# tomasjakab/imm

Hardware: AMD Instinct MI355X
Metric: training images/sec at 128x128 K=10 (higher is better)
Workload: dtype bf16; 1 GPU; BASELINE configs[1] (N>1: configs[2]): CelebA-shape 128x128 K=10 IMM training step (fwd + VGG16 perceptual loss + bwd + clip + Adam), batch 32 per GPU; global_batch=32, image_size=128, n_maps=10, parallelism=dp1, hip_graph=True, weights=seeded random init; synthetic VGG16 (vgg16.caffemodel.h5 unavailable offline)

## Files before the change

__graft_entry__.py:

```python
import os
import sys

ROOT = os.path.dirname(os.path.abspath(__file__))
if ROOT not in sys.path:
    sys.path.insert(0, ROOT)


def build():
    from imm_amd import build as _b
    lib = _b.build()
    import imm_amd
    from imm_amd import _lib
    handle = _lib.load()
    for name in _lib.declared_symbols() + _lib.alignment_symbols() + _lib.compose_symbols() + _lib.unalign_symbols() + _lib.track_symbols():
        getattr(handle, name)
    from oracle import imm_oracle, np_ref
    print('built', lib)


def smoke():
    import torch
    from oracle import imm_oracle as O
    from imm_amd.models.imm_model import IMMModel
    from imm_amd.train.cnn_train_multi import TrainStep
    from imm_amd.utils.box import Box
    assert torch.cuda.is_available(), 'smoke() needs cuda:0'
    torch.cuda.set_device(0)
    cfg = O.default_model_config(10)
    inputs = O.synthetic_inputs(2, 128, seed=0)
    model = IMMModel(Box(dict(cfg)), dtype=torch.bfloat16, device='cuda:0')
    ts = TrainStep(model, 2, 128, world_size=1, use_graph=True)
    loss = ts.step(inputs)
    ts.synchronize()
    eng = model.engine
    P, S = O.init_params(cfg, 128)
    out = O.forward(P, S, inputs, cfg, training=True)
    mu_err = float((eng.mu.cpu() - out['gauss_yx']).abs().max())
    loss_rel = abs(float(loss) - float(out['loss'])) / abs(float(out['loss']))
    print('smoke: loss %.4f (oracle %.4f, rel %.2e)  max|mu - oracle| %.2e  step_count %d' % (
        float(loss), float(out['loss']), loss_rel, mu_err, int(eng.step_count)))
    assert mu_err < 1e-3, mu_err
    assert loss_rel < 1e-3, loss_rel
    assert int(eng.step_count) == 1 and bool(torch.isfinite(eng.params).all())


if __name__ == '__main__':
    build()
    if len(sys.argv) > 1 and sys.argv[1] == 'smoke':
        smoke()
```

imm_amd/_lib.py:

```python
import ctypes as C
import os

import torch

_HERE = os.path.dirname(os.path.abspath(__file__))
LIB_PATH = os.environ.get('IMM_HIP_LIB') or os.path.join(_HERE, 'libimm_hip.so')

IMM_BF16, IMM_F16, IMM_F32 = 0, 1, 2
CONV_BIAS, CONV_RELU, CONV_STATS, CONV_MASK, CONV_OUT_F32 = 1, 2, 4, 8, 16
SSE_BLOCKS = 512
OPTIMIZERS = {'adam': 0, 'adadelta': 1, 'adagrad': 2}
GAUSS_MODES = {'rot': 0, 'flat': 1, 'ankush': 2}
ABI_VERSION = 28


class ImmHipError(RuntimeError):
    pass


class ConvDesc(C.Structure):
    _fields_ = [(n, C.c_int32) for n in (
        'batch', 'hi', 'wi', 'ci', 'ldx', 'ho', 'wo', 'co', 'ldy', 'kh', 'kw', 'stride', 'pad_t', 'pad_l',
        'updiv', 'kpad', 'flags', 'ldmask', 'out_scale', 'out_off_y', 'out_off_x')]


class WgradJob(C.Structure):
    _fields_ = [('desc', ConvDesc), ('x', C.c_void_p), ('dy', C.c_void_p), ('slab', C.c_void_p), ('lddy', C.c_int32),
                ('nsplit', C.c_int32), ('x_scale', C.c_void_p), ('x_shift', C.c_void_p), ('x_relu', C.c_int32),
                ('reserved', C.c_int32)]


class OptHParams(C.Structure):
    _fields_ = [('lr_start', C.c_float), ('lr_decay', C.c_float), ('lr_step', C.c_int32), ('lr_multiple', C.c_float),
                ('beta1', C.c_float), ('beta2', C.c_float), ('eps', C.c_float), ('clip', C.c_float),
                ('grad_scale', C.c_float), ('optim', C.c_int32),
                ('scale_growth_interval', C.c_int32), ('scale_max', C.c_float)]


class KeypointDesc(C.Structure):
    _fields_ = [('w', C.c_void_p), ('b', C.c_void_p), ('geom', C.c_void_p), ('keypoints', C.c_void_p), ('m', C.c_int32),
                ('image_size', C.c_int32)]


_P, _I, _L, _F, _D = C.c_void_p, C.c_int, C.c_int64, C.c_float, C.c_double
_SIGS = {
    'imm_abi_version': [],
    'imm_device_info': [_P],
    'imm_set_cu_limit': [_I],
    'imm_get_cu_limit': [],
    'imm_graph_begin': [_P],
    'imm_graph_end': [_P, C.POINTER(C.c_void_p)],
    'imm_graph_launch': [_P, _P],
    'imm_graph_destroy': [_P],
    'imm_pack_weights': [_P, _P, _I, _I, _I, _I, _I, _I, _I, _I, _I, _P],
    'imm_pack_weights_multi': [_P, _P, _I, _I, _I, _P],
    'imm_pack_weights_multi_blocks': [_I, _I, _I],
    'imm_wgrad_reduce_multi': [_P, _P, _I, _I, _P],
    'imm_conv2d': [C.POINTER(ConvDesc), _I, _P, _P, _P, _P, _P, _P, _P],
    'imm_conv_stats_blocks': [C.POINTER(ConvDesc)],
    'imm_conv2d_variant': [C.POINTER(ConvDesc), _I],
    'imm_conv2d_tap_supported': [C.POINTER(ConvDesc)],
    'imm_conv2d_tap': [C.POINTER(ConvDesc), _I, _P, _P, _P, _P, _P, _I, _P, _I, _P, _I, _I, _P],
    'imm_conv2d_wgrad': [C.POINTER(ConvDesc), _I, _P, _P, _I, _P, _I, _P],
    'imm_conv2d_wgrad_splits': [C.POINTER(ConvDesc), _I],
    'imm_conv2d_wgrad_variant': [C.POINTER(ConvDesc), _I, _I, C.POINTER(C.c_int), C.POINTER(C.c_int), C.POINTER(C.c_int)],
    'imm_conv2d_wgrad_multi_plan': [_P, _I, _I, _P],
    'imm_conv2d_wgrad_multi': [_P, _P, _P],
    'imm_conv2d_wgrad_reduce': [_P, _I, _I, _I, _I, _I, _I, _I, _P, _P],
    'imm_colsum': [_P, _I, _L, _I, _I, _I, _P, _P, _P],
    'imm_colsum_blocks': [_L, _I],
    'imm_bn_finalize': [_P, _I, _I, _L, _P, _P, _F, _F, _I, _P, _P, _P, _P, _P, _P, _P],
    'imm_bn_apply_relu': [_P, _I, _L, _I, _I, _P, _P, _I, _P, _I, _P],
    'imm_bn_apply_fused': [_P, _I, _I, _L, _P, _P, _F, _F, _I, _P, _P, _P, _P, _P, _P, _P, _I, _I, _I, _P, _I, _P, _I, _I, _I, _P],
    'imm_bn_bwd_apply_fused': [_P, _I, _I, _L, _P, _P, _I, _P, _I, _I, _P, _P, _P, _P, _I, _P, _P, _P, _I, _P],
    'imm_rows_reduce': [_P, _I, _I, _I, _P, _P],
    'imm_bn_bwd_reduce': [_P, _I, _P, _I, _I, _L, _I, _P, _P, _P, _P, _I, _P, _P],
    'imm_bn_bwd_blocks': [_L, _I],
    'imm_bn_bwd_reduce_up': [_P, _I, _P, _I, _P, _I, _I, _I, _I, _I, _I, _P, _P, _P, _P, _I, _P, _P],
    'imm_bn_bwd_finalize': [_P, _I, _I, _I, _L, _P, _P, _P, _I, _P, _P, _P, _P],
    'imm_bn_bwd_apply': [_P, _I, _P, _I, _I, _L, _I, _P, _P, _P, _P, _I, _P, _P, _I, _P],
    'imm_upsample2x_fwd': [_P, _P, _I, _I, _I, _I, _I, _I, _I, _P],
    'imm_upsample2x_bwd': [_P, _P, _I, _I, _I, _I, _I, _I, _I, _P],
    'imm_resize_ac_fwd': [_P, _P, _I, _I, _I, _I, _I, _I, _I, _I, _I, _P],
    'imm_resize_ac_bwd': [_P, _P, _I, _I, _I, _I, _I, _I, _I, _I, _I, _P],
    'imm_maxpool2_fwd': [_P, _P, _I, _I, _I, _I, _I, _P],
    'imm_maxpool2_bwd': [_P, _P, _P, _I, _I, _I, _I, _I, _I, _P],
    'imm_pack_image': [_P, _P, _I, _L, _P],
    'imm_pack_image_taps': [_P, _P, _I, _I, _I, _I, _I, _I, _I, _P],
    'imm_softargmax_gauss_fwd': [_P, _I, _I, _I, _I, _I, _F, _I, _P, _P, _P, _P, _I, _I, _I, _P],
    'imm_softargmax_gauss_bwd': [_P, _I, _I, _I, _I, _I, _I, _F, _I, _P, _P, _P, _P, _I, _I, _P],
    'imm_gauss_render_f32': [_P, _I, _I, _F, _I, _P, _I, _P],
    'imm_pose_head_fwd': [_P, _I, _I, _P, _I, _P, _I, _I, _I, _I, _I, _F, _I, _P, _I, _P, _P, _P, _P, _I, _I,
                          C.POINTER(KeypointDesc), _P],
    'imm_pose_head_bwd': [_P, _I, _I, _I, _I, _I, _I, _F, _I, _P, _P, _P, _P, _I, _I, _P, _I, _I, _P, _I, _P, _P],
    'imm_vgg_conv1_1_fwd': [_P, _P, _I, _I, _I, _P, _P, _P, _I, _I, _P],
    'imm_vgg_head_supported': [_I, _I, _I],
    'imm_vgg_head_fwd': [_P, _P, _I, _I, _I, _P, _P, _P, _I, _P, _P, _I, _P, _P, _I, _P],
    'imm_vgg_conv1_1_bwd': [_P, _I, _I, _I, _P, _P, _P, _I, _P, _P, _I, _I, _P, _I, _P],
    'imm_image_loss_grad': [_P, _P, _I, _I, _I, _P, _P, _I, _I, _P, _I, _I, _P],
    'imm_copy_f32': [_P, _P, _L, _P],
    'imm_debug_stamp': [_P, _I, _P],
    'imm_tps_warp': [_P, _I, _I, _I, _I, _I, _P, _I, _P, _P, _I, _P, _P, _I, _P],
    'imm_tps_warp_pad': [_P, _I, _I, _I, _I, _I, _I, _I, _I, _I, _I, _I, _I, _I, _P, _I, _P, _P, _I, _P],
    'imm_conv2d_group': [_P, _I, _I, _P, _P, _P, _P, _P, _P],
    'imm_conv_first_supported': [_I, _I, _I, _I],
    'imm_conv_first_stats_blocks': [_I, _I],
    'imm_conv_first': [_P, _P, _I, _P, _P, _I, _P, _I, _I, _I, _I, _I, _P],
    'imm_conv2d_nol_supported': [C.POINTER(ConvDesc)],
    'imm_conv2d_nol_stats_blocks': [C.POINTER(ConvDesc)],
    'imm_conv2d_nol': [C.POINTER(ConvDesc), _I, _P, _P, _P, _I, _P, _P, _P, _P, _P],
    'imm_conv2d_dgrad_s2_supported': [_I, _I, _I, _I, _I, _I],
    'imm_conv2d_dgrad_s2': [_P, _I, _P, _I, _P, _I, _I, _I, _I, _I, _I, _P],
    'imm_conv2d_group_stats_blocks': [_P, _I],
    'imm_upsample2x_bwd_bn': [_P, _P, _I, _I, _I, _I, _I, _I, _I, _P, _I, _P, _P],
    'imm_upsample2x_bwd_bn_blocks': [_I, _I, _I, _I],
    'imm_crc32c': [_P, C.c_uint64, C.POINTER(C.c_uint32)],
    'imm_rccl_unique_id': [_P],
    'imm_rccl_init': [_I, _I, _P, C.POINTER(C.c_void_p)],
    'imm_rccl_allreduce': [_P, _P, _L, _P],
    'imm_rccl_destroy': [_P],
    'imm_resize_crop_u8': [_P, _P, _P, _P, _I, _I, _I, _I, _I, _I, _I, _I, _P, _I, _P],
    'imm_unpool_tap_grad': [_P, _P, _P, _P, _I, _I, _I, _I, _P, _I, _P, _I, _P],
    'imm_masked_sse_pool': [_P, _P, _I, _I, _I, _I, _P, _I, _P, _P, _P, _P],
    'imm_masked_sse_multi': [_I, _P, _P, _P, _P, _P, _I, _I, _P, _I, _I, _P],
    'imm_masked_sse_all': [_I, _P, _P, _P, _P, _P, _I, _I, _P, _I, _I, _P, _I, _P, _I, _I, _P, _P],
    'imm_masked_sse': [_P, _P, _I, _I, _I, _I, _P, _I, _I, _P, _P],
    'imm_masked_sse_f32': [_P, _I, _P, _I, _I, _I, _I, _P, _I, _P, _P],
    'imm_perceptual_finalize': [_P, _I, _P, _P, _I, _P, _I, _I, _P, _P, _P],
    'imm_cost_ema': [_P, _P, _F, _P],
    'imm_rms16': [_P, _L, _I, _P, _I, _P, _P],
    'imm_tap_grad': [_P, _I, _P, _P, _I, _I, _I, _I, _P, _I, _P, _I, _I, _I, _P],
    'imm_weight_decay_loss': [_P, _P, _P, _P, _I, _P, _P, _P, _P],
    'imm_clip_adam_step': [_P, _P, _P, _P, _P, _P, _P, _I, _I, _P, _P, _P, _P, _P, _P, _P, C.POINTER(OptHParams), _P, _P],
}

_SIGS_ALIGN = {
    'imm_align_coeffs': [_P, _P, _I, _I, _I, _P, _P],
    'imm_align_warp_u8': [_P, _I, _P, _P, _I, _P, _P, _P, _P, _I, _I, _I, _I, _P, _I, _P],
}

_SIGS_COMPOSE = {
    'imm_compose_u8': [_P, _P, _P, _I, _P, _P, _P, _P, _I, _I, _I, _I, _P],
}

_SIGS_UNALIGN = {
    'imm_unalign_maps': [_P, _P, _P, _P, _I, _I, _I, _I, _P, _P, _P],
    'imm_unalign_u8': [_P, _P, _P, _I, _P, _P, _P, _P, _F, _P, _I, _I, _I, _I, _P],
}

_SIGS_TRACK = {
    'imm_track_step': [_P, _P, _P, _P, _I, _I, _I, _I, _I, _I, _D, _D, _D, _D, _D, _D, _I, _P, _P, _P, _P, _P, _P],
}

_SIGS64 = {
    'imm_conv2d_workspace_bytes': [C.POINTER(ConvDesc)],
    'imm_conv2d_group_workspace_bytes': [_P, _I],
    'imm_conv2d_wgrad_workspace_bytes': [C.POINTER(ConvDesc), _I, _I],
    'imm_conv2d_wgrad_multi_table_bytes': [_I],
    'imm_colsum_workspace_bytes': [_L, _I],
    'imm_bn_bwd_workspace_bytes': [_L, _I],
    'imm_upsample2x_bwd_bn_workspace_bytes': [_I, _I, _I, _I],
    'imm_masked_sse_workspace_bytes': [_I],
    'imm_vgg_head_scratch_bytes': [_I, _I],
}

_lib = None


def declared_symbols():
    return sorted(list(_SIGS) + list(_SIGS64) + ['imm_last_error', 'imm_source_digest'])


def alignment_symbols():
    return sorted(_SIGS_ALIGN)


def compose_symbols():
    return sorted(_SIGS_COMPOSE)


def unalign_symbols():
    return sorted(_SIGS_UNALIGN)


def track_symbols():
    return sorted(_SIGS_TRACK)


def load():
    global _lib
    if _lib is not None:
        return _lib
    if not os.path.exists(LIB_PATH):
        raise ImmHipError('libimm_hip.so not found at %s: build it with `python imm_amd/build.py` '
                          '(there is no CPU fallback for the product path)' % LIB_PATH)
    if 'IMM_HIP_LIB' not in os.environ and os.path.isdir(os.path.join(_HERE, 'csrc')):
        from . import build as _b
        want, have = _b.source_digest(), _b.library_digest(LIB_PATH)
        if want != have:
            if not _b.have_compiler():
                raise ImmHipError('libimm_hip.so is stale (built from sources %s.., checkout is %s..) and hipcc is not '
                                  'available to rebuild it' % (have[:12] or '?', want[:12]))
            _b.build(verbose=False)
    lib = C.CDLL(LIB_PATH)
    for name in ('imm_last_error', 'imm_source_digest'):
        getattr(lib, name).restype = C.c_char_p
        getattr(lib, name).argtypes = []
    for name, args in list(_SIGS.items()) + list(_SIGS_ALIGN.items()) + list(_SIGS_COMPOSE.items()) + list(_SIGS_UNALIGN.items()) + list(_SIGS_TRACK.items()):
        fn = getattr(lib, name)
        fn.argtypes = args
        fn.restype = C.c_int
    for name, args in _SIGS64.items():
        fn = getattr(lib, name)
        fn.argtypes = args
        fn.restype = C.c_int64
    v = lib.imm_abi_version()
    if v != ABI_VERSION:
        raise ImmHipError('libimm_hip.so ABI %d != expected %d' % (v, ABI_VERSION))
    _lib = lib
    return lib


def check(rc, what):
    if rc != 0:
        raise ImmHipError('%s failed (%d): %s' % (what, rc, load().imm_last_error().decode()))


def call(name, *args):
    rc = getattr(load(), name)(*args)
    if rc != 0:
        raise ImmHipError('%s failed (%d): %s' % (name, rc, load().imm_last_error().decode()))
```

imm_amd/csrc/loss_optim.hip:

```cpp
#include "common.h"

#define LO_THREADS 256
#define IMM_NORM2_SANE 1e30f

template <typename ET>
__global__ __launch_bounds__(LO_THREADS) void masked_sse_kernel(const typename ET::T* __restrict__ a, const typename ET::T* __restrict__ b,
                                                                int batch, int s, int c8n, const float* __restrict__ mask,
                                                                int S, int l1, float* __restrict__ partial) {
  __shared__ float red[4];
  const int r = S / s;
  const int64_t total = (int64_t)batch * s * s * c8n;
  float acc = 0.f;
  for (int64_t idx = (int64_t)blockIdx.x * blockDim.x + threadIdx.x; idx < total;
       idx += (int64_t)gridDim.x * blockDim.x) {
    const int64_t p = idx / c8n;
    float mk = 1.f;
    if (mask) {
      const int xx = (int)(p % s);
      const int64_t t = p / s;
      const int yy = (int)(t % s);
      const int64_t bi = t / s;
      mk = mask[(bi * S + (int64_t)yy * r) * S + (int64_t)xx * r];
    }
    float fa[8], fb[8];
// ... 101 lines not shown
  if (c == 3) {
    const bool a4 = lda == 4 && ((uintptr_t)a & 15) == 0, b4 = ldb == 4 && ((uintptr_t)b & 15) == 0;
    for (; p + 3 * stride < npix; p += 4 * stride) {
      float va[4][3], vb[4][3], mk[4];
#pragma unroll
      for (int u = 0; u < 4; ++u) {
        const int64_t q = p + u * stride;
        if (a4) { const float4 t = *(const float4*)(a + q * 4); va[u][0] = t.x; va[u][1] = t.y; va[u][2] = t.z; }
        else { va[u][0] = a[q * lda]; va[u][1] = a[q * lda + 1]; va[u][2] = a[q * lda + 2]; }
        if (b4) { const float4 t = *(const float4*)(b + q * 4); vb[u][0] = t.x; vb[u][1] = t.y; vb[u][2] = t.z; }
        else { vb[u][0] = b[q * ldb]; vb[u][1] = b[q * ldb + 1]; vb[u][2] = b[q * ldb + 2]; }
        mk[u] = mask ? mask[q] : 1.f;
      }
#pragma unroll
      for (int u = 0; u < 4; ++u) {
        float sq = 0.f;
#pragma unroll
        for (int ch = 0; ch < 3; ++ch) { const float d = va[u][ch] - vb[u][ch]; sq += l1 ? fabsf(d) : d * d; }
        acc += mk[u] * sq;
      }
    }
  }
  for (; p < npix; p += stride) {
    float sq = 0.f;
    for (int ch = 0; ch < c; ++ch) { const float d = a[p * lda + ch] - b[p * ldb + ch]; sq += l1 ? fabsf(d) : d * d; }
    acc += (mask ? mask[p] : 1.f) * sq;
  }
  return acc;
}

__global__ __launch_bounds__(LO_THREADS) void masked_sse_f32_kernel(const float* __restrict__ a, int lda,
                                                                    const float* __restrict__ b, int ldb, int64_t npix,
                                                                    int c, const float* __restrict__ mask, int l1,
                                                                    float* __restrict__ partial) {
  __shared__ float red[4];
  float acc = sse_f32_thread_sum(a, lda, b, ldb, npix, c, mask, l1);
  acc = block_sum_256(acc, red);
  if (threadIdx.x == 0) partial[blockIdx.x] = acc;
}

struct SseRgbArgs { const float* a; const float* b; int lda, ldb, c; int64_t npix; float* partial; };
template <typename ET>
__global__ __launch_bounds__(LO_THREADS) void masked_sse_all_kernel(const SseMultiArgs g, int n16, const SseRgbArgs rgb, int batch,
                                                                    const float* __restrict__ mask, int S, int l1) {
  __shared__ float red[4];
  const int f = blockIdx.y;
  float acc = 0.f;
  if (f == n16) {
    acc = sse_f32_thread_sum(rgb.a, rgb.lda, rgb.b, rgb.ldb, rgb.npix, rgb.c, mask, l1);
    acc = block_sum_256(acc, red);
    if (threadIdx.x == 0) rgb.partial[blockIdx.x] = acc;
    return;
  }
  const typename ET::T* __restrict__ a = (const typename ET::T*)g.a[f];
  const typename ET::T* __restrict__ b = (const typename ET::T*)g.b[f];
  const int s = g.s[f], c8n = g.c8n[f];
  const int r = S / s;
  const int64_t total = (int64_t)batch * s * s * c8n;
  for (int64_t idx = (int64_t)blockIdx.x * blockDim.x + threadIdx.x; idx < total;
       idx += (int64_t)gridDim.x * blockDim.x) {
    const int64_t p = idx / c8n;
    float mk = 1.f;
    if (mask) {
      const int xx = (int)(p % s);
      const int64_t t = p / s;
      const int yy = (int)(t % s);
      const int64_t bi = t / s;
      mk = mask[(bi * S + (int64_t)yy * r) * S + (int64_t)xx * r];
    }
    float fa[8], fb[8];
    unpack8<ET>(ld8<ET>(a + idx * 8), fa);
    unpack8<ET>(ld8<ET>(b + idx * 8), fb);
    float sq = 0.f;
#pragma unroll
    for (int i = 0; i < 8; ++i) { const float d = fa[i] - fb[i]; sq += l1 ? fabsf(d) : d * d; }
    acc += mk * sq;
  }
  acc = block_sum_256(acc, red);
  if (threadIdx.x == 0) g.partial[f][blockIdx.x] = acc;
}

extern "C" int imm_masked_sse(const void* a, const void* b, int dtype, int batch, int s, int c, const float* mask, int S,
                              int l1, float* partial, void* stream) {
  IMM_REQUIRE(a && b && partial && batch > 0 && s > 0 && c > 0 && c % 8 == 0, "masked_sse: args");
  IMM_REQUIRE(mask == nullptr || (S >= s && S % s == 0), "masked_sse: mask side %d not a multiple of feature side %d", S, s);
  IMM_DISPATCH_DTYPE_F32(dtype, hipLaunchKernelGGL((masked_sse_kernel<ET>), dim3(IMM_SSE_BLOCKS), dim3(LO_THREADS), 0,
                                               (hipStream_t)stream, (const typename ET::T*)a, (const typename ET::T*)b, batch, s, c / 8,
                                               mask, S, l1, partial));
  IMM_CHECK_LAUNCH("imm_masked_sse");
  return 0;
}

extern "C" int imm_masked_sse_multi(int n, const void* const* a, const void* const* b, const int32_t* s_host, const int32_t* c_host,
                                    float* const* partial, int dtype, int batch, const float* mask, int S, int l1, void* stream) {
  IMM_REQUIRE(n >= 1 && n <= 8 && a && b && s_host && c_host && partial && batch > 0, "masked_sse_multi: args");
  SseMultiArgs g;
  for (int i = 0; i < 8; ++i) {
    const int k = i < n ? i : 0;
    IMM_REQUIRE(a[k] && b[k] && partial[k] && s_host[k] > 0 && c_host[k] > 0 && c_host[k] % 8 == 0, "masked_sse_multi: feature %d", k);
    IMM_REQUIRE(mask == nullptr || (S >= s_host[k] && S % s_host[k] == 0), "masked_sse_multi: mask side %d vs feature side %d", S, s_host[k]);
    g.a[i] = a[k]; g.b[i] = b[k]; g.s[i] = s_host[k]; g.c8n[i] = c_host[k] / 8; g.partial[i] = partial[k];
  }
  IMM_DISPATCH_DTYPE_F32(dtype, hipLaunchKernelGGL((masked_sse_multi_kernel<ET>), dim3(IMM_SSE_BLOCKS, n), dim3(LO_THREADS), 0,
                                               (hipStream_t)stream, g, batch, mask, S, l1));
  IMM_CHECK_LAUNCH("imm_masked_sse_multi");
  return 0;
}

extern "C" int imm_masked_sse_all(int n, const void* const* a, const void* const* b, const int32_t* s_host, const int32_t* c_host,
                                  float* const* partial, int dtype, int batch, const float* mask, int S, int l1,
                                  const float* img_a, int lda, const float* img_b, int ldb, int img_c, float* img_partial, void* stream) {
  IMM_REQUIRE(n >= 1 && n <= 8 && a && b && s_host && c_host && partial && batch > 0, "masked_sse_all: args");
  IMM_REQUIRE(img_a && img_b && img_partial && img_c > 0 && lda >= img_c && ldb >= img_c && S > 0, "masked_sse_all: image pair");
  SseMultiArgs g;
  for (int i = 0; i < 8; ++i) {
    const int k = i < n ? i : 0;
    IMM_REQUIRE(a[k] && b[k] && partial[k] && s_host[k] > 0 && c_host[k] > 0 && c_host[k] % 8 == 0, "masked_sse_all: feature %d", k);
    IMM_REQUIRE(S >= s_host[k] && S % s_host[k] == 0, "masked_sse_all: image side %d vs feature side %d", S, s_host[k]);
    g.a[i] = a[k]; g.b[i] = b[k]; g.s[i] = s_host[k]; g.c8n[i] = c_host[k] / 8; g.partial[i] = partial[k];
  }
  SseRgbArgs rgb;
  rgb.a = img_a; rgb.b = img_b; rgb.lda = lda; rgb.ldb = ldb; rgb.c = img_c; rgb.npix = (int64_t)batch * S * S; rgb.partial = img_partial;
  IMM_DISPATCH_DTYPE_F32(dtype, hipLaunchKernelGGL((masked_sse_all_kernel<ET>), dim3(IMM_SSE_BLOCKS, n + 1), dim3(LO_THREADS), 0,
                                               (hipStream_t)stream, g, n, rgb, batch, mask, S, l1));
  IMM_CHECK_LAUNCH("imm_masked_sse_all");
  return 0;
}

extern "C" int imm_masked_sse_pool(const void* a, const void* b, int dtype, int batch, int s, int c, const float* mask, int S,
                                   float* partial, void* pool_a, void* pool_b, void* stream) {
  IMM_REQUIRE(a && b && partial && pool_b && batch > 0 && s > 0 && s % 2 == 0 && c > 0 && c % 8 == 0, "masked_sse_pool: args");
  IMM_REQUIRE(mask == nullptr || (S >= s && S % s == 0), "masked_sse_pool: mask side %d not a multiple of feature side %d", S, s);
  IMM_DISPATCH_DTYPE_F32(dtype, hipLaunchKernelGGL((masked_sse_pool_kernel<ET>), dim3(IMM_SSE_BLOCKS), dim3(LO_THREADS), 0,
                                               (hipStream_t)stream, (const typename ET::T*)a, (const typename ET::T*)b, batch, s, c / 8,
                                               mask, S, partial, (typename ET::T*)pool_a, (typename ET::T*)pool_b));
  IMM_CHECK_LAUNCH("imm_masked_sse_pool");
  return 0;
}

extern "C" int imm_masked_sse_f32(const float* a, int lda, const float* b, int ldb, int batch, int s, int c,
                                  const float* mask, int l1, float* partial, void* stream) {
  IMM_REQUIRE(a && b && partial && batch > 0 && s > 0 && c > 0 && lda >= c && ldb >= c, "masked_sse_f32: args");
  hipLaunchKernelGGL(masked_sse_f32_kernel, dim3(IMM_SSE_BLOCKS), dim3(LO_THREADS), 0, (hipStream_t)stream, a, lda, b, ldb,
                     (int64_t)batch * s * s, c, mask, l1, partial);
  IMM_CHECK_LAUNCH("imm_masked_sse_f32");
  return 0;
}

#define PF_THREADS 1024
__global__ __launch_bounds__(PF_THREADS) void perceptual_finalize_kernel(const float* __restrict__ partial, int nfeat,
                                                                         const float* __restrict__ nel, float* agg,
                                                                         int training, const float* __restrict__ wd_loss,
                                                                         int l1, int mode, const float* __restrict__ loss_scale,
                                                                         float* __restrict__ out) {
  __shared__ double sse[16];
  const int tid = threadIdx.x, lane = tid & 63, wave = tid >> 6;
  const float nel_f = tid < nfeat ? nel[tid] : 1.f;
  const float agg_f = tid < nfeat ? agg[tid] : 1.f;
  const float ls = (tid < nfeat && loss_scale) ? loss_scale[0] : 1.f;
  const float wd = (tid == 0 && wd_loss) ? wd_loss[0] : 0.f;
  if (wave < nfeat) {
    const float* pf = partial + wave * IMM_SSE_BLOCKS + lane;
    float x[IMM_SSE_BLOCKS / 64];
#pragma unroll
    for (int i = 0; i < IMM_SSE_BLOCKS / 64; ++i) x[i] = pf[64 * i];
    double v = 0.0;
#pragma unroll
    for (int i = 0; i < IMM_SSE_BLOCKS / 64; ++i) v += (double)x[i];
#pragma unroll 1
    for (int o = 32; o >= 1; o >>= 1) v += __shfl_xor(v, o, 64);
    if (lane == 0) sse[wave] = v;
  }
  __syncthreads();
  if (mode == IMM_LOSS_L2) {
    if (tid == 0) {
      const float m = (float)(sse[0] / (double)nel_f);
      out[0] = m; out[nfeat] = m;
      out[2 * nfeat] = ls * ((1000.f / 255.f) * 2.f / nel_f);
      out[3 * nfeat] = 1000.f * m;
      out[3 * nfeat + 1] = wd;
      out[3 * nfeat + 2] = 1000.f * m / 255.f + wd;
    }
    return;
  }
  __shared__ float terms[16];
  if (tid < nfeat) {
    const int f = tid;
    const float m = (float)(sse[f] / (double)nel_f);
    const float a = agg_f;
    const float wl = a + 0.01f * (m - a);
    const float term = m / wl;
    out[f] = term;
    out[nfeat + f] = m;
    out[2 * nfeat + f] = ls * (1000.f * (1.f / wl - 0.01f * m / (wl * wl)) * (l1 ? 1.f : 2.f) / nel_f);
    if (training) agg[f] = wl;
    terms[f] = term;
  }
  __syncthreads();
  if (tid == 0) {
    float rec = 0.f;
    for (int f = 0; f < nfeat; ++f) rec += terms[f];
    rec *= 1000.f;
    out[3 * nfeat] = rec;
    out[3 * nfeat + 1] = wd;
    out[3 * nfeat + 2] = rec + wd;
  }
}

extern "C" int imm_perceptual_finalize(const float* partial, int nfeat, const float* nel, float* agg, int training,
                                       const float* wd_loss, int l1, int mode, const float* loss_scale, float* out,
                                       void* stream) {
  IMM_REQUIRE(partial && nel && agg && out && nfeat > 0 && nfeat <= 16, "perceptual_finalize: args");
  IMM_REQUIRE(mode == IMM_LOSS_PERCEPTUAL || (mode == IMM_LOSS_L2 && nfeat == 1 && !l1), "perceptual_finalize: mode");
  hipLaunchKernelGGL(perceptual_finalize_kernel, dim3(1), dim3(PF_THREADS), 0, (hipStream_t)stream, partial, nfeat, nel,
                     agg, training, wd_loss, l1, mode, loss_scale, out);
  IMM_CHECK_LAUNCH("imm_perceptual_finalize");
  return 0;
}

template <typename ET>
__global__ void tap_grad_kernel(typename ET::T* __restrict__ da, int has_in, const typename ET::T* __restrict__ ap,
                                const typename ET::T* __restrict__ ag, int batch, int s, int c8n, const float* __restrict__ mask,
                                int S, const float* __restrict__ coef, int idx_coef, int relu, int l1) {
  const int r = S / s;
  const float ck = coef[idx_coef];
  const int64_t total = (int64_t)batch * s * s * c8n;
  for (int64_t idx = (int64_t)blockIdx.x * blockDim.x + threadIdx.x; idx < total;
       idx += (int64_t)gridDim.x * blockDim.x) {
    const int64_t p = idx / c8n;
    float mk = 1.f;
    if (mask) {
      const int xx = (int)(p % s);
      const int64_t t = p / s;
      const int yy = (int)(t % s);
      const int64_t bi = t / s;
      mk = mask[(bi * S + (int64_t)yy * r) * S + (int64_t)xx * r];
    }
    float fp[8], fg[8], d[8];
    unpack8<ET>(ld8<ET>(ap + idx * 8), fp);
    unpack8<ET>(ld8<ET>(ag + idx * 8), fg);
    if (has_in) unpack8<ET>(ld8<ET>(da + idx * 8), d);
    const float cm = ck * mk;
#pragma unroll
    for (int i = 0; i < 8; ++i) {
      float e = fp[i] - fg[i];
      if (l1) e = e > 0.f ? 1.f : (e < 0.f ? -1.f : 0.f);
      float v = (has_in ? d[i] : 0.f) + cm * e;
      if (relu && !(fp[i] > 0.f)) v = 0.f;
      d[i] = v;
    }
    st8<ET>(da + idx * 8, pack8<ET>(d));
  }
}

template <typename ET>
__global__ void unpool_tap_grad_kernel(typename ET::T* __restrict__ da, const typename ET::T* __restrict__ dpool,
                                       const typename ET::T* __restrict__ ap, const typename ET::T* __restrict__ ag, int batch, int s,
                                       int c8n, const float* __restrict__ mask, int S, const float* __restrict__ coef,
                                       int idx_coef) {
  const int r = S / s, so = s / 2, c = c8n * 8;
  const float ck = coef[idx_coef];
  const int64_t total = (int64_t)batch * so * so * c8n;
  for (int64_t idx = (int64_t)blockIdx.x * blockDim.x + threadIdx.x; idx < total;
       idx += (int64_t)gridDim.x * blockDim.x) {
    const int cg = (int)(idx % c8n);
    int64_t t = idx / c8n;
    const int X = (int)(t % so); t /= so;
    const int Y = (int)(t % so);
    const int64_t bi = t / so;
    const int64_t off = ((bi * s + 2 * Y) * s + 2 * X) * c + cg * 8;
    const int64_t qoff[4] = {off, off + c, off + (int64_t)s * c, off + (int64_t)s * c + c};
    float fp[4][8], fg[4][8], g[8], o[4][8], cm[4];
#pragma unroll
    for (int q = 0; q < 4; ++q) {
      unpack8<ET>(ld8<ET>(ap + qoff[q]), fp[q]);
      unpack8<ET>(ld8<ET>(ag + qoff[q]), fg[q]);
      const int yy = 2 * Y + (q >> 1), xx = 2 * X + (q & 1);
      cm[q] = ck * (mask ? mask[(bi * S + (int64_t)yy * r) * S + (int64_t)xx * r] : 1.f);
    }
    unpack8<ET>(ld8<ET>(dpool + ((bi * so + Y) * so + X) * c + cg * 8), g);
#pragma unroll
    for (int i = 0; i < 8; ++i) {
      int am = 0; float mv = fp[0][i];
#pragma unroll
      for (int q = 1; q < 4; ++q) if (fp[q][i] > mv) { mv = fp[q][i]; am = q; }
#pragma unroll
      for (int q = 0; q < 4; ++q) {
        float v = ((q == am) ? g[i] : 0.f) + cm[q] * (fp[q][i] - fg[q][i]);
        if (!(fp[q][i] > 0.f)) v = 0.f;
        o[q][i] = v;
      }
    }
#pragma unroll
    for (int q = 0; q < 4; ++q) st8<ET>(da + qoff[q], pack8<ET>(o[q]));
  }
}

extern "C" int imm_unpool_tap_grad(void* da, const void* dpool, const void* a_pred, const void* a_gt, int dtype, int batch, int s,
                                   int c, const float* mask, int S, const float* coef, int idx, void* stream) {
  IMM_REQUIRE(da && dpool && a_pred && a_gt && coef && batch > 0 && s > 0 && s % 2 == 0 && c > 0 && c % 8 == 0 && idx >= 0,
              "unpool_tap_grad: args");
  IMM_REQUIRE(mask == nullptr || (S >= s && S % s == 0), "unpool_tap_grad: mask side");
  const int64_t total = (int64_t)batch * (s / 2) * (s / 2) * (c / 8);
  int64_t blocks = (total + LO_THREADS - 1) / LO_THREADS;
  if (blocks > 16384) blocks = 16384;
  IMM_DISPATCH_DTYPE_F32(dtype, hipLaunchKernelGGL((unpool_tap_grad_kernel<ET>), dim3((int)blocks), dim3(LO_THREADS), 0,
                                               (hipStream_t)stream, (typename ET::T*)da, (const typename ET::T*)dpool,
                                               (const typename ET::T*)a_pred, (const typename ET::T*)a_gt, batch, s, c / 8, mask, S, coef, idx));
  IMM_CHECK_LAUNCH("imm_unpool_tap_grad");
  return 0;
}

extern "C" int imm_tap_grad(void* da, int has_in, const void* a_pred, const void* a_gt, int dtype, int batch, int s, int c,
                            const float* mask, int S, const float* coef, int idx, int relu, int l1, void* stream) {
  IMM_REQUIRE(da && a_pred && a_gt && coef && batch > 0 && s > 0 && c > 0 && c % 8 == 0 && idx >= 0, "tap_grad: args");
  IMM_REQUIRE(mask == nullptr || (S >= s && S % s == 0), "tap_grad: mask side");
  const int64_t total = (int64_t)batch * s * s * (c / 8);
  int64_t blocks = (total + LO_THREADS - 1) / LO_THREADS;
  if (blocks > 16384) blocks = 16384;
  IMM_DISPATCH_DTYPE_F32(dtype, hipLaunchKernelGGL((tap_grad_kernel<ET>), dim3((int)blocks), dim3(LO_THREADS), 0,
                                               (hipStream_t)stream, (typename ET::T*)da, has_in, (const typename ET::T*)a_pred,
                                               (const typename ET::T*)a_gt, batch, s, c / 8, mask, S, coef, idx, relu, l1));
  IMM_CHECK_LAUNCH("imm_tap_grad");
  return 0;
}

template <typename ET>
__global__ void image_loss_grad_kernel(const float* __restrict__ gt, const float* __restrict__ pred, int ldp, int64_t npix,
                                       const float* __restrict__ mask, const float* __restrict__ coef, int idx, int l1,
                                       typename ET::T* __restrict__ dpred, int lddp) {
  const int nvec = lddp / 8;
  const float ck = coef[idx];
  for (int64_t i = (int64_t)blockIdx.x * blockDim.x + threadIdx.x; i < npix * nvec; i += (int64_t)gridDim.x * blockDim.x) {
    const int64_t p = i / nvec;
    const int cg = (int)(i - p * nvec);
    float o[8] = {0.f, 0.f, 0.f, 0.f, 0.f, 0.f, 0.f, 0.f};
    if (cg == 0) {
      const float cm = ck * (mask ? mask[p] : 1.f);
#pragma unroll
      for (int ch = 0; ch < 3; ++ch) {
        float d = pred[p * ldp + ch] - gt[p * 3 + ch];
        if (l1) d = d > 0.f ? 1.f : (d < 0.f ? -1.f : 0.f);
        o[ch] = cm * d;
      }
    }
    st8<ET>(dpred + p * lddp + cg * 8, pack8<ET>(o));
  }
}

extern "C" int imm_image_loss_grad(const float* gt, const float* pred, int ldp, int batch, int s, const float* mask,
                                   const float* coef, int idx, int l1, void* dpred, int lddp, int dtype, void* stream) {
  IMM_REQUIRE(gt && pred && coef && dpred && batch > 0 && s > 0 && ldp >= 3 && idx >= 0, "image_loss_grad: args");
  IMM_REQUIRE(lddp >= 8 && lddp % 8 == 0, "image_loss_grad: lddp=%d must be a multiple of 8", lddp);
  const int64_t npix = (int64_t)batch * s * s;
  int64_t blocks = (npix * (lddp / 8) + LO_THREADS - 1) / LO_THREADS;
  if (blocks > 8192) blocks = 8192;
  IMM_DISPATCH_DTYPE_F32(dtype, hipLaunchKernelGGL((image_loss_grad_kernel<ET>), dim3((int)blocks), dim3(LO_THREADS), 0,
                                               (hipStream_t)stream, gt, pred, ldp, npix, mask, coef, idx, l1,
                                               (typename ET::T*)dpred, lddp));
  IMM_CHECK_LAUNCH("imm_image_loss_grad");
  return 0;
}

__global__ __launch_bounds__(LO_THREADS) void wd_partial_kernel(const float* __restrict__ params,
                                                                const int32_t* __restrict__ blk_seg,
                                                                const int32_t* __restrict__ blk_begin,
                                                                const int32_t* __restrict__ blk_end,
                                                                const float* __restrict__ seg_wd,
                                                                float* __restrict__ blk_partial) {
  __shared__ float red[4];
  const int blk = blockIdx.x;
  const float wd = seg_wd[blk_seg[blk]];
  float acc = 0.f;
  if (wd != 0.f)
    for (int i = blk_begin[blk] + threadIdx.x; i < blk_end[blk]; i += LO_THREADS) { const float w = params[i]; acc += w * w; }
  acc = block_sum_256(acc, red);
  if (threadIdx.x == 0) blk_partial[blk] = 0.5f * wd * acc;
}

__global__ __launch_bounds__(LO_THREADS) void sum_partials_kernel(const float* __restrict__ partial, int n, float* out) {
  __shared__ double dred[LO_THREADS];
  double v = 0.0;
  for (int i = threadIdx.x; i < n; i += LO_THREADS) v += (double)partial[i];
  dred[threadIdx.x] = v;
  __syncthreads();
  for (int o = LO_THREADS / 2; o > 0; o >>= 1) {
    if (threadIdx.x < o) dred[threadIdx.x] += dred[threadIdx.x + o];
    __syncthreads();
  }
  if (threadIdx.x == 0) out[0] = (float)dred[0];
}

extern "C" int imm_weight_decay_loss(const float* params, const int32_t* blk_seg, const int32_t* blk_begin,
                                     const int32_t* blk_end, int nblk, const float* seg_wd, float* blk_partial, float* out,
                                     void* stream) {
  IMM_REQUIRE(params && blk_seg && blk_begin && blk_end && seg_wd && blk_partial && out && nblk > 0, "weight_decay_loss: args");
  hipLaunchKernelGGL(wd_partial_kernel, dim3(nblk), dim3(LO_THREADS), 0, (hipStream_t)stream, params, blk_seg, blk_begin,
                     blk_end, seg_wd, blk_partial);
  hipLaunchKernelGGL(sum_partials_kernel, dim3(1), dim3(LO_THREADS), 0, (hipStream_t)stream, blk_partial, nblk, out);
  IMM_CHECK_LAUNCH("imm_weight_decay_loss");
  return 0;
}

__global__ void cost_ema_kernel(const float* __restrict__ cost3, float* __restrict__ state, float decay) {
  if (threadIdx.x < 3) state[threadIdx.x] = decay * state[threadIdx.x] + (1.f - decay) * cost3[threadIdx.x];
  if (threadIdx.x == 3) state[3] += 1.f;
}

extern "C" int imm_cost_ema(const float* cost3, float* state4, float decay, void* stream) {
  IMM_REQUIRE(cost3 && state4 && decay >= 0.f && decay < 1.f, "cost_ema: args");
  hipLaunchKernelGGL(cost_ema_kernel, dim3(1), dim3(64), 0, (hipStream_t)stream, cost3, state4, decay);
  IMM_CHECK_LAUNCH("imm_cost_ema");
  return 0;
}

template <typename ET>
__global__ __launch_bounds__(LO_THREADS) void sumsq16_kernel(const typename ET::T* __restrict__ x, int64_t n8, float* __restrict__ partial) {
  __shared__ float red[4];
  float acc = 0.f;
  for (int64_t i = (int64_t)blockIdx.x * LO_THREADS + threadIdx.x; i < n8; i += (int64_t)gridDim.x * LO_THREADS) {
    float f[8];
    unpack8<ET>(ld8<ET>(x + i * 8), f);
#pragma unroll
    for (int e = 0; e < 8; ++e) acc = fmaf(f[e], f[e], acc);
  }
  acc = block_sum_256(acc, red);
  if (threadIdx.x == 0) partial[blockIdx.x] = acc;
}

__global__ __launch_bounds__(LO_THREADS) void rms_finish_kernel(const float* __restrict__ partial, int n, double count, float* out) {
  __shared__ double dred[LO_THREADS];
  double v = 0.0;
  for (int i = threadIdx.x; i < n; i += LO_THREADS) v += (double)partial[i];
  dred[threadIdx.x] = v;
  __syncthreads();
  for (int o = LO_THREADS / 2; o > 0; o >>= 1) {
    if (threadIdx.x < o) dred[threadIdx.x] += dred[threadIdx.x + o];
    __syncthreads();
  }
  if (threadIdx.x == 0) out[0] = (float)sqrt(dred[0] / count);
}

extern "C" int imm_rms16(const void* x, int64_t n, int dtype, float* partial, int nblk, float* out, void* stream) {
  IMM_REQUIRE(x && partial && out && n > 0 && n % 8 == 0 && nblk > 0 && nblk <= 4096, "rms16: args (n must be a multiple of 8)");
  IMM_REQUIRE(((uintptr_t)x % 16) == 0, "rms16: 16-byte alignment");
  IMM_DISPATCH_DTYPE_F32(dtype, hipLaunchKernelGGL((sumsq16_kernel<ET>), dim3(nblk), dim3(LO_THREADS), 0, (hipStream_t)stream,
                                              (const typename ET::T*)x, n / 8, partial));
  hipLaunchKernelGGL(rms_finish_kernel, dim3(1), dim3(LO_THREADS), 0, (hipStream_t)stream, partial, nblk, (double)n, out);
  IMM_CHECK_LAUNCH("imm_rms16");
  return 0;
}

__device__ __forceinline__ void opt_learning_rate(const imm_opt_hparams& hp, int gs, int tt, float* lr_t, float* lr) {
  const double l = (double)hp.lr_multiple * (double)hp.lr_start * pow((double)hp.lr_decay, (double)(gs / hp.lr_step));
  *lr_t = (float)(l * sqrt(1.0 - pow((double)hp.beta2, (double)tt)) / (1.0 - pow((double)hp.beta1, (double)tt)));
  *lr = (float)l;
}

__global__ __launch_bounds__(LO_THREADS) void grad_prepare_kernel(const float* __restrict__ params, float* __restrict__ grads,
                                                                  const int32_t* __restrict__ blk_seg,
                                                                  const int32_t* __restrict__ blk_begin,
                                                                  const int32_t* __restrict__ blk_end,
                                                                  const float* __restrict__ seg_wd, float grad_scale,
                                                                  const float* __restrict__ loss_scale,
                                                                  float* __restrict__ blk_partial, int nblk,
                                                                  const int32_t* __restrict__ step_count,
                                                                  const int32_t* __restrict__ adam_t, float* __restrict__ lr_state,
                                                                  imm_opt_hparams hp) {
  __shared__ float red[4];
  const int blk = blockIdx.x;
  if (blk == nblk) {
    if (threadIdx.x == 0) opt_learning_rate(hp, step_count[0], adam_t[0] + 1, lr_state, lr_state + 1);
    return;
  }
  if (loss_scale) grad_scale *= 1.f / loss_scale[0];
  const float wd = seg_wd[blk_seg[blk]];
  float acc = 0.f;
  const int b0 = blk_begin[blk], b1 = blk_end[blk];
  const int a0 = min((b0 + 3) & ~3, b1), a1 = max(a0, b1 & ~3);
  for (int i = b0 + threadIdx.x; i < a0; i += LO_THREADS) {
    const float g = grads[i] * grad_scale + wd * params[i];
    grads[i] = g; acc += g * g;
  }
  for (int i = a0 + 4 * threadIdx.x; i < a1; i += 4 * LO_THREADS) {
    float4 g = *(const float4*)(grads + i);
    const float4 w = *(const float4*)(params + i);
    g.x = g.x * grad_scale + wd * w.x; g.y = g.y * grad_scale + wd * w.y;
    g.z = g.z * grad_scale + wd * w.z; g.w = g.w * grad_scale + wd * w.w;
    *(float4*)(grads + i) = g;
    acc += (g.x * g.x + g.y * g.y) + (g.z * g.z + g.w * g.w);
  }
  for (int i = a1 + threadIdx.x; i < b1; i += LO_THREADS) {
    const float g = grads[i] * grad_scale + wd * params[i];
    grads[i] = g; acc += g * g;
  }
  acc = block_sum_256(acc, red);
  if (threadIdx.x == 0) blk_partial[blk] = acc;
}

__global__ __launch_bounds__(LO_THREADS) void clip_adam_kernel(float* __restrict__ params, const float* __restrict__ grads,
                                                               float* __restrict__ m, float* __restrict__ v,
                                                               const int32_t* __restrict__ blk_seg,
                                                               const int32_t* __restrict__ blk_begin,
                                                               const int32_t* __restrict__ blk_end,
                                                               const int32_t* __restrict__ seg_first_blk,
                                                               const float* __restrict__ blk_partial, int nblk,
                                                               float* __restrict__ seg_norm2, int32_t* __restrict__ step_count,
                                                               int32_t* __restrict__ adam_t, const float* __restrict__ lr_state,
                                                               float* __restrict__ ls, imm_opt_hparams hp) {
  __shared__ double dred[LO_THREADS / 64];
  const int blk = blockIdx.x, tid = threadIdx.x;
  const bool extra = blk == nblk;
  const int seg = extra ? 0 : blk_seg[blk];
  const int b0 = extra ? 0 : blk_begin[blk], b1 = extra ? 0 : blk_end[blk];
  const int a0 = min((b0 + 3) & ~3, b1), a1 = max(a0, b1 & ~3);
  const int i0 = a0 + 4 * tid;
  const bool first = i0 < a1;
  float4 g0 = {0.f, 0.f, 0.f, 0.f}, m0 = g0, v0 = g0, w0 = g0;
  if (first) { g0 = *(const float4*)(grads + i0); m0 = *(const float4*)(m + i0); v0 = *(const float4*)(v + i0); w0 = *(const float4*)(params + i0); }

  const int f0 = seg_first_blk[seg], f1 = seg_first_blk[seg + 1];
  double ps = 0.0;
  int bad = 0;
  const int sb1 = ls != nullptr ? nblk : f1;
  int sb0 = tid;
  if (ls == nullptr && f0 > tid) sb0 = tid + (f0 - tid + LO_THREADS - 1) / LO_THREADS * LO_THREADS;
  for (int b = sb0; b < sb1; b += LO_THREADS) {
    const float p = blk_partial[b];
    bad |= !(p <= IMM_NORM2_SANE);
    if (b >= f0 && b < f1) ps += (double)p;
  }
#pragma unroll
  for (int o = 32; o > 0; o >>= 1) ps += __shfl_xor(ps, o, 64);
  if ((tid & 63) == 0) dred[tid >> 6] = ps;
  bad = __syncthreads_or(bad);
  const bool skip = ls != nullptr && bad != 0;
  double t = 0.0;
#pragma unroll
  for (int w = 0; w < LO_THREADS / 64; ++w) t += dred[w];
  const float norm2 = (float)t;
  if (tid == 0 && !extra && blk == f0) seg_norm2[seg] = norm2;
  if (extra) {
    if (tid == 0) {
      if (ls) {
        float S = ls[0], clean = ls[1];
        if (skip) { S = fmaxf(S * 0.5f, 1.f); clean = 0.f; ls[2] += 1.f; }
        else if (hp.scale_growth_interval > 0 && clean + 1.f >= (float)hp.scale_growth_interval) {
          S = fminf(S * 2.f, hp.scale_max > 0.f ? hp.scale_max : S * 2.f); clean = 0.f;
        } else clean += 1.f;
        ls[0] = S; ls[1] = clean; ls[3] = skip ? 1.f : 0.f;
      }
      if (!skip) {
        step_count[0] += 1;
        adam_t[0] += 1;
      }
    }
    return;
  }
  if (skip) return;
  float factor = 1.f;
  if (hp.clip > 0.f) factor = hp.clip / fmaxf(sqrtf(norm2), hp.clip);
  const float lr_t = lr_state[0], lr = lr_state[1];
  auto one = [&](float g, float& mi, float& vi, float& w) {
    g *= factor;
    if (hp.optim == IMM_OPT_ADAM) {
      mi = hp.beta1 * mi + (1.f - hp.beta1) * g;
      vi = hp.beta2 * vi + (1.f - hp.beta2) * g * g;
      w -= lr_t * mi / (sqrtf(vi) + hp.eps);
    } else if (hp.optim == IMM_OPT_ADADELTA) {
      vi = hp.beta1 * vi + (1.f - hp.beta1) * g * g;
      const float u = sqrtf(mi + hp.eps) / sqrtf(vi + hp.eps) * g;
      mi = hp.beta1 * mi + (1.f - hp.beta1) * u * u;
      w -= lr * u;
    } else {
      vi += g * g;
      w -= lr * g / sqrtf(vi);
    }
  };
  for (int i = b0 + tid; i < a0; i += LO_THREADS) one(grads[i], m[i], v[i], params[i]);
  if (first) {
    one(g0.x, m0.x, v0.x, w0.x); one(g0.y, m0.y, v0.y, w0.y); one(g0.z, m0.z, v0.z, w0.z); one(g0.w, m0.w, v0.w, w0.w);
    *(float4*)(m + i0) = m0; *(float4*)(v + i0) = v0; *(float4*)(params + i0) = w0;
  }
  for (int i = i0 + 4 * LO_THREADS; i < a1; i += 4 * LO_THREADS) {
    const float4 g = *(const float4*)(grads + i);
    float4 mi = *(const float4*)(m + i), vi = *(const float4*)(v + i), w = *(const float4*)(params + i);
    one(g.x, mi.x, vi.x, w.x); one(g.y, mi.y, vi.y, w.y); one(g.z, mi.z, vi.z, w.z); one(g.w, mi.w, vi.w, w.w);
    *(float4*)(m + i) = mi; *(float4*)(v + i) = vi; *(float4*)(params + i) = w;
  }
  for (int i = a1 + tid; i < b1; i += LO_THREADS) one(grads[i], m[i], v[i], params[i]);
}

extern "C" int imm_clip_adam_step(float* params, float* grads, float* m, float* v, const int32_t* blk_seg,
                                  const int32_t* blk_begin, const int32_t* blk_end, int nblk, int nseg,
                                  const int32_t* seg_first_blk, const float* seg_wd, float* blk_partial, float* seg_norm2,
                                  int32_t* step_count, int32_t* adam_t, float* lr_state, const imm_opt_hparams* hp,
                                  float* loss_scale_state, void* stream) {
  IMM_REQUIRE(params && grads && m && v && blk_seg && blk_begin && blk_end && seg_first_blk && seg_wd && blk_partial &&
                  seg_norm2 && step_count && adam_t && lr_state && hp, "clip_adam_step: null");
  IMM_REQUIRE(nblk > 0 && nseg > 0 && hp->lr_step > 0, "clip_adam_step: dims");
  IMM_REQUIRE(hp->optim >= IMM_OPT_ADAM && hp->optim <= IMM_OPT_ADAGRAD, "clip_adam_step: optim %d", hp->optim);
  hipStream_t s = (hipStream_t)stream;
  hipLaunchKernelGGL(grad_prepare_kernel, dim3(nblk + 1), dim3(LO_THREADS), 0, s, params, grads, blk_seg, blk_begin, blk_end,
                     seg_wd, hp->grad_scale, loss_scale_state, blk_partial, nblk, step_count, adam_t, lr_state, *hp);
  hipLaunchKernelGGL(clip_adam_kernel, dim3(nblk + 1), dim3(LO_THREADS), 0, s, params, grads, m, v, blk_seg, blk_begin, blk_end,
                     seg_first_blk, blk_partial, nblk, seg_norm2, step_count, adam_t, lr_state, loss_scale_state, *hp);
  IMM_CHECK_LAUNCH("imm_clip_adam_step");
  return 0;
}
```

imm_amd/engine.py:

```python
import math
import os
from collections import OrderedDict

import numpy as np
import torch

from . import _lib as L
from . import ops

BN_EPS = 1e-3
BN_MOMENTUM = 0.99
BN_DIRECT_ROWS = int(os.environ.get('IMM_BN_DIRECT_ROWS', '512'))
WEIGHT_DECAY = 1e-5
INIT_STD = 0.01
PERCEPTUAL_WS = [100.0, 1.6, 2.3, 1.8, 2.8, 100.0]
SUPPORTED_COMP = ['input', 'conv1_2', 'conv2_2', 'conv3_2', 'conv4_2', 'conv5_2']
VGG_LAYERS = [('conv1_1', 1, 64), ('conv1_2', 64, 64), ('conv2_1', 64, 128), ('conv2_2', 128, 128),
              ('conv3_1', 128, 256), ('conv3_2', 256, 256), ('conv3_3', 256, 256),
              ('conv4_1', 256, 512), ('conv4_2', 512, 512), ('conv4_3', 512, 512),
              ('conv5_1', 512, 512), ('conv5_2', 512, 512)]
VGG_POOL_AFTER = ('conv1_2', 'conv2_2', 'conv3_3', 'conv4_3')
WGRAD_MULTI_MAX_JOBS, WGRAD_MULTI_MAX_VARIANTS = 64, 16


# ... 2 lines not shown
    for gk, members in groups.items():
        generic = gk[0] // 100000 == 0
        members = list(members)
        while members:
            room_jobs, room_slots = max_jobs - cur_jobs, max_slots - cur_slots
            take = min(len(members), room_jobs, room_slots) if generic else (min(len(members), room_jobs) if room_slots >= 1 else 0)
            if take <= 0:
                chunks.append(cur); cur, cur_jobs, cur_slots = [], 0, 0
                continue
            part, members = members[:take], members[take:]
            cur.append((gk, part)); cur_jobs += len(part); cur_slots += len(part) if generic else 1
    if cur:
        chunks.append(cur)
    return chunks
COST_EMA_STATE = 'summaries/cost_movavg'
VGG_TAPS = {'conv1_2': 1, 'conv2_2': 2, 'conv3_2': 3, 'conv4_2': 4, 'conv5_2': 5}


def encoder_spec(n_filters):
    f = n_filters
    return [(7, 3, f, 1), (3, f, f, 1), (3, f, 2 * f, 2), (3, 2 * f, 2 * f, 1), (3, 2 * f, 4 * f, 2),
            (3, 4 * f, 4 * f, 1), (3, 4 * f, 8 * f, 2), (3, 8 * f, 8 * f, 1)]


def renderer_spec(cfg, image_size, n_out):
    filters = cfg.n_filters_render * 8
    cin = cfg.n_filters * 8 + cfg.n_maps
    size, spec = 16, []
    while size <= image_size:
        spec.append((3, cin, filters, True, False))
        if size == image_size:
            spec.append((3, filters, n_out, False, False))
            break
        spec.append((3, filters, filters, True, True))
        cin = filters
        size *= 2
        if filters >= 8:
            filters //= 2
    return spec


def render_sizes(cfg, max_size):
    sizes, size = [], max_size
    while True:
        sizes.append(size)
        if size <= cfg.min_res:
            break
        size = size // cfg.renderer_stride
    return sizes


def n_renderer_out(cfg):
    extra = len(cfg.perceptual.comp) if getattr(cfg, 'channels_bug_fix', False) else 0
    return 3 + extra


def trainable_spec(cfg, image_size):
    out = []

    def add(scope, k, cin, cout, bn):
        out.append((scope + '/w', (k, k, cin, cout), WEIGHT_DECAY))
        out.append((scope + '/b', (cout,), 0.0))
        if bn:
            out.append((scope + '/gamma', (cout,), 0.0))
            out.append((scope + '/beta', (cout,), 0.0))

    for enc in ('image_encoder', 'pose_encoder'):
        for i, (k, ci, co, _s) in enumerate(encoder_spec(cfg.n_filters)):
            add('model/%s/encoder/conv_%d' % (enc, i + 1), k, ci, co, True)
        if enc == 'pose_encoder':
            add('model/pose_encoder/conv_1', 1, cfg.n_filters * 8, cfg.n_maps, False)
    for i, (k, ci, co, bn, _u) in enumerate(renderer_spec(cfg, image_size, n_renderer_out(cfg))):
        add('model/renderer/conv_%d' % (i + 1), k, ci, co, bn)
    return out


def truncated_normal(rng, shape, std):
    z = rng.standard_normal(shape)
    bad = np.abs(z) > 2.0
    while bad.any():
        z[bad] = rng.standard_normal(int(bad.sum()))
        bad = np.abs(z) > 2.0
    return (z * std).astype(np.float32)


def synthetic_vgg_weights(seed=2):
    rng = np.random.default_rng(seed)
    w = OrderedDict()
    for name, cin, cout in VGG_LAYERS:
        w['vgg16/%s/weights' % name] = torch.from_numpy(
            (rng.standard_normal((3, 3, cin, cout)) * math.sqrt(2.0 / (9 * cin))).astype(np.float32))
        w['vgg16/%s/biases' % name] = torch.from_numpy((rng.standard_normal(cout) * 0.1).astype(np.float32))
    return w


class _Launch:
    __slots__ = ('fn', 'tag', 'flops', 'bytes', 'name', 'lane', 'variant', 'cus', 'group')

    def __init__(self, fn, tag, flops=0.0, nbytes=0.0, name='', lane=0, variant='', cus=0, group=''):
        self.fn, self.tag, self.flops, self.bytes, self.name, self.lane, self.variant = fn, tag, flops, nbytes, name, lane, variant
        self.cus, self.group = cus, group


class _ConvLayer:
    pass


class IMMEngine:
    def __init__(self, cfg, batch, image_size, device='cuda:0', act_dtype=torch.bfloat16, seed=1, vgg_weights=None,
                 hparams=None, world_size=1, dp_buckets=None):
        if cfg.gauss_mode not in L.GAUSS_MODES:
            raise ValueError('Unknown mode: ' + str(cfg.gauss_mode))
        if cfg.reconstruction_loss not in ('perceptual', 'l2'):
            raise ValueError('Reconsutruction loss-type: ' + str(cfg.reconstruction_loss) + ' not understood')
        self.loss_kind = cfg.reconstruction_loss
        self.comp = list(cfg.perceptual.comp) if self.loss_kind == 'perceptual' else ['input']
        if self.loss_kind == 'perceptual':
            if not self.comp or len(set(self.comp)) != len(self.comp) or len(self.comp) > len(PERCEPTUAL_WS):
                raise ValueError('perceptual.comp must name 1..%d distinct features, got %r' % (len(PERCEPTUAL_WS), self.comp))
            if any(n not in SUPPORTED_COMP for n in self.comp):
                raise NotImplementedError('perceptual.comp entries must come from %r (the layers the shipped configs tap), got %r'
                                          % (SUPPORTED_COMP, self.comp))
        self.l1 = self.loss_kind == 'perceptual' and not cfg.perceptual.l2
        if image_size % 16 or image_size < 64:
            raise ValueError('image side must be a multiple of 16 and >= 64')
        L.load()
        self.cfg, self.B, self.S, self.dev, self.dt = cfg, int(batch), int(image_size), torch.device(device), act_dtype
        self.f32 = act_dtype == torch.float32
        self.K = int(cfg.n_maps)
        self.world_size = world_size
        self.dp_buckets = int(dp_buckets if dp_buckets is not None else os.environ.get('IMM_DP_BUCKETS', '1'))
        self.use_mask = bool(cfg.loss_mask)
        self.n_cu, self.arch = ops.device_info()
        self._alloc_bytes = 0

        self.spec = trainable_spec(cfg, self.S)
        sizes = [int(np.prod(s)) for _n, s, _w in self.spec]
        self.tab = ops.SegmentTable(sizes, [w for _n, _s, w in self.spec], self.dev)
        self.params = self._zeros(self.tab.total)
        self.grads = self._zeros(self.tab.total)
        self.adam_m = self._zeros(self.tab.total)
        self.adam_v = self._zeros(self.tab.total)
        self.pview, self.gview = OrderedDict(), OrderedDict()
        for i, (name, shape, _wd) in enumerate(self.spec):
            o0, o1 = self.tab.offsets[i], self.tab.offsets[i + 1]
            self.pview[name] = self.params[o0:o1].view(shape)
            self.gview[name] = self.grads[o0:o1].view(shape)
        self.opt_blk_partial = self._zeros(self.tab.nblk)
        self.seg_norm2 = self._zeros(self.tab.nseg)
        self.step_count = torch.zeros(1, dtype=torch.int32, device=self.dev)
        self.adam_t = torch.zeros(1, dtype=torch.int32, device=self.dev)
        self.lr_state = self._zeros(2)
        self.wd_loss = self._zeros(1)
        hp = dict(lr_start=1e-3, lr_decay=0.95, lr_step=100000, lr_multiple=1.0, beta1=0.9, beta2=0.999, eps=1e-8,
                  clip=1.0, grad_scale=1.0 / world_size, optim='adam', scale_growth_interval=1000, scale_max=2.0 ** 24)
        hp.update(hparams or {})
        ls0 = hp.pop('loss_scale', 4096.0 if act_dtype == torch.float16 else 0.0) or 0.0
        if ls0 and (ls0 < 1.0 or math.log2(ls0) != int(math.log2(ls0))):
            raise ValueError('loss_scale must be a power of two >= 1, got %r' % (ls0,))
        self.loss_scale_state = None
        if ls0:
            self.loss_scale_state = self._zeros(4)
            self.loss_scale_state[0] = float(ls0)
        self._loss_scale_init = float(ls0)
        self.optim = str(hp['optim']).lower()
        if self.optim not in L.OPTIMIZERS:
            raise ValueError('Optimizer = %s not suppoerted' % hp['optim'])
        if self.optim == 'adadelta':
            hp.update(beta1=0.95, eps=1e-6)
        hp['optim'] = L.OPTIMIZERS[self.optim]
        self.hp = ops.OptHParams(**hp)

        self.state = OrderedDict()
        self.nfeat = len(self.comp)
        self.loss_agg = torch.tensor(PERCEPTUAL_WS[:self.nfeat], dtype=torch.float32, device=self.dev)
        self.vgg_w = OrderedDict()
        for k, v in (vgg_weights or synthetic_vgg_weights()).items():
            self.vgg_w[k] = torch.empty(tuple(v.shape), dtype=v.dtype, device=self.dev)
            ops.upload(self.vgg_w[k], v, k)

        self.prog_pack, self.prog_fwd, self.prog_bwd, self.prog_opt = [], [], [], []
        self.two_streams = os.environ.get('IMM_TWO_STREAMS', '1') != '0'
        self.nol = os.environ.get('IMM_NOL', '0') != '0' and not self.f32
        self._skip_tags = set(t for t in os.environ.get('IMM_DEBUG_SKIP_TAGS', '').split(',') if t)
        self._stamp_mode = os.environ.get('IMM_DEBUG_STAMPS', '')
        self._stamp_buf = torch.zeros(8192, dtype=torch.int64, device=self.dev) if self._stamp_mode else None
        self._stamp_names = []
        self._side = None
        self._pack_jobs, self._reduce_jobs, self._wgrad_pending, self._colsum_pending = [], [], [], []
        self._training = True
        self._build_network()
        self.init_parameters(seed)

    def _zeros(self, *shape, dtype=torch.float32):
        t = torch.zeros(*shape, dtype=dtype, device=self.dev)
        self._alloc_bytes += t.numel() * t.element_size()
        return t

    def _act(self, *shape):
        return self._zeros(*shape, dtype=self.dt)

    def init_parameters(self, seed=1):
        rng = np.random.default_rng(seed)
        host = torch.zeros(self.tab.total, dtype=torch.float32)
        for i, (name, shape, _wd) in enumerate(self.spec):
            o0 = self.tab.offsets[i]
            n = int(np.prod(shape))
            if name.endswith('/w'):
                host[o0:o0 + n] = torch.from_numpy(truncated_normal(rng, shape, INIT_STD)).reshape(-1)
            elif name.endswith('/gamma'):
                host[o0:o0 + n] = 1.0
        ops.upload(self.params, host, 'the initial parameters')
        for k, v in self.state.items():
            v.fill_(1.0 if k.endswith('moving_variance') else 0.0)
        self.loss_agg.copy_(torch.tensor(PERCEPTUAL_WS[:self.nfeat]))
        self.reset_optimizer_slots(); self.grads.zero_(); self.step_count.zero_()
        self.run(self.prog_pack)

    def reset_optimizer_slots(self):
        self.adam_m.zero_()
        self.adam_v.fill_(0.1 if self.optim == 'adagrad' else 0.0)
        self.adam_t.zero_()
        if self.loss_scale_state is not None:
            self.loss_scale_state.zero_()
            self.loss_scale_state[0] = self._loss_scale_init

    def load_parameters(self, named, state=None):
        for name in self.pview:
            ops.upload(self.pview[name], named[name], name)
        if state:
            for k, v in state.items():
                if k in self.state:
                    ops.upload(self.state[k], v, k)
                elif k.startswith('loss/') and k.endswith('_agg'):
                    if self.loss_kind == 'perceptual' and k[5:-4] in self.comp:
                        self.loss_agg[self.comp.index(k[5:-4])] = float(v)
                elif k.startswith('vgg16/'):
                    ops.upload(self.vgg_w[k], v, k)
                elif k == COST_EMA_STATE:
                    ops.upload(self.cost_ema, torch.as_tensor(v, dtype=torch.float32).reshape(4), k)
                else:
                    raise KeyError(k)
            self._pack_vgg()
        self.run(self.prog_pack)

    def named_parameters(self):
        return OrderedDict((k, v.detach().clone()) for k, v in self.pview.items())

    def named_state(self):
        out = OrderedDict((k, v.detach().clone()) for k, v in self.state.items())
        if self.loss_kind == 'perceptual':
            for i, name in enumerate(self.comp):
                out['loss/%s_agg' % name] = self.loss_agg[i].detach().clone()
        out[COST_EMA_STATE] = self.cost_ema.detach().clone()
        return out

    def _add(self, prog, fn, tag, flops=0.0, nbytes=0.0, name='', desc=None, variant=''):
        cus = int(getattr(self, '_cur_cus', 0))
        if desc is not None:
            if cus:
                ops.set_cu_limit(cus)
            try:
                variant = '%s:%d' % ops.conv2d_variant(desc, self.dt)
            finally:
                if cus:
                    ops.set_cu_limit(0)
        prog.append(_Launch(fn, tag, flops, nbytes, name or getattr(self, '_cur_scope', ''), getattr(self, '_cur_lane', 0), variant,
                            cus, getattr(self, '_cur_group', '')))

    def _signal(self, prog, key, lane=None):
        prog.append(_Launch(None, 'record:' + key, lane=self._cur_lane if lane is None else lane, group=getattr(self, '_cur_group', '')))

    def _wait(self, prog, key, lane):
        prog.append(_Launch(None, 'wait:' + key, lane=lane))

    def _mark(self, prog, what, lane=1):
        prog.append(_Launch(None, what, lane=lane, group=getattr(self, '_cur_group', '')))

    def _nol_consumer_ok(self, H, W, ci, ldx, co, k, stride, bn, out_f32):
        if not self.nol or k != 3 or ci != ldx:
            return False
        ldy = ops.round_up(co, 4) if out_f32 else ops.round_up(co, 8)
        flags = L.CONV_BIAS | (L.CONV_OUT_F32 if out_f32 else 0) | (L.CONV_STATS if bn else 0)
        fd = ops.fwd_desc(self.B, H, W, ci, ldx, co, ldy, k, stride, flags)
        if not ops.conv2d_nol_supported(fd):
            return False
        lddy = ldy if not out_f32 else ops.round_up(co, 32)
        key, _wps, _units, _pcu = ops.conv2d_wgrad_variant(fd, lddy, self.dt)
        return key // 100000 == 2

    def _conv_block(self, scope, x, H, W, ci_real, ci_pad, ldx, co, k, stride, bn, relu, needs_dgrad,
                    out=None, ldo=None, out_f32=False, kw=None, up2x=False, fwd_launch=True, nol_src=None, defer_apply=False,
                    first_src=None):
        B, dt, dev = self.B, self.dt, self.dev
        self._cur_scope = scope
        lay = _ConvLayer()
        lay.scope, lay.bn, lay.relu, lay.x, lay.ldx = scope, bn, relu, x, ldx
        lay.nol_src = nol_src
        assert nol_src is None or (nol_src.bn and x is nol_src.y and ldx == nol_src.ldy)
        kw = k if kw is None else kw
        lay.ci_real, lay.ci_pad, lay.co, lay.k, lay.stride, lay.H, lay.W, lay.kw = ci_real, ci_pad, co, k, stride, H, W, kw
        flags = L.CONV_BIAS | (L.CONV_OUT_F32 if out_f32 else 0)
        ldy = ops.round_up(co, 4) if out_f32 else ops.round_up(co, 8)
        lay.ldy = ldy
        fd = ops.fwd_desc(B, H, W, ci_pad, ldx, co, ldy, k, stride, flags | (L.CONV_STATS if bn else 0), kw=kw)
        fd_eval = ops.fwd_desc(B, H, W, ci_pad, ldx, co, ldy, k, stride, flags, kw=kw)
        lay.fd, lay.Ho, lay.Wo = fd, fd.ho, fd.wo
        npix = B * fd.ho * fd.wo
        lay.npix = npix
        w, b = self.pview[scope + '/w'], self.pview[scope + '/b']
        rows = ops.round_up(co, 128)
        lay.wt = self._zeros(rows, fd.kpad, dtype=dt)
        self._pack_jobs.append(((w.data_ptr(), lay.wt.data_ptr(), 0, k, kw, ci_real, co, ci_pad, rows, fd.kpad), rows * fd.kpad))
        lay.y = self._zeros(B, fd.ho, fd.wo, ldy, dtype=torch.float32 if out_f32 else dt)
        flops = 2.0 * npix * k * kw * ci_real * co
        if bn:
            cus_q = int(getattr(self, '_cur_cus', 0))
            if cus_q:
                ops.set_cu_limit(cus_q)
            try:
                nblk = (ops.conv_first_stats_blocks(B, H) if first_src is not None else
                        ops.conv_stats_blocks(fd) if nol_src is None else ops.conv2d_nol_stats_blocks(fd))
            finally:
                if cus_q:
                    ops.set_cu_limit(0)
            lay.stats = self._zeros(nblk, 2, co)
            lay.scale, lay.shift, lay.mean, lay.rstd = (self._zeros(co) for _ in range(4))
            mm, mv = self._zeros(co), self._zeros(co)
            mv.fill_(1.0)
            self.state[scope + '/moving_mean'], self.state[scope + '/moving_variance'] = mm, mv
            gamma, beta = self.pview[scope + '/gamma'], self.pview[scope + '/beta']
            fused_up = bool(up2x) and not defer_apply and nblk <= BN_DIRECT_ROWS and co % 32 == 0
            if out is None and not defer_apply and not fused_up:
                out, ldo = self._act(B, fd.ho, fd.wo, co), co
            lay.out, lay.ldo = out, (ldo if out is not None else None)
            lay.nol = bool(defer_apply)

            def f_conv():
                if first_src is not None:
                    ops.conv_first(first_src, lay.wt, b, lay.y, ldy, lay.stats if self._training else None, B, H, co,
                                   L.CONV_BIAS | (L.CONV_STATS if self._training else 0))
                elif nol_src is not None:
                    ops.conv2d_nol(fd if self._training else fd_eval, x, nol_src.scale, nol_src.shift, nol_src.relu, lay.wt, b, lay.y,
                                   lay.stats if self._training else None)
# ... 338 lines not shown
        self.n_fwd_model = len(self.prog_fwd)

        self.vgg_act, self.vgg_wt, self.vgg_wtd, self.vgg_desc = OrderedDict(), {}, {}, {}
        self.vgg_pool = {}
        self.tap_idx = {n: k for k, n in enumerate(self.comp)}
        vnames = [n for n, _ci, _co in VGG_LAYERS]
        taps = [n for n in self.comp if n != 'input'] if self.loss_kind == 'perceptual' else []
        self.vgg_layers = VGG_LAYERS[:max(vnames.index(n) for n in taps) + 1] if taps else []
        nfeat = self.nfeat
        self.sse_partial = self._zeros(nfeat, L.SSE_BLOCKS)
        fuse_ok = not self.l1
        fused_sse = set()
        self._sse_input_early = ('input' in self.tap_idx and bool(self.vgg_layers) and
                                 os.environ.get('IMM_SSE_INPUT_LANE', '0') != '0')
        if self._sse_input_early:
            idx0 = self.tap_idx['input']
            self._cur_scope = 'loss'
            self._mark(self.prog_fwd, 'fork', lane=1)
            self._cur_lane = 1
            self._add(self.prog_fwd, lambda: ops.masked_sse_f32(self.in_future, 3, self.pred, self.ldp, B, S, 3, self.in_mask,
                                                                self.sse_partial[idx0], self.l1), 'sse')
            self._cur_lane = 0
        split = bool(self.vgg_layers) and os.environ.get('IMM_VGG_SPLIT', '0') != '0'
        self.vgg_split = split
        self.gt_cus = int(os.environ.get('IMM_GT_CUS', '128')) if split else 0
        halves = ([('gt', slice(0, B), 2, self.gt_cus), ('pred', slice(B, 2 * B), 0, 0)] if split else
                  [('', slice(0, 2 * B), 0, 0)])
        gt_prog = []
        for hname, hs, lane, cus in halves:
            if not self.vgg_layers:
                break
            prog = gt_prog if hname == 'gt' else self.prog_fwd
            self._cur_lane, self._cur_cus, self._cur_group = lane, cus, ('gt' if hname == 'gt' else '')
            sfx = ' [%s]' % hname if hname else ''
            nb = hs.stop - hs.start
            if hname != 'pred':
                self.w11 = self._zeros(9, 64); self.b11 = self._zeros(64)
                a = self._act(2 * B, S, S, 64)
                self.vgg_act['conv1_1'] = (a, S)
            a = self.vgg_act['conv1_1'][0]
            hv = {'': 3, 'gt': 1, 'pred': 2}[hname]
            head_fused = (not split and len(self.vgg_layers) > 1 and not self.f32 and os.environ.get('IMM_VGG_HEAD', '1') != '0'
                          and ops.vgg_head_supported(B, S, dt))
            self.vgg_head_fused = head_fused
            if head_fused:
                self.vgg_gray = torch.empty(ops.vgg_head_scratch_bytes(B, S), dtype=torch.uint8, device=self.dev)
            else:
                self._add(prog, (lambda a=a, hv=hv: ops.vgg_conv1_1_fwd(self.in_future, self.pred, self.ldp, B, S, self.w11, self.b11, a, hv)),
                          'vgg_conv1_1', 2.0 * nb * S * S * 9 * 64, nb * S * S * 128.0, name='vgg16/conv1_1' + sfx)
            x, H = a, S
            for li, (name, cin, cout) in enumerate(self.vgg_layers[1:], start=1):
                fd = ops.fwd_desc(nb, H, H, cin, cin, cout, cout, 3, 1, L.CONV_BIAS | L.CONV_RELU)
                if hname != 'pred':
                    wt = self._zeros(ops.round_up(cout, 128), fd.kpad, dtype=dt)
                    wtd = self._zeros(ops.round_up(cin, 128), ops.round_up(9 * cout, 32), dtype=dt)
                    y = self._act(2 * B, H, H, cout)
                    self.vgg_wt[name], self.vgg_wtd[name], self.vgg_desc[name] = wt, wtd, fd
                    self.vgg_act[name] = (y, H)
                wt, y = self.vgg_wt[name], self.vgg_act[name][0]
                bias = self.vgg_w['vgg16/%s/biases' % name]
                if li == 1 and head_fused:
                    self._add(prog, (lambda a=a, wt=wt, bias=bias, y=y: ops.vgg_head_fwd(
                        self.in_future, self.pred, self.ldp, B, S, self.w11, self.b11, wt, bias, a, B, y, self.vgg_gray)),
                              'vgg_fwd', 2.0 * nb * S * S * 9 * (64 + cin * cout),
                              nb * S * S * 12.0 + 2.0 * (B * S * S * 64 + nb * S * S * cout + 9 * cin * cout),
                              name='vgg16/conv1_1+' + name, variant='vgg_head')
                else:
                    self._add(prog, (lambda fd=fd, x=x, wt=wt, bias=bias, y=y, hs=hs: ops.conv2d(fd, x[hs], wt, bias, y[hs])),
                              'vgg_fwd', 2.0 * nb * H * H * 9 * cin * cout, 2.0 * (nb * H * H * (cin + cout) + 9 * cin * cout),
                              name='vgg16/' + name + sfx, desc=fd)
                if hname == 'gt' and name in taps:
                    self._signal(prog, 'gt:' + name)
                x = y
                if name in VGG_POOL_AFTER and li < len(self.vgg_layers) - 1:
                    if hname != 'pred':
                        self.vgg_pool[name] = self._act(2 * B, H // 2, H // 2, cout)
                    p = self.vgg_pool[name]
                    if name in taps and fuse_ok and hname != 'gt':
                        idx = self.tap_idx[name]
                        fused_sse.add(name)
                        if hname == 'pred':
                            self._wait(prog, 'gt:' + name, lane=0)
                        pa = None if hname == 'pred' else p[:B]
                        self._add(prog, (lambda x=x, p=p, pa=pa, H=H, cout=cout, idx=idx: ops.masked_sse_pool(
                            x[:B], x[B:], B, H, cout, self.in_mask, S, self.sse_partial[idx], pa, p[B:])), 'sse',
                                  0.0, 2 * B * H * H * cout * 2.5, name='vgg16/%s+pool' % name)
                    else:
                        self._add(prog, (lambda x=x, p=p, H=H, cout=cout, hs=hs, nb=nb: ops.maxpool2_fwd(x[hs], p[hs], nb, H, H, cout)),
                                  'maxpool', 0.0, nb * H * H * cout * 2.5, name='vgg16/pool_' + name + sfx)
                    x, H = p, H // 2
        self._cur_lane, self._cur_cus, self._cur_group = 0, 0, ''
        if gt_prog:
            self._cur_group = 'gt'
            head = []
            self._mark(head, 'fork', lane=2)
            self._cur_group = ''
            self.prog_fwd[0:0] = head + gt_prog
            self.n_fwd_model += len(head) + len(gt_prog)
        if self.vgg_layers:
            self._pack_vgg()

        nel = []
        for name in self.comp:
            if name == 'input':
                nel.append(float(B * S * S * 3))
            else:
                y, H = self.vgg_act[name]
                nel.append(float(B * H * H * y.shape[-1]))
        self.nel = torch.tensor(nel, dtype=torch.float32, device=self.dev)
        self.loss_out = self._zeros(3 * nfeat + 3)
        self.cost_ema = self._zeros(4)
        mask = self.in_mask
        l1 = self.l1
        self._cur_scope = 'loss'
        if self._sse_input_early:
            self._mark(self.prog_fwd, 'join', lane=1)
        tail = [name for name in taps if name not in fused_sse]
        sse_all = ('input' in self.tap_idx and not self._sse_input_early and len(tail) > 1 and
                   os.environ.get('IMM_SSE_ALL', '1') != '0')
        if 'input' in self.tap_idx and not self._sse_input_early and not sse_all:
            idx0 = self.tap_idx['input']
            self._add(self.prog_fwd, lambda: ops.masked_sse_f32(self.in_future, 3, self.pred, self.ldp, B, S, 3, mask,
                                                                self.sse_partial[idx0], l1), 'sse')
        if self.vgg_split:
            self._cur_group = 'gt'
            self._mark(self.prog_fwd, 'join', lane=2)
            self._cur_group = ''
        if len(tail) > 1:
            feats = []
            for name in tail:
                y, H = self.vgg_act[name]
                feats.append((y[:B], y[B:], H, y.shape[-1], self.sse_partial[self.tap_idx[name]]))
            self.sse_multi = ops.SseMulti(feats)
            if sse_all:
                idx0 = self.tap_idx['input']
                self._add(self.prog_fwd, lambda: ops.masked_sse_all(self.sse_multi, B, mask, S, self.in_future, 3, self.pred, self.ldp, 3,
                                                                    self.sse_partial[idx0], l1), 'sse', 0.0,
                          sum(2 * B * f[2] * f[2] * f[3] * 2.0 for f in feats) + B * S * S * (3 + self.ldp + 1) * 4.0)
            else:
                self._add(self.prog_fwd, lambda: ops.masked_sse_multi(self.sse_multi, B, mask, S, l1), 'sse', 0.0,
                          sum(2 * B * f[2] * f[2] * f[3] * 2.0 for f in feats))
            tail = []
        for name in tail:
            idx = self.tap_idx[name]
            y, H = self.vgg_act[name]
            c = y.shape[-1]
            self._add(self.prog_fwd, (lambda y=y, H=H, c=c, idx=idx: ops.masked_sse(y[:B], y[B:], B, H, c, mask, S,
                                                                                  self.sse_partial[idx], l1)), 'sse',
                      0.0, 2 * B * H * H * c * 2.0)
        mode = ops.LOSS_L2 if self.loss_kind == 'l2' else ops.LOSS_PERCEPTUAL
        self._add(self.prog_fwd, lambda: ops.perceptual_finalize(self.sse_partial, nfeat, self.nel, self.loss_agg,
                                                                 self._training, self.wd_loss, self.loss_out, l1, mode,
                                                                 self.loss_scale_state), 'loss_finalize')
        self.coef = self.loss_out[2 * nfeat:3 * nfeat]

        self._build_backward()
        self.pack_tab = ops.pack_table([j for j, _n in self._pack_jobs], self.dev)
        self._add(self.prog_pack, lambda: ops.pack_weights_multi(self.pack_tab, dt), 'pack')

        self._add(self.prog_opt, lambda: ops.clip_adam_step(self.params, self.grads, self.adam_m, self.adam_v, self.tab,
                                                            self.opt_blk_partial, self.seg_norm2, self.step_count,
                                                            self.adam_t, self.lr_state, self.hp, self.loss_scale_state),
                  'clip_adam', 0.0, self.tab.total * 36.0)
        self.prog_opt.extend(self.prog_pack)

    def _pack_vgg(self):
        if not self.vgg_layers:
            return
        w = self.vgg_w
        self.w11.copy_(w['vgg16/conv1_1/weights'].reshape(9, 64))
        self.b11.copy_(w['vgg16/conv1_1/biases'])
        for name, cin, cout in self.vgg_layers[1:]:
            fd = self.vgg_desc[name]
            wm = w['vgg16/%s/weights' % name]
            ops.pack_weights(wm, self.vgg_wt[name], 0, 3, 3, cin, cout, cin, self.vgg_wt[name].shape[0], fd.kpad)
            wtd = self.vgg_wtd[name]
            ops.pack_weights(wm, wtd, 1, 3, 3, cin, cout, cout, wtd.shape[0], wtd.shape[1])

    def _build_backward(self):
        B, S, K, dt, Cj = self.B, self.S, self.K, self.dt, self.Cj
        mask = self.in_mask
        acts = self.vgg_act
        l1 = self.l1
        names = [n for n, _ci, _co in self.vgg_layers]
        taps = self.tap_idx
        dbuf = {n: self._act(B, acts[n][1], acts[n][1], acts[n][0].shape[-1]) for n in names}
        dpool = {n: self._act(B, acts[n][1] // 2, acts[n][1] // 2, acts[n][0].shape[-1]) for n in self.vgg_pool}

        def pred_half(t):
            return t[B:]

        def tap(name, has_in):
            y, H = acts[name]
            c = y.shape[-1]
            self._add(self.prog_bwd, lambda: ops.tap_grad(dbuf[name], has_in, y[B:], y[:B], B, H, c, mask, S, self.coef,
                                                          taps[name], True, l1), 'tap_grad', 0.0, B * H * H * c * 8.0)

        fused_taps = set()

        def dgrad(name, dst, mask_ref, tap_of=None):
            cin, cout = [(ci, co) for n, ci, co in VGG_LAYERS if n == name][0]
            H = acts[name][1]
            wtd = self.vgg_wtd[name]
            src = dbuf[name]
            flops = 2.0 * B * H * H * 9 * cin * cout
            if tap_of is not None:
                dt0 = ops.dgrad_desc(B, H, H, cin, cin, cout, cout, 3, 1, 0)
                if not self.f32 and ops.conv2d_tap_supported(dt0):
                    ya = acts[tap_of][0]
                    self._add(self.prog_bwd, lambda: ops.conv2d_tap(dt0, src, wtd, dst, ya[B:], ya[:B], cin, mask, S, self.coef,
                                                                    taps[tap_of], l1), 'vgg_dgrad', flops,
                              2.0 * (B * H * H * (3 * cin + cout) + 9 * cin * cout), name='vgg16/%s+tap(%s)' % (name, tap_of), desc=dt0)
                    fused_taps.add(tap_of)
                    return
            flags = L.CONV_MASK if mask_ref is not None else 0
            dd = ops.dgrad_desc(B, H, H, cin, cin, cout, cout, 3, 1, flags, ldmask=cin)
            self._add(self.prog_bwd, lambda: ops.conv2d(dd, src, wtd, None, dst, None, mask_ref), 'vgg_dgrad', flops,
                      2.0 * (B * H * H * (cin + cout + (cin if mask_ref is not None else 0)) + 9 * cin * cout), name='vgg16/' + name,
                      desc=dd)

        def unpool(src_name, dy, relu_mask):
            y, H = acts[src_name]
            c = y.shape[-1]
            self._add(self.prog_bwd, lambda: ops.maxpool2_bwd(y[B:], dy, dbuf[src_name], B, H, H, c, relu_mask), 'maxpool_bwd',
                      0.0, B * H * H * c * 5.0)

        def unpool_tap(name, dy):
            if l1:
                unpool(name, dy, 0); tap(name, True)
                return
            y, H = acts[name]
            c = y.shape[-1]
            self._add(self.prog_bwd, lambda: ops.unpool_tap_grad(dbuf[name], dy, y[B:], y[:B], B, H, c, mask, S, self.coef,
                                                                 taps[name]), 'tap_grad', 0.0, B * H * H * c * 8.5)

        for i in range(len(names) - 1, 0, -1):
            name, prev = names[i], names[i - 1]
            deepest = i == len(names) - 1
            if name in self.vgg_pool:
                if name in taps:
                    unpool_tap(name, dpool[name])
                else:
                    unpool(name, dpool[name], 1)
            elif name in taps and name not in fused_taps:
                tap(name, not deepest)
            if prev in self.vgg_pool:
                dgrad(name, dpool[prev], None)
            elif prev in taps:
                dgrad(name, dbuf[prev], None, tap_of=prev)
            else:
                dgrad(name, dbuf[prev], pred_half(acts[prev][0]))
        last = self.ren[-1]
        self.d_pred = self._act(B, S, S, last.lddy)
        in_idx = taps.get('input', -1)
        if names:
            self._add(self.prog_bwd, lambda: ops.vgg_conv1_1_bwd(dbuf['conv1_1'], B, S, self.w11, self.in_future, self.pred,
                                                                 self.ldp, mask, self.coef, self.d_pred, last.lddy, in_idx, l1),
                      'vgg_conv1_1_bwd', 2.0 * B * S * S * 9 * 64)
        else:
            self._add(self.prog_bwd, lambda: ops.image_loss_grad(self.in_future, self.pred, self.ldp, B, S, mask, self.coef, in_idx,
                                                                 self.d_pred, last.lddy, l1), 'image_loss_grad')

        ups = {idx: (ub, H, co) for idx, ub, H, co in self.ren_up}
        d_out, ldd = self.d_pred, last.lddy
        up_src = None
        for i in range(len(self.ren) - 1, -1, -1):
            lay = self.ren[i]
            if i == 0:
                dx, lddx = self.d_joint, Cj
            else:
                prev = self.ren[i - 1]
                if (i - 1) in ups:
                    _ub, Hp, cp = ups[i - 1]
                    dx, lddx = self._act(B, 2 * Hp, 2 * Hp, cp), cp
                else:
                    dx, lddx = self._act(B, prev.Ho, prev.Wo, prev.co), prev.co
            self._conv_backward(lay, d_out, ldd, dx, lddx, up_src=up_src)
            up_src = None
            if i > 0:
                if (i - 1) in ups:
                    _ub, Hp, cp = ups[i - 1]
                    d_prev = self._act(B, Hp, Hp, cp)
                    if prev.bn:
                        up_src = (dx, lddx)
                    else:
                        self._add(self.prog_bwd, (lambda dx=dx, d_prev=d_prev, Hp=Hp, cp=cp:
                                                  ops.upsample2x_bwd(dx, d_prev, B, Hp, Hp, cp, cp, cp)), 'upsample_bwd',
                                  0.0, B * Hp * Hp * cp * 10.0)
                    d_out, ldd = d_prev, cp
                else:
                    d_out, ldd = dx, lddx

        self.n_bwd_bucket0 = None
        if self.dp_buckets >= 2:
            for scope, fn in self._colsum_pending:
                self._add(self.prog_bwd, fn, 'colsum', name=scope)
            self._colsum_pending = []
            self._flush_wgrads('renderer')
            self.reduce_tab_ren = ops.reduce_table([j for j, _n in self._reduce_jobs], [n for _j, n in self._reduce_jobs], self.dev)
            self._add(self.prog_bwd, lambda: ops.wgrad_reduce_multi(self.reduce_tab_ren), 'wgrad_reduce', name='renderer')
            self._reduce_jobs = []
            self.n_bwd_bucket0 = len(self.prog_bwd)
        self.wg_cus = int(os.environ.get('IMM_WG_CUS', '0')) if self.dp_buckets < 2 else 0
        if self.wg_cus:
            self._mark(self.prog_bwd, 'fork', lane=2)
            self._cur_lane = 2
            self._flush_wgrads('renderer', cus=self.wg_cus)
            self.reduce_tab_ren = ops.reduce_table([j for j, _n in self._reduce_jobs], [n for _j, n in self._reduce_jobs], self.dev)
            self._add(self.prog_bwd, lambda: ops.wgrad_reduce_multi(self.reduce_tab_ren), 'wgrad_reduce', name='renderer')
            self._reduce_jobs = []
            self._cur_lane = 0
        self.bucket0_offset = self.tab.offsets[[n for n, _s, _w in self.spec].index('model/renderer/conv_1/w')]
        self._mark(self.prog_bwd, 'fork')
        nf8 = 8 * self.cfg.n_filters
        He = self.He
        ph = self.pose_head
        self.d_heat = self._act(B, He, He, ph.lddy)
        dg = self.d_joint[..., nf8:]
        d_feat = self._act(B, He, He, nf8)
        self._colsum_needs_dheat = False
        if self.fused_head:
            self.head_bias_partial = self._zeros(B, K)
            flops_h = 2.0 * B * He * He * nf8 * K
            self._add(self.prog_bwd, lambda: ops.pose_head_bwd(dg, Cj, B, He, He, K, self.inv_std, 16, self.mu, self.py, self.px,
                                                               self.d_heat, ph.lddy, ph.wt_d, nf8, d_feat, nf8,
                                                               self.head_bias_partial, self.cfg.gauss_mode), 'bottleneck_bwd', flops_h)
            self._wgrad_pending.append((ph, self.d_heat, ph.lddy, flops_h))
            gb_h = self.gview['model/pose_encoder/conv_1/b']
            self._reduce_jobs.append(((self.head_bias_partial.data_ptr(), gb_h.data_ptr(), B, 1, 1, 1, K, 1), K))
        else:
            self._add(self.prog_bwd, lambda: ops.softargmax_gauss_bwd(dg, Cj, B, He, He, K, self.inv_std, 16, self.mu, self.py,
                                                                      self.px, self.d_heat, ph.lddy, self.cfg.gauss_mode), 'bottleneck_bwd')
            if self.two_streams:
                self._signal(self.prog_bwd, 'd_heat', lane=0)
                self._colsum_needs_dheat = True
            self._conv_backward(ph, self.d_heat, ph.lddy, d_feat, nf8)
        self._encoder_backward(self.enc_pose, d_feat, nf8)

        self._cur_lane = 1
        self._cur_scope = 'loss'
        self._add(self.prog_bwd, lambda: ops.cost_ema(self.loss_out[3 * self.nfeat:], self.cost_ema, 0.99), 'cost_ema')
        if He == 16:
            self._encoder_backward(self.enc_im, self.d_joint, Cj)
        else:
            e = self.enc_im[-1]
            d_e = self._act(B, He, He, nf8)
            self._add(self.prog_bwd, lambda: ops.resize_ac_bwd(self.d_joint, d_e, B, He, He, 16, 16, nf8, Cj, nf8), 'resize_ac_bwd')
            self._encoder_backward(self.enc_im, d_e, nf8)
        if self._colsum_needs_dheat:
            self._wait(self.prog_bwd, 'd_heat', lane=1)
        for scope, fn in self._colsum_pending:
            self._add(self.prog_bwd, fn, 'colsum', name=scope)
        self._colsum_pending = []
        self._cur_lane = 0
        self._mark(self.prog_bwd, 'join')
        if self.wg_cus:
            self._mark(self.prog_bwd, 'join', lane=2)
        self._flush_wgrads('encoders' if (self.n_bwd_bucket0 is not None or self.wg_cus) else 'all layers')
        if self._reduce_jobs:
            self.reduce_tab = ops.reduce_table([j for j, _n in self._reduce_jobs], [n for _j, n in self._reduce_jobs], self.dev)
            self._add(self.prog_bwd, lambda: ops.wgrad_reduce_multi(self.reduce_tab), 'wgrad_reduce',
                      name='encoders' if (self.n_bwd_bucket0 is not None or self.wg_cus) else 'all layers')

    def _encoder_backward(self, layers, d_out, ldd):
        B = self.B
        for i in range(len(layers) - 1, -1, -1):
            lay = layers[i]
            if i > 0:
                prev = layers[i - 1]
                dx, lddx = self._act(B, prev.Ho, prev.Wo, prev.co), prev.co
            else:
                dx, lddx = None, 0
            self._conv_backward(lay, d_out, ldd, dx, lddx)
            d_out, ldd = dx, lddx

    def run(self, prog):
        if not self.two_streams:
            for l in prog:
                if l.fn is not None:
                    self._issue(l)
            return
        main = torch.cuda.current_stream(self.dev)
        streams = {0: main}
        events = {}
        joined = {0}

        def lane_stream(i):
            if i not in streams:
                streams[i] = self._side_stream(i)
            return streams[i]
        pname = ('fwd' if prog is self.prog_fwd else 'opt' if (prog is self.prog_opt or not prog) else
                 'bwd' if (prog is self.prog_bwd or prog[0] is self.prog_bwd[0]) else
                 'bwd2' if prog[-1] is self.prog_bwd[-1] else 'opt')
        if self._stamp_mode and prog is self.prog_fwd:
            self._stamp_names = []

        def stamp(lane, label):
            if not self._stamp_mode or len(self._stamp_names) >= self._stamp_buf.numel():
                return
            with torch.cuda.stream(lane_stream(lane)):
                ops.debug_stamp(self._stamp_buf, len(self._stamp_names))
            self._stamp_names.append((lane, '%s:%s' % (pname, label)))
        stamp(0, 'start')
        for l in prog:
            if l.fn is not None and l.tag in self._skip_tags:
                continue
            if l.fn is not None:
                if l.lane == 0:
                    self._issue(l)
                else:
                    with torch.cuda.stream(lane_stream(l.lane)):
                        self._issue(l)
                if self._stamp_mode == 'all':
                    stamp(l.lane, '%s %s' % (l.tag, l.name))
            elif l.tag == 'fork':
                stamp(0, 'fork' if l.lane == 1 else 'fork%d' % l.lane)
                ev = torch.cuda.Event(); ev.record(main); lane_stream(l.lane).wait_event(ev)
                stamp(l.lane, 'fork: lane %d released' % l.lane)
            elif l.tag == 'join':
                stamp(l.lane, 'join: lane %d done' % l.lane)
                stamp(0, 'join: lane 0 arrives' if l.lane == 1 else 'join%d: lane 0 arrives' % l.lane)
                ev = torch.cuda.Event(); ev.record(lane_stream(l.lane)); main.wait_event(ev)
                stamp(0, 'join: lane 0 resumes' if l.lane == 1 else 'join%d: lane 0 resumes' % l.lane)
            elif l.tag.startswith('record:'):
                stamp(l.lane, l.tag)
                ev = torch.cuda.Event(); ev.record(lane_stream(l.lane)); events[l.tag[7:]] = ev
            elif l.tag.startswith('wait:'):
                stamp(l.lane, l.tag + ' arrives')
                lane_stream(l.lane).wait_event(events[l.tag[5:]])
                stamp(l.lane, l.tag + ' resumes')
        stamp(0, 'end')

    @staticmethod
    def _issue(l):
        if l.cus:
            ops.set_cu_limit(l.cus)
            try:
                l.fn()
            finally:
                ops.set_cu_limit(0)
        else:
            l.fn()

    def stamp_report(self):
        torch.cuda.synchronize(self.dev)
        t = self._stamp_buf[:len(self._stamp_names)].cpu().tolist()
        return [((v - t[0]) / 100.0, lane, label) for v, (lane, label) in zip(t, self._stamp_names)]

    def _side_stream(self, i=1):
        if self._side is None:
            self._side = {}
        if i not in self._side:
            self._side[i] = torch.cuda.Stream(device=self.dev)
        return self._side[i]

    def run_timed(self, prog):
        evs = []
        for l in prog:
            if l.fn is None:
                continue
            e0, e1 = torch.cuda.Event(enable_timing=True), torch.cuda.Event(enable_timing=True)
            e0.record()
            self._issue(l)
            e1.record()
            evs.append((l, e0, e1))
        torch.cuda.synchronize()
        self.last_variants = [l.variant for l, _e0, _e1 in evs]
        return [(l.tag, e0.elapsed_time(e1), l.flops, l.bytes, l.name) for l, e0, e1 in evs]

    def set_inputs(self, image, future_image, mask=None):
        if getattr(self, '_stager', None) is None:
            self._stager = ops.PinnedStager()
        self._stager.copy(self.in_image, image, 'image')
        self._stager.copy(self.in_future, future_image, 'future_image')
        if self.use_mask:
            if mask is None:
                raise RuntimeError('No loss mask recieved but is required.')
            self._stager.copy(self.in_mask, mask, 'mask')

    def forward(self, training=True):
        self._training = bool(training)
        self.run(self.prog_fwd)

    def forward_model_only(self, training=False):
        self._training = bool(training)
        self.run([l for l in self.prog_fwd[:self.n_fwd_model] if l.group != 'gt'])

    def backward(self):
        self.run(self.prog_bwd)

    def snapshot(self):
        return {'params': self.params.clone(), 'm': self.adam_m.clone(), 'v': self.adam_v.clone(),
                'step': self.step_count.clone(), 'adam_t': self.adam_t.clone(), 'agg': self.loss_agg.clone(), 'grads': self.grads.clone(), 'cost_ema': self.cost_ema.clone(),
                'state': {k: v.clone() for k, v in self.state.items()},
                'loss_scale': None if self.loss_scale_state is None else self.loss_scale_state.clone()}

    def restore(self, snap):
        self.params.copy_(snap['params']); self.adam_m.copy_(snap['m']); self.adam_v.copy_(snap['v'])
        self.step_count.copy_(snap['step']); self.adam_t.copy_(snap['adam_t']); self.loss_agg.copy_(snap['agg']); self.grads.copy_(snap['grads']); self.cost_ema.copy_(snap['cost_ema'])
        for k, v in snap['state'].items():
            self.state[k].copy_(v)
        if self.loss_scale_state is not None:
            self.loss_scale_state.copy_(snap['loss_scale'])
        self.run(self.prog_pack)

    def optimizer_step(self):
        self.run(self.prog_opt)

    @property
    def loss(self):
        return self.loss_out[3 * self.nfeat + 2]

    @property
    def loss_terms(self):
        return self.loss_out[:self.nfeat]

    @property
    def loss_scale(self):
        return 1.0 if self.loss_scale_state is None else float(self.loss_scale_state[0])

    def cost_summaries(self):
        raw = [float(v) for v in self.loss_out[3 * self.nfeat:3 * self.nfeat + 3]]
        ema = [float(v) for v in self.cost_ema]
        out = {}
        for i, name in enumerate(('reconstruction_loss', 'weights_loss', 'loss_total')):
            out[name + '_raw'] = raw[i]
            out[name + '_avg'] = ema[i]
        return out

    def vgg_activations(self):
        if getattr(self, 'vgg_head_fused', False) and 'conv1_1' in self.vgg_act:
            a = self.vgg_act['conv1_1'][0]
            ops.vgg_conv1_1_fwd(self.in_future, self.pred, self.ldp, self.B, self.S, self.w11, self.b11, a, 1)
        return self.vgg_act

    def vgg_activation_rms(self):
        if not getattr(self, 'vgg_act', None):
            return {}
        if getattr(self, '_rms_scratch', None) is None:
            self._rms_scratch = (self._zeros(1024), self._zeros(1))
        part, out = self._rms_scratch
        res = {}
        for name, (y, _h) in self.vgg_activations().items():
            ops.rms16(y, part, out)
            res['activation/' + name] = float(out)
        return res

    def named_gradients(self):
        inv = 1.0 / self.loss_scale
        return OrderedDict((k, v.detach() * inv) for k, v in self.gview.items())

    @property
    def future_im_pred(self):
        return self.pred[..., :3]

    def memory_bytes(self):
        return self._alloc_bytes

    def step_flops(self):
        return sum(l.flops for p in (self.prog_fwd, self.prog_bwd) for l in p if l.fn is not None)
```

imm_amd/ops.py:

```python
import ctypes as C

import torch

from . import _lib as L
from ._lib import ConvDesc, OptHParams, call


def _s():
    return C.c_void_p(torch.cuda.current_stream().cuda_stream)


def _p(t):
    if t is None:
        return None
    return C.c_void_p(t.data_ptr())


def dtype_enum(dt):
    if dt == torch.bfloat16:
        return L.IMM_BF16
    if dt == torch.float16:
        return L.IMM_F16
    if dt == torch.float32:
        return L.IMM_F32
    raise ValueError('activation dtype must be torch.bfloat16 / torch.float16 (or torch.float32: the witness engine), got %r' % (dt,))


def round_up(x, m):
    return (x + m - 1) // m * m


def same_pad_before(n_in, k, s):
    n_out = -(-n_in // s)
    return max((n_out - 1) * s + k - n_in, 0) // 2, n_out


def fwd_desc(batch, hi, wi, ci, ldx, co, ldy, k, stride, flags, ldmask=0, kw=None):
    kw = k if kw is None else kw
    pt, ho = same_pad_before(hi, k, stride)
    pl, wo = same_pad_before(wi, kw, stride)
    return ConvDesc(batch=batch, hi=hi, wi=wi, ci=ci, ldx=ldx, ho=ho, wo=wo, co=co, ldy=ldy, kh=k, kw=kw,
                    stride=stride, pad_t=pt, pad_l=pl, updiv=1, kpad=round_up(k * kw * ci, 32), flags=flags,
                    ldmask=ldmask)


def dgrad_desc(batch, hi, wi, ci_out, lddx, co_pad, lddy, k, stride, flags, ldmask=0):
    pt, ho = same_pad_before(hi, k, stride)
    pl, wo = same_pad_before(wi, k, stride)
    return ConvDesc(batch=batch, hi=ho, wi=wo, ci=co_pad, ldx=lddy, ho=hi, wo=wi, co=ci_out, ldy=lddx, kh=k, kw=k,
                    stride=1, pad_t=k - 1 - pt, pad_l=k - 1 - pl, updiv=stride, kpad=round_up(k * k * co_pad, 32),
                    flags=flags, ldmask=ldmask)


def dgrad_s2_class_descs(batch, hi, wi, ci_out, lddx, co_pad, lddy, k, flags=0, ldmask=0):
    pt, ho = same_pad_before(hi, k, 2)
    pl, wo = same_pad_before(wi, k, 2)
    if pt != 0 or pl != 0 or hi != 2 * ho or wi != 2 * wo:
        return None
    out = []
    for py in (0, 1):
        for px in (0, 1):
            ny, nx = (k - py + 1) // 2, (k - px + 1) // 2
            d = ConvDesc(batch=batch, hi=ho, wi=wo, ci=co_pad, ldx=lddy, ho=ho, wo=wo, co=ci_out, ldy=lddx, kh=ny, kw=nx,
                         stride=1, pad_t=ny - 1, pad_l=nx - 1, updiv=1, kpad=round_up(ny * nx * co_pad, 32), flags=flags,
                         ldmask=ldmask, out_scale=2, out_off_y=py, out_off_x=px)
            out.append((d, 4 + 2 * py + px))
    return out


def device_info():
    out = (C.c_int32 * 2)()
    call('imm_device_info', C.cast(out, C.c_void_p))
    return int(out[0]), int(out[1])


def set_cu_limit(cus):
    call('imm_set_cu_limit', int(cus))


class Graph:

    def __init__(self):
        self._exec = C.c_void_p()

    def capture_begin(self):
        call('imm_graph_begin', _s())

    def capture_end(self):
        call('imm_graph_end', _s(), C.byref(self._exec))

    def launch(self):
        call('imm_graph_launch', self._exec, _s())

    def __del__(self):
        try:
            if self._exec:
                L.load().imm_graph_destroy(self._exec)
        except Exception:
            pass


def pack_weights(w, wt, mode, kh, kw, ci_real, co_real, c_pad, rows, kpad):
    call('imm_pack_weights', _p(w), _p(wt), dtype_enum(wt.dtype), mode, kh, kw, ci_real, co_real, c_pad, rows, kpad, _s())


class JobTable:

    def __init__(self, jobs, items_per_job, items_per_block, device, blocks_per_job=None):
        first = [0]
        if blocks_per_job is None:
            blocks_per_job = [max(1, -(-int(n) // items_per_block)) for n in items_per_job]
        for n in blocks_per_job:
            first.append(first[-1] + int(n))
        rows = [list(j) + [0] * (12 - len(j)) for j in jobs]
        self.jobs = torch.tensor(rows, dtype=torch.int64, device=device)
        self.blk_first = torch.tensor(first, dtype=torch.int32, device=device)
        self.n_jobs, self.n_blocks = len(jobs), first[-1]


def pack_table(jobs, device):
    blocks = []
    for j in jobs:
        n = L.load().imm_pack_weights_multi_blocks(int(j[2]), int(j[8]), int(j[9]))
        if n <= 0:
            raise L.ImmHipError('imm_pack_weights_multi_blocks(%d, %d, %d) failed' % (j[2], j[8], j[9]))
        blocks.append(n)
    return JobTable(jobs, None, None, device, blocks_per_job=blocks)


def pack_weights_multi(tab, dtype):
    call('imm_pack_weights_multi', _p(tab.jobs), _p(tab.blk_first), tab.n_jobs, tab.n_blocks, dtype_enum(dtype), _s())


def reduce_table(jobs, outputs_per_job, device):
    rows, blocks = [], []
    for j, n in zip(jobs, outputs_per_job):
        lanes = 1
        while lanes < min(16, int(j[2])):
            lanes *= 2
        rows.append(tuple(j[:8]) + (lanes,))
        blocks.append(max(1, -(-int(n) // (1024 // lanes))))
    return JobTable(rows, None, None, device, blocks_per_job=blocks)


def wgrad_reduce_multi(tab):
    call('imm_wgrad_reduce_multi', _p(tab.jobs), _p(tab.blk_first), tab.n_jobs, tab.n_blocks, _s())


def conv2d(desc, x, wt, bias, y, stats=None, mask=None):
    call('imm_conv2d', C.byref(desc), dtype_enum(x.dtype), _p(x), _p(wt), _p(bias), _p(y), _p(stats), _p(mask), _s())


def conv2d_tap_supported(desc):
    return bool(L.load().imm_conv2d_tap_supported(C.byref(desc)))


def conv2d_tap(desc, x, wt, y, a_pred, a_gt, lda, loss_mask, S, coef, idx, l1=False):
    call('imm_conv2d_tap', C.byref(desc), dtype_enum(x.dtype), _p(x), _p(wt), _p(y), _p(a_pred), _p(a_gt), lda, _p(loss_mask), S,
         _p(coef), idx, int(l1), _s())


def conv_stats_blocks(desc):
    n = L.load().imm_conv_stats_blocks(C.byref(desc))
    if n <= 0:
        raise L.ImmHipError('imm_conv_stats_blocks: ' + L.load().imm_last_error().decode())
    return n


def conv2d_wgrad(desc, x, dy, lddy, slab, nsplit):
    call('imm_conv2d_wgrad', C.byref(desc), dtype_enum(x.dtype), _p(x), _p(dy), lddy, _p(slab), nsplit, _s())


CONV_FAMILIES = {1: 'igemm', 2: 'igemm64', 3: 'halo', 4: 'halo2', 5: 'hdeep', 6: 'hdeep6', 7: 's2f', 8: 'f32'}


def conv2d_variant(desc, dtype):
    key = L.load().imm_conv2d_variant(C.byref(desc), dtype_enum(dtype))
    if key < 0:
        raise L.ImmHipError('imm_conv2d_variant: ' + L.load().imm_last_error().decode())
    return CONV_FAMILIES[key // 100000], key


def conv2d_wgrad_variant(desc, lddy, dtype):
    wps, units, pcu = C.c_int(0), C.c_int(0), C.c_int(0)
    key = L.load().imm_conv2d_wgrad_variant(C.byref(desc), lddy, dtype_enum(dtype), C.byref(wps), C.byref(units), C.byref(pcu))
    if key < 0:
        raise L.ImmHipError('imm_conv2d_wgrad_variant: ' + L.load().imm_last_error().decode())
    return key, wps.value, units.value, pcu.value


class WgradMulti(object):

    def __init__(self, jobs, dtype):
        n = len(jobs)
        self.keep = [t for j in jobs for t in (j[1], j[2], j[4])] + [t for j in jobs if len(j) > 6 and j[6] for t in j[6][:2]]
        arr = (L.WgradJob * n)()
        for i, job in enumerate(jobs):
            desc, x, dy, lddy, slab, nsplit = job[:6]
            arr[i].desc = desc
            arr[i].x, arr[i].dy, arr[i].slab = x.data_ptr(), dy.data_ptr(), slab.data_ptr()
            arr[i].lddy, arr[i].nsplit = int(lddy), int(nsplit)
            if len(job) > 6 and job[6]:
                arr[i].x_scale, arr[i].x_shift, arr[i].x_relu = job[6][0].data_ptr(), job[6][1].data_ptr(), int(bool(job[6][2]))
        nbytes = L.load().imm_conv2d_wgrad_multi_table_bytes(n)
        if nbytes <= 0:
            raise L.ImmHipError('imm_conv2d_wgrad_multi_table_bytes(%d)' % n)
        self.host = (C.c_ubyte * nbytes)()
        call('imm_conv2d_wgrad_multi_plan', C.cast(arr, C.c_void_p), n, dtype_enum(dtype), C.cast(self.host, C.c_void_p))
        self.dev = torch.frombuffer(self.host, dtype=torch.uint8).clone().to(jobs[0][1].device)
        self.n = n


def conv2d_wgrad_multi(multi):
    call('imm_conv2d_wgrad_multi', C.cast(multi.host, C.c_void_p), _p(multi.dev), _s())


def conv2d_wgrad_splits(desc, lddy):
    n = L.load().imm_conv2d_wgrad_splits(C.byref(desc), lddy)
    if n < 0:
        raise L.ImmHipError('imm_conv2d_wgrad_splits failed')
    return n


def conv2d_wgrad_reduce(slab, nsplit, kh, kw, ci_pad, ci_real, co, kpad, dw):
    call('imm_conv2d_wgrad_reduce', _p(slab), nsplit, kh, kw, ci_pad, ci_real, co, kpad, _p(dw), _s())


def colsum_blocks(npix, c):
    n = L.load().imm_colsum_blocks(npix, c)
    if n <= 0:
        raise L.ImmHipError('imm_colsum_blocks(%d,%d) unsupported' % (npix, c))
    return n


def colsum(dy, npix, c, c_out, ld, partial, out):
    call('imm_colsum', _p(dy), dtype_enum(dy.dtype), npix, c, c_out, ld, _p(partial), _p(out), _s())


def bn_finalize(partial, nblk, c, count, gamma, beta, eps, momentum, training, mm, mv, scale, shift, mean, rstd):
    call('imm_bn_finalize', _p(partial), nblk, c, count, _p(gamma), _p(beta), eps, momentum, int(training), _p(mm),
         _p(mv), _p(scale), _p(shift), _p(mean), _p(rstd), _s())


def bn_apply_relu(y, npix, c, ldy, scale, shift, relu, x_out, ldx):
    call('imm_bn_apply_relu', _p(y), dtype_enum(y.dtype), npix, c, ldy, _p(scale), _p(shift), int(relu), _p(x_out), ldx, _s())


def bn_apply_fused(partial, nblk, c, count, gamma, beta, eps, momentum, training, mm, mv, scale, shift, mean, rstd, y, ldy,
                   relu, x_out, ldx, up2x=None, ldu=0, h=0, w=0):
    call('imm_bn_apply_fused', _p(partial), nblk, c, count, _p(gamma), _p(beta), eps, momentum, int(training), _p(mm), _p(mv),
         _p(scale), _p(shift), _p(mean), _p(rstd), _p(y), dtype_enum(y.dtype), ldy, int(relu), _p(x_out), ldx,
         _p(up2x), ldu, h, w, _s())


def bn_bwd_apply_fused(partial, nblk, c, count, gamma, dout, lddo, y, ldy, scale, shift, mean, rstd, relu, dgamma, dbeta,
                       dy_out, lddy):
    call('imm_bn_bwd_apply_fused', _p(partial), nblk, c, count, _p(gamma), _p(dout), lddo, _p(y), ldy, dtype_enum(y.dtype),
         _p(scale), _p(shift), _p(mean), _p(rstd), int(relu), _p(dgamma), _p(dbeta), _p(dy_out), lddy, _s())


def bn_bwd_blocks(npix, c):
    n = L.load().imm_bn_bwd_blocks(npix, c)
    if n <= 0:
        raise L.ImmHipError('imm_bn_bwd_blocks(%d,%d) unsupported' % (npix, c))
    return n


def rows_reduce(src, rows, width, group, dst):
    call('imm_rows_reduce', _p(src), rows, width, group, _p(dst), _s())


def bn_bwd_reduce(dout, lddo, y, ldy, npix, c, scale, shift, mean, rstd, relu, partial):
    call('imm_bn_bwd_reduce', _p(dout), lddo, _p(y), ldy, dtype_enum(y.dtype), npix, c, _p(scale), _p(shift), _p(mean),
         _p(rstd), int(relu), _p(partial), _s())


def bn_bwd_reduce_up(dy_up, lddy, dprev, lddp, y, ldy, batch, h, w, c, scale, shift, mean, rstd, relu, partial):
    call('imm_bn_bwd_reduce_up', _p(dy_up), lddy, _p(dprev), lddp, _p(y), ldy, dtype_enum(y.dtype), batch, h, w, c, _p(scale),
         _p(shift), _p(mean), _p(rstd), int(relu), _p(partial), _s())


def bn_bwd_finalize(partial, nblk, c, count, gamma, beta, rstd, dgamma, dbeta, coef, from_out=False, ldp=None):
    call('imm_bn_bwd_finalize', _p(partial), nblk, c, c if ldp is None else ldp, count, _p(gamma), _p(beta), _p(rstd),
         int(from_out), _p(dgamma), _p(dbeta), _p(coef), _s())


def bn_bwd_apply(dout, lddo, y, ldy, npix, c, scale, shift, mean, rstd, relu, coef, dy_out, lddy):
    call('imm_bn_bwd_apply', _p(dout), lddo, _p(y), ldy, dtype_enum(y.dtype), npix, c, _p(scale), _p(shift), _p(mean),
         _p(rstd), int(relu), _p(coef), _p(dy_out), lddy, _s())


def upsample2x_fwd(x, y, batch, h, w, c, ldx, ldy):
# ... 13 lines not shown

def upsample2x_bwd_bn(dy, dx, batch, h, w, c, lddy, lddx, out, ldo, partial):
    call('imm_upsample2x_bwd_bn', _p(dy), _p(dx), dtype_enum(dy.dtype), batch, h, w, c, lddy, lddx, _p(out), ldo, _p(partial), _s())


def resize_ac_fwd(x, y, batch, hi, wi, ho, wo, c, ldx, ldy):
    call('imm_resize_ac_fwd', _p(x), _p(y), dtype_enum(x.dtype), batch, hi, wi, ho, wo, c, ldx, ldy, _s())


def resize_ac_bwd(dy, dx, batch, hi, wi, ho, wo, c, lddy, lddx):
    call('imm_resize_ac_bwd', _p(dy), _p(dx), dtype_enum(dy.dtype), batch, hi, wi, ho, wo, c, lddy, lddx, _s())


def maxpool2_fwd(x, y, batch, h, w, c):
    call('imm_maxpool2_fwd', _p(x), _p(y), dtype_enum(x.dtype), batch, h, w, c, _s())


def maxpool2_bwd(x, dy, dx, batch, h, w, c, relu_mask):
    call('imm_maxpool2_bwd', _p(x), _p(dy), _p(dx), dtype_enum(x.dtype), batch, h, w, c, int(relu_mask), _s())


def pack_image_taps(src, dst, batch, h, w, kw, pad_l, ld):
    call('imm_pack_image_taps', _p(src), _p(dst), dtype_enum(dst.dtype), batch, h, w, kw, pad_l, ld, _s())


def pack_image(src, dst, npix):
    call('imm_pack_image', _p(src), _p(dst), dtype_enum(dst.dtype), npix, _s())


def gauss_mode_enum(mode):
    if mode not in L.GAUSS_MODES:
        raise ValueError('Unknown mode: ' + str(mode))
    return L.GAUSS_MODES[mode]


def softargmax_gauss_fwd(heat, ldh, batch, h, w, k, inv_std, s, mu, py, px, gauss_out, ldg, dtype, mode='rot'):
    call('imm_softargmax_gauss_fwd', _p(heat), ldh, batch, h, w, k, float(inv_std), s, _p(mu), _p(py), _p(px),
         _p(gauss_out), ldg, dtype_enum(dtype), gauss_mode_enum(mode), _s())


def gauss_render_fwd(mu, batch, k, inv_std, s, gauss_out, ldg, dtype, mode='rot'):
    call('imm_softargmax_gauss_fwd', None, 0, batch, 0, 0, k, float(inv_std), s, _p(mu), None, None, _p(gauss_out), ldg,
         dtype_enum(dtype), gauss_mode_enum(mode), _s())


def softargmax_gauss_bwd(dgauss, ldg, batch, h, w, k, inv_std, s, mu, py, px, dheat, lddh, mode='rot'):
    call('imm_softargmax_gauss_bwd', _p(dgauss), ldg, dtype_enum(dheat.dtype), batch, h, w, k, float(inv_std), s, _p(mu),
         _p(py), _p(px), _p(dheat), lddh, gauss_mode_enum(mode), _s())


MAX_KEYPOINTS = 16


def keypoint_desc(w, b, geom, keypoints, image_size):
    m = int(keypoints.shape[1])
    if not 1 <= m <= MAX_KEYPOINTS:
        raise ValueError('the keypoint epilogue serves 1..%d annotated points, got %d' % (MAX_KEYPOINTS, m))
    if tuple(w.shape[1:]) != (2 * m,) or tuple(b.shape) != (2 * m,) or geom.shape[1:] != (4,) or keypoints.shape[2:] != (2,):
        raise ValueError('keypoint descriptor shapes: w %s, b %s, geom %s, keypoints %s' % (
            tuple(w.shape), tuple(b.shape), tuple(geom.shape), tuple(keypoints.shape)))
    for t in (w, b, geom, keypoints):
        if t.dtype != torch.float32 or not t.is_contiguous():
            raise ValueError('keypoint descriptor tensors must be contiguous float32')
    return L.KeypointDesc(w.data_ptr(), b.data_ptr(), geom.data_ptr(), keypoints.data_ptr(), m, int(image_size))


def pose_head_fwd(feat, ldf, c, wt, bias, batch, h, w, k, inv_std, s, heat, ldh, mu, py, px, gauss_out, ldg, dtype, mode='rot',
                  keypoints=None):
    if keypoints is not None:
        if int(keypoints.m) > MAX_KEYPOINTS or k > 64:
            raise ValueError('the keypoint epilogue serves M <= %d, K <= 64 (M=%d, K=%d)' % (MAX_KEYPOINTS, int(keypoints.m), k))
        keypoints = C.byref(keypoints)
    call('imm_pose_head_fwd', _p(feat), ldf, c, _p(wt), wt.shape[1], _p(bias), dtype_enum(dtype), batch, h, w, k, float(inv_std), s,
         _p(heat), ldh, _p(mu), _p(py), _p(px), _p(gauss_out), ldg, gauss_mode_enum(mode), keypoints, _s())


def pose_head_bwd(dgauss, ldg, batch, h, w, k, inv_std, s, mu, py, px, dheat, lddh, wt_dgrad, c, dfeat, lddf, bias_partial, mode='rot'):
    call('imm_pose_head_bwd', _p(dgauss), ldg, dtype_enum(dheat.dtype), batch, h, w, k, float(inv_std), s, _p(mu), _p(py), _p(px),
         _p(dheat), lddh, gauss_mode_enum(mode), _p(wt_dgrad), wt_dgrad.shape[1], c, _p(dfeat), lddf, _p(bias_partial), _s())


def gauss_render_f32(mu, batch, k, inv_std, s, out, mode='rot'):
    call('imm_gauss_render_f32', _p(mu), batch, k, float(inv_std), s, _p(out), gauss_mode_enum(mode), _s())


def vgg_head_supported(batch, s, dtype):
    if dtype not in (torch.bfloat16, torch.float16):
        return False
    return bool(L.load().imm_vgg_head_supported(batch, s, dtype_enum(dtype)))


def vgg_head_scratch_bytes(batch, s):
    return int(L.load().imm_vgg_head_scratch_bytes(batch, s))


def vgg_head_fwd(gt, pred, ldp, batch, s, w11, b11, wt12, b12, a11, store_from, y12, gray_scratch):
    call('imm_vgg_head_fwd', _p(gt), _p(pred), ldp, batch, s, _p(w11), _p(b11), _p(wt12), wt12.shape[1], _p(b12), _p(a11),
         store_from, _p(y12), _p(gray_scratch), dtype_enum(y12.dtype), _s())


def vgg_conv1_1_fwd(gt, pred, ldp, batch, s, w, b, out, halves=3):
    call('imm_vgg_conv1_1_fwd', _p(gt), _p(pred), ldp, batch, s, _p(w), _p(b), _p(out), dtype_enum(out.dtype), halves, _s())


def vgg_conv1_1_bwd(dz, batch, s, w, gt, pred, ldp, mask, coef, dpred, lddp, input_idx=0, l1=False):
    call('imm_vgg_conv1_1_bwd', _p(dz), dtype_enum(dz.dtype), batch, s, _p(w), _p(gt), _p(pred), ldp, _p(mask), _p(coef),
         int(input_idx), int(l1), _p(dpred), lddp, _s())


def image_loss_grad(gt, pred, ldp, batch, s, mask, coef, idx, dpred, lddp, l1=False):
    call('imm_image_loss_grad', _p(gt), _p(pred), ldp, batch, s, _p(mask), _p(coef), int(idx), int(l1), _p(dpred), lddp,
         dtype_enum(dpred.dtype), _s())


def masked_sse(a, b, batch, s, c, mask, S, partial, l1=False):
    call('imm_masked_sse', _p(a), _p(b), dtype_enum(a.dtype), batch, s, c, _p(mask), S, int(l1), _p(partial), _s())


class SseMulti:

    def __init__(self, feats):
        n = len(feats)
        self.n = n
        self.keep = feats
        self.a = (C.c_void_p * n)(*[f[0].data_ptr() for f in feats])
        self.b = (C.c_void_p * n)(*[f[1].data_ptr() for f in feats])
        self.s = (C.c_int32 * n)(*[int(f[2]) for f in feats])
        self.c = (C.c_int32 * n)(*[int(f[3]) for f in feats])
        self.p = (C.c_void_p * n)(*[f[4].data_ptr() for f in feats])
        self.dtype = feats[0][0].dtype


def masked_sse_multi(g, batch, mask, S, l1=False):
    call('imm_masked_sse_multi', g.n, C.cast(g.a, C.c_void_p), C.cast(g.b, C.c_void_p), C.cast(g.s, C.c_void_p), C.cast(g.c, C.c_void_p),
         C.cast(g.p, C.c_void_p), dtype_enum(g.dtype), batch, _p(mask), S, int(l1), _s())


def masked_sse_all(g, batch, mask, S, img_a, lda, img_b, ldb, img_c, img_partial, l1=False):
    call('imm_masked_sse_all', g.n, C.cast(g.a, C.c_void_p), C.cast(g.b, C.c_void_p), C.cast(g.s, C.c_void_p), C.cast(g.c, C.c_void_p),
         C.cast(g.p, C.c_void_p), dtype_enum(g.dtype), batch, _p(mask), S, int(l1), _p(img_a), lda, _p(img_b), ldb, img_c,
         _p(img_partial), _s())


def masked_sse_f32(a, lda, b, ldb, batch, s, c, mask, partial, l1=False):
    call('imm_masked_sse_f32', _p(a), lda, _p(b), ldb, batch, s, c, _p(mask), int(l1), _p(partial), _s())


LOSS_PERCEPTUAL, LOSS_L2 = 0, 1


def perceptual_finalize(partial, nfeat, nel, agg, training, wd_loss, out, l1=False, mode=LOSS_PERCEPTUAL, loss_scale=None):
    call('imm_perceptual_finalize', _p(partial), nfeat, _p(nel), _p(agg), int(training), _p(wd_loss), int(l1), int(mode),
         _p(loss_scale), _p(out), _s())


def tap_grad(da, has_in, a_pred, a_gt, batch, s, c, mask, S, coef, idx, relu, l1=False):
    call('imm_tap_grad', _p(da), int(has_in), _p(a_pred), _p(a_gt), dtype_enum(da.dtype), batch, s, c, _p(mask), S,
         _p(coef), idx, int(relu), int(l1), _s())


def copy_f32(dst, src):
    assert dst.dtype == torch.float32 and src.dtype == torch.float32 and dst.numel() == src.numel()
    assert dst.is_contiguous() and src.is_contiguous() and (dst.is_cuda or dst.is_pinned()) and (src.is_cuda or src.is_pinned())
    call('imm_copy_f32', _p(dst), _p(src), dst.numel(), _s())


def upload(dst, src, what='tensor'):
    if not dst.is_cuda:
        dst.copy_(torch.as_tensor(src).reshape(dst.shape))
        return
    src = torch.as_tensor(src)
    if src.is_cuda:
        dst.copy_(src.reshape(dst.shape))
        return
    stage = torch.empty(dst.shape, dtype=dst.dtype, pin_memory=True)
    stage.copy_(src.reshape(dst.shape))
    back = torch.empty(dst.shape, dtype=dst.dtype, pin_memory=True)
    stream = torch.cuda.current_stream(dst.device)
    dst.copy_(stage, non_blocking=True)
    back.copy_(dst, non_blocking=True)
    stream.synchronize()
    if not torch.equal(back.reshape(-1).view(torch.uint8), stage.reshape(-1).view(torch.uint8)):
        nbad = int((back.reshape(-1).view(torch.uint8) != stage.reshape(-1).view(torch.uint8)).sum())
        raise RuntimeError('imm_amd: host-to-device upload of %s (%d bytes) does not read back as written (%d bytes differ)'
                           % (what, stage.numel() * stage.element_size(), nbad))


class PinnedStager:

    def __init__(self):
        self._slots = {}

    def copy(self, dst, src, key=None):
        src = torch.as_tensor(src)
        if not dst.is_cuda or src.is_cuda:
            dst.copy_(src.reshape(dst.shape))
            return
        key = dst.data_ptr() if key is None else key
        ent = self._slots.get(key)
        if ent is None or ent['bufs'][0].shape != dst.shape or ent['bufs'][0].dtype != dst.dtype:
            ent = {'bufs': [torch.empty(dst.shape, dtype=dst.dtype, pin_memory=True) for _ in range(2)], 'evs': [None, None], 'i': 0}
            self._slots[key] = ent
        i = ent['i']
        ent['i'] = 1 - i
        if ent['evs'][i] is not None:
            ent['evs'][i].synchronize()
        ent['bufs'][i].copy_(src.reshape(dst.shape))
        dst.copy_(ent['bufs'][i], non_blocking=True)
        ev = torch.cuda.Event()
        ev.record(torch.cuda.current_stream(dst.device))
        ent['evs'][i] = ev


def to_device_pinned(src, device, dtype=None):
    src = torch.as_tensor(src)
    device = torch.device(device)
    dtype = src.dtype if dtype is None else dtype
    if device.type != 'cuda' or src.is_cuda:
        return src.to(device=device, dtype=dtype)
    stage = torch.empty(src.shape, dtype=dtype, pin_memory=True)
    stage.copy_(src)
    dst = torch.empty(src.shape, dtype=dtype, device=device)
    dst.copy_(stage, non_blocking=True)
    ev = torch.cuda.Event()
    ev.record(torch.cuda.current_stream(device))
    ev.synchronize()
    return dst


def download(src):
    if not src.is_cuda:
        return src.detach().clone()
    back = torch.empty(src.shape, dtype=src.dtype, pin_memory=True)
    back.copy_(src.detach(), non_blocking=True)
    torch.cuda.current_stream(src.device).synchronize()
    return back.clone()


def cost_ema(cost3, state4, decay=0.99):
    call('imm_cost_ema', _p(cost3), _p(state4), float(decay), _s())


def rms16(x, partial, out):
    assert x.is_contiguous() and x.numel() % 8 == 0
    call('imm_rms16', _p(x), x.numel(), dtype_enum(x.dtype), _p(partial), min(int(partial.numel()), 4096), _p(out), _s())


def weight_decay_loss(params, tab, blk_partial, out):
    call('imm_weight_decay_loss', _p(params), _p(tab.blk_seg), _p(tab.blk_begin), _p(tab.blk_end), tab.nblk, _p(tab.seg_wd),
         _p(blk_partial), _p(out), _s())


def clip_adam_step(params, grads, m, v, tab, blk_partial, seg_norm2, step_count, adam_t, lr_state, hp, loss_scale_state=None):
    call('imm_clip_adam_step', _p(params), _p(grads), _p(m), _p(v), _p(tab.blk_seg), _p(tab.blk_begin), _p(tab.blk_end),
         tab.nblk, tab.nseg, _p(tab.seg_first_blk), _p(tab.seg_wd), _p(blk_partial), _p(seg_norm2), _p(step_count),
         _p(adam_t), _p(lr_state), C.byref(hp), _p(loss_scale_state), _s())


class SegmentTable:
    CHUNK = 2048

    def __init__(self, sizes, wds, device):
        offs = [0]
        for n in sizes:
            offs.append(offs[-1] + int(n))
        blk_seg, blk_begin, blk_end, first = [], [], [], [0]
        for s, n in enumerate(sizes):
            for b0 in range(0, int(n), self.CHUNK):
                blk_seg.append(s)
                blk_begin.append(offs[s] + b0)
                blk_end.append(offs[s] + min(int(n), b0 + self.CHUNK))
            first.append(len(blk_seg))
        self.offsets = offs
        self.nseg, self.nblk, self.total = len(sizes), len(blk_seg), offs[-1]
        i32 = dict(dtype=torch.int32, device=device)
        self.blk_seg = torch.tensor(blk_seg, **i32)
        self.blk_begin = torch.tensor(blk_begin, **i32)
        self.blk_end = torch.tensor(blk_end, **i32)
        self.seg_first_blk = torch.tensor(first, **i32)
        self.seg_wd = torch.tensor([float(w) for w in wds], dtype=torch.float32, device=device)


def debug_stamp(slots, index):
    call('imm_debug_stamp', _p(slots), int(index), _s())


def tps_warp(src, basis_t, w_tps, dst=None, dst_c0=None, dst_rest=None):
    b, h, w, c = src.shape
    call('imm_tps_warp', _p(src), src.stride(2), b, h, w, c, _p(basis_t), basis_t.shape[0], _p(w_tps), _p(dst),
         dst.stride(2) if dst is not None else 0, _p(dst_c0), _p(dst_rest), dst_rest.stride(2) if dst_rest is not None else 0, _s())


def tps_warp_pad(src, basis_t, w_tps, pad_yx, grid_hw, crop_yx, dst):
    b, h, w, c = src.shape
    call('imm_tps_warp_pad', _p(src), src.stride(2), b, h, w, c, pad_yx[0], pad_yx[1], grid_hw[0], grid_hw[1], crop_yx[0], crop_yx[1],
         dst.shape[1], dst.shape[2], _p(basis_t), basis_t.shape[0], _p(w_tps), _p(dst), dst.stride(2), _s())


def resize_crop_u8(src_u8, offsets, hw, c, resize_hw, crop_yx, out_hw, dst, ld_dst=None, boxes=None):
    if boxes is not None and (boxes.dtype != torch.int32 or boxes.dim() != 2 or boxes.shape[1] != 5 or not boxes.is_contiguous()):
        raise ValueError('boxes must be contiguous int32 [n, 5], got %s %s' % (boxes.dtype, tuple(boxes.shape)))
    batch = hw.shape[0] if boxes is None else boxes.shape[0]
    call('imm_resize_crop_u8', _p(src_u8), _p(offsets), _p(hw), _p(boxes), batch, c, resize_hw[0], resize_hw[1], crop_yx[0],
         crop_yx[1], out_hw[0], out_hw[1], _p(dst), dst.stride(2) if ld_dst is None else ld_dst, _s())


MAX_ALIGN_M3 = 67


def align_coeffs(mu, ft, k, m3, coef):
    if ft.dtype != torch.float32 or ft.numel() != 4 * k * m3 or not ft.is_contiguous():
        raise ValueError('ft must be contiguous f32 [2K, 2 m3] = [%d, %d], got %s %s' % (2 * k, 2 * m3, ft.dtype, tuple(ft.shape)))
    n = mu.shape[0]
    assert mu.is_contiguous() and coef.is_contiguous() and mu.numel() == n * 2 * k and coef.numel() == n * 2 * m3
    call('imm_align_coeffs', _p(mu), _p(ft), n, int(k), int(m3), _p(coef), _s())


def align_warp_u8(src, offsets, hw, boxes, geom, coef, basis_t, image_size, dst, ld_dst=None):
    n, So = dst.shape[0], dst.shape[1]
    m3 = coef.shape[1]
    f32 = src.dtype == torch.float32
    if f32:
        if tuple(src.shape) != (n, image_size, image_size, 3) or not src.is_contiguous():
            raise ValueError('an f32 source must be contiguous [n, S, S, 3], got %s' % (tuple(src.shape),))
        n_images = n
    else:
        if src.dtype != torch.uint8 or offsets is None or hw is None or boxes is None:
            raise ValueError('a u8 source needs offsets, hw and boxes')
        if boxes.dtype != torch.int32 or tuple(boxes.shape) != (n, 5) or not boxes.is_contiguous():
            raise ValueError('boxes must be contiguous int32 [n, 5], got %s %s' % (boxes.dtype, tuple(boxes.shape)))
        n_images = hw.shape[0]
    if dst.shape[2] != So or tuple(geom.shape) != (n, 4) or tuple(coef.shape) != (n, m3, 2) or not (geom.is_contiguous() and coef.is_contiguous()):
        raise ValueError('dst [n, So, So, c], geom [n, 4], coef [n, m3, 2] (contiguous)')
    if (m3 > 3) != (basis_t is not None) or (basis_t is not None and (tuple(basis_t.shape) != (m3, So * So) or not basis_t.is_contiguous())):
        raise ValueError('basis_t must be contiguous f32 [m3, So * So] for m3 > 3 and None for m3 == 3')
    call('imm_align_warp_u8', _p(src), int(f32), _p(offsets), _p(hw), int(n_images), _p(boxes), _p(geom), _p(coef), _p(basis_t), int(m3),
         n, int(image_size), So, _p(dst), dst.stride(2) if ld_dst is None else ld_dst, _s())


def compose_u8(photos, offsets, hw, boxes, links, inv_ramp, faces, max_box_pixels):
    n = boxes.shape[0]
    if photos.dtype != torch.uint8 or photos.dim() != 1 or not photos.is_contiguous():
        raise ValueError('photos must be the flat contiguous u8 buffer, got %s %s' % (photos.dtype, tuple(photos.shape)))
    if boxes.dtype != torch.int32 or tuple(boxes.shape) != (n, 5) or not boxes.is_contiguous():
        raise ValueError('boxes must be contiguous int32 [n, 5], got %s %s' % (boxes.dtype, tuple(boxes.shape)))
    if links.dtype != torch.int32 or tuple(links.shape) != (n, 2) or not links.is_contiguous():
        raise ValueError('links must be contiguous int32 [n, 2], got %s %s' % (links.dtype, tuple(links.shape)))
    if inv_ramp.dtype != torch.float32 or tuple(inv_ramp.shape) != (n, 2) or not inv_ramp.is_contiguous():
        raise ValueError('inv_ramp must be contiguous f32 [n, 2], got %s %s' % (inv_ramp.dtype, tuple(inv_ramp.shape)))
    S, ld = faces.shape[1], faces.stride(2)
    if (faces.dtype != torch.float32 or faces.dim() != 4 or faces.shape[0] != n or faces.shape[2] != S or faces.shape[3] < 3 or
            faces.stride(3) != 1 or faces.stride(1) != S * ld or faces.stride(0) != S * S * ld):
        raise ValueError('faces must be f32 [n, S, S, >= 3] with dense pixels of one stride, got %s %s strides %s' % (
            faces.dtype, tuple(faces.shape), tuple(faces.stride())))
    call('imm_compose_u8', _p(photos), _p(offsets), _p(hw), int(hw.shape[0]), _p(boxes), _p(links), _p(inv_ramp), _p(faces), int(ld), n,
         int(S), int(max_box_pixels), _s())


def unalign_maps(coef, geom, boxes, hw, image_size, out_size, fwd, bbox):
    n = boxes.shape[0]
    if boxes.dtype != torch.int32 or tuple(boxes.shape) != (n, 5) or not boxes.is_contiguous():
        raise ValueError('boxes must be contiguous int32 [n, 5], got %s %s' % (boxes.dtype, tuple(boxes.shape)))
    if coef.dtype != torch.float32 or tuple(coef.shape) != (n, 3, 2) or not coef.is_contiguous():
        raise ValueError('coef must be contiguous f32 [n, 3, 2] (the similarity and affine models), got %s %s' % (
            coef.dtype, tuple(coef.shape)))
    if geom.dtype != torch.float32 or tuple(geom.shape) != (n, 4) or not geom.is_contiguous():
        raise ValueError('geom must be contiguous f32 [n, 4], got %s %s' % (geom.dtype, tuple(geom.shape)))
    if hw.dtype != torch.int32 or hw.dim() != 2 or hw.shape[1] != 2 or not hw.is_contiguous():
        raise ValueError('hw must be contiguous int32 [images, 2], got %s %s' % (hw.dtype, tuple(hw.shape)))
    if fwd.dtype != torch.float32 or tuple(fwd.shape) != (n, 6) or not fwd.is_contiguous():
        raise ValueError('fwd must be contiguous f32 [n, 6], got %s %s' % (fwd.dtype, tuple(fwd.shape)))
    if bbox.dtype != torch.int32 or tuple(bbox.shape) != (n, 4) or not bbox.is_contiguous():
        raise ValueError('bbox must be contiguous int32 [n, 4], got %s %s' % (bbox.dtype, tuple(bbox.shape)))
    call('imm_unalign_maps', _p(coef), _p(geom), _p(boxes), _p(hw), int(hw.shape[0]), n, int(image_size), int(out_size), _p(fwd),
         _p(bbox), _s())


def unalign_u8(photos, offsets, hw, boxes, links, fwd, bbox, inv_ramp, faces, max_pixels):
    n = boxes.shape[0]
    if photos.dtype != torch.uint8 or photos.dim() != 1 or not photos.is_contiguous():
        raise ValueError('photos must be the flat contiguous u8 buffer, got %s %s' % (photos.dtype, tuple(photos.shape)))
    if boxes.dtype != torch.int32 or tuple(boxes.shape) != (n, 5) or not boxes.is_contiguous():
        raise ValueError('boxes must be contiguous int32 [n, 5], got %s %s' % (boxes.dtype, tuple(boxes.shape)))
    if links.dtype != torch.int32 or tuple(links.shape) != (n, 2) or not links.is_contiguous():
        raise ValueError('links must be contiguous int32 [n, 2], got %s %s' % (links.dtype, tuple(links.shape)))
    if fwd.dtype != torch.float32 or tuple(fwd.shape) != (n, 6) or not fwd.is_contiguous():
        raise ValueError('fwd must be contiguous f32 [n, 6], got %s %s' % (fwd.dtype, tuple(fwd.shape)))
    if bbox.dtype != torch.int32 or tuple(bbox.shape) != (n, 4) or not bbox.is_contiguous():
        raise ValueError('bbox must be contiguous int32 [n, 4], got %s %s' % (bbox.dtype, tuple(bbox.shape)))
    So, ld = faces.shape[1], faces.stride(2)
    if (faces.dtype != torch.float32 or faces.dim() != 4 or faces.shape[0] != n or faces.shape[2] != So or faces.shape[3] < 3 or
            faces.stride(3) != 1 or faces.stride(1) != So * ld or faces.stride(0) != So * So * ld):
        raise ValueError('faces must be f32 [n, So, So, >= 3] with dense pixels of one stride, got %s %s strides %s' % (
            faces.dtype, tuple(faces.shape), tuple(faces.stride())))
    call('imm_unalign_u8', _p(photos), _p(offsets), _p(hw), int(hw.shape[0]), _p(boxes), _p(links), _p(fwd), _p(bbox), float(inv_ramp),
         _p(faces), int(ld), n, int(So), int(max_pixels), _s())


def track_step(mu, boxes, hw, state, image_size, next_image, init, box_smooth, min_cutoff, beta, d_cutoff, c, te, filter_off, points,
               points_smooth, boxes_next, geom_next, flags):
    F, K = mu.shape[0], mu.shape[1]
    for name, t, dt, shape in (('mu', mu, torch.float32, (F, K, 2)), ('boxes', boxes, torch.int32, (F, 5)),
                               ('state', state, torch.float64, (F, 5 + 6 * K)), ('points', points, torch.float32, (F, K, 2)),
# ... 111 lines not shown
```

imm_amd/train/cnn_train_multi.py:

```python
import json
import os
import time

import torch
import torch.distributed as dist

from .. import ops


def split_inputs(inputs, num_splits, index):
    out = {}
    for k, v in inputs.items():
        n = v.shape[0]
        assert n % num_splits == 0, 'Batch size must be divisible by number of GPUs'
        per = n // num_splits
        out[k] = v[index * per:(index + 1) * per]
    return out


def average_gradients(flat_grads, world_size, group=None, force=False, async_op=False):
    if world_size > 1 or (force and dist.is_initialized()):
        if flat_grads.is_cuda and dist.get_backend(group) == 'gloo':
            host = _pinned_like(flat_grads)
            stream = torch.cuda.current_stream(flat_grads.device)
            ops.copy_f32(host, flat_grads.detach())
            stream.synchronize()
            dist.all_reduce(host, op=dist.ReduceOp.SUM, group=group)
            ops.copy_f32(flat_grads, host)
            stream.synchronize()
            return None
        return dist.all_reduce(flat_grads, op=dist.ReduceOp.SUM, group=group, async_op=async_op)
    return None


_PINNED = {}


def _pinned_like(t):
    key = (t.numel(), t.dtype)
    if key not in _PINNED:
        _PINNED[key] = torch.empty(t.numel(), dtype=t.dtype).pin_memory()
    return _PINNED[key].view(t.shape)


def mean_tower_loss(loss, world_size, group=None):
    if world_size > 1 and dist.is_initialized():
        t = loss.detach().reshape(1).to(torch.float32).clone()
        if t.is_cuda and dist.get_backend(group) == 'gloo':
            t = t.cpu()
        dist.all_reduce(t, op=dist.ReduceOp.SUM, group=group)
        return float(t) / world_size
    return float(loss)


class TrainStep:

    COLLECTIVES = ('pg', 'native', 'graph')

    def __init__(self, model, batch_per_rank, image_size, world_size=1, use_graph=True, group=None, split_graphs=False,
                 collective=None, debug_poison=None):
        self.model = model
        self.world_size = world_size
        self.split = split_graphs or world_size > 1
        self.group = group
        model.require_vgg()
        self.engine = model._get_engine(batch_per_rank, image_size)
        model._master = self.engine
        self.buckets = 2 if self.engine.n_bwd_bucket0 is not None else 1
        if abs(self.engine.hp.grad_scale - 1.0 / world_size) > 1e-9:
            raise ValueError('engine was built for world_size %g' % (1.0 / self.engine.hp.grad_scale))
        self.use_graph = use_graph
        if collective is None:
            collective = ('graph' if os.environ.get('IMM_RCCL_GRAPH', '0') != '0' else
                          'native' if os.environ.get('IMM_RCCL_NATIVE', '0') != '0' else 'pg')
        if collective not in self.COLLECTIVES:
            raise ValueError('collective must be one of %r, got %r' % (self.COLLECTIVES, collective))
        if collective == 'graph' and not use_graph:
            raise ValueError("collective 'graph' needs use_graph=True")
        self.collective = collective if self.split else None
        if debug_poison is None:
            debug_poison = os.environ.get('IMM_DEBUG_POISON_GRADS', '0') != '0'
        self.debug_poison = bool(debug_poison)
        self._poison_mask = None
        self.after_backward = None
        self.graph_resident = self.split and use_graph and collective == 'graph'
        self.native_comm = None
        if self.split and collective in ('native', 'graph'):
            rank = dist.get_rank(group) if dist.is_initialized() else 0
            with torch.cuda.device(self.engine.dev):
                self.native_comm = ops.RcclComm(rank, world_size, group)
            self.comm_stream = torch.cuda.Stream(device=self.engine.dev)
        self.stream = torch.cuda.Stream(device=self.engine.dev)
        self._graphs = None
        torch.cuda.synchronize(self.engine.dev)

    def _probe(self, flat):
        if self.debug_poison:
            flat.mul_(2.0)

    def _poison(self):
        eng = self.engine
        if self._poison_mask is None:
            snap = eng.snapshot()
            eng.grads.fill_(float('nan'))
            eng.forward(True); eng.backward()
            torch.cuda.current_stream(eng.dev).synchronize()
            self._poison_mask = ~torch.isnan(eng.grads)
            eng.restore(snap)
            torch.cuda.current_stream(eng.dev).synchronize()
        eng.grads.masked_fill_(self._poison_mask, float('nan'))

    def _capture(self):
        eng = self.engine
        with torch.cuda.stream(self.stream):
            if self.debug_poison and self._poison_mask is None:
                snap0 = eng.snapshot(); self._poison(); eng.restore(snap0)
            snap = eng.snapshot()
            eng.forward(True); eng.backward(); eng.optimizer_step()
            self.stream.synchronize()
            eng.restore(snap)
            self.stream.synchronize()
            eng._training = True
            if self.graph_resident:
                self.native_comm.all_reduce_sum(eng.grads)
                self.stream.synchronize()
                g = ops.Graph()
                g.capture_begin()
                if self.buckets < 2:
                    eng.run(eng.prog_fwd); eng.run(eng.prog_bwd)
                    self.native_comm.all_reduce_sum(eng.grads); self._probe(eng.grads)
                else:
                    n0, off = eng.n_bwd_bucket0, eng.bucket0_offset
                    eng.run(eng.prog_fwd); eng.run(eng.prog_bwd[:n0])
                    fork = torch.cuda.Event(); fork.record(self.stream)
                    self.comm_stream.wait_event(fork)
                    with torch.cuda.stream(self.comm_stream):
                        self.native_comm.all_reduce_sum(eng.grads[off:]); self._probe(eng.grads[off:])
                    eng.run(eng.prog_bwd[n0:])
                    tail = torch.cuda.Event(); tail.record(self.stream)
                    self.comm_stream.wait_event(tail)
                    with torch.cuda.stream(self.comm_stream):
                        self.native_comm.all_reduce_sum(eng.grads[:off]); self._probe(eng.grads[:off])
                    join = torch.cuda.Event(); join.record(self.comm_stream)
                    self.stream.wait_event(join)
                eng.run(eng.prog_opt)
                if self.debug_poison:
                    self._poison()
                g.capture_end()
                self._graphs = (g,)
            elif not self.split:
                g = ops.Graph()
                g.capture_begin()
                eng.run(eng.prog_fwd); eng.run(eng.prog_bwd); eng.run(eng.prog_opt)
                g.capture_end()
                self._graphs = (g,)
            elif self.buckets < 2:
                g1 = ops.Graph()
                g1.capture_begin()
                eng.run(eng.prog_fwd); eng.run(eng.prog_bwd)
                g1.capture_end()
                g2 = ops.Graph()
                g2.capture_begin()
                eng.run(eng.prog_opt)
                g2.capture_end()
                self._graphs = (g1, g2)
            else:
                n0 = eng.n_bwd_bucket0
                g1 = ops.Graph()
                g1.capture_begin()
                eng.run(eng.prog_fwd); eng.run(eng.prog_bwd[:n0])
                g1.capture_end()
                g1b = ops.Graph()
                g1b.capture_begin()
                eng.run(eng.prog_bwd[n0:])
                g1b.capture_end()
                g2 = ops.Graph()
                g2.capture_begin()
                eng.run(eng.prog_opt)
                g2.capture_end()
                self._graphs = (g1, g1b, g2)

    def step(self, inputs=None):
        eng = self.engine
        self.stream.wait_stream(torch.cuda.current_stream(eng.dev))
        with torch.cuda.stream(self.stream):
            if inputs is not None:
                eng.set_inputs(inputs['image'], inputs['future_image'], inputs.get('mask'))
                for v in (inputs['image'], inputs['future_image'], inputs.get('mask')):
                    if torch.is_tensor(v) and v.is_cuda:
                        v.record_stream(self.stream)
            if self.use_graph:
                if self._graphs is None:
                    self._capture()
                self._graphs[0].launch()
                hook = self.after_backward
                if self.graph_resident:
                    pass
                elif self.split and self.native_comm is not None:
                    if hook is not None and self.buckets < 2:
                        hook(eng)
                    self._native_exchange(eng)
                elif self.split and self.buckets < 2:
                    if hook is not None:
                        hook(eng)
                    average_gradients(eng.grads, self.world_size, self.group, force=True); self._probe(eng.grads)
                    self._graphs[1].launch()
                elif self.split:
                    off = eng.bucket0_offset
                    w0 = average_gradients(eng.grads[off:], self.world_size, self.group, force=True, async_op=True)
                    self._graphs[1].launch()
                    if hook is not None:
                        hook(eng)
                    w1 = average_gradients(eng.grads[:off], self.world_size, self.group, force=True, async_op=True)
                    for w in (w0, w1):
                        if w is not None:
                            w.wait()
                    self._probe(eng.grads)
                    self._graphs[2].launch()
                if self.debug_poison and not self.graph_resident and self.split:
                    self._poison()
            else:
                eng.forward(True)
                eng.backward()
                if self.after_backward is not None:
                    self.after_backward(eng)
                average_gradients(eng.grads, self.world_size, self.group)
                eng.optimizer_step()
        torch.cuda.current_stream(eng.dev).wait_stream(self.stream)
        return eng.loss

    def _native_exchange(self, eng):
        def on_comm(flat):
            ev = torch.cuda.Event(); ev.record(self.stream)
            self.comm_stream.wait_event(ev)
            with torch.cuda.stream(self.comm_stream):
                self.native_comm.all_reduce_sum(flat); self._probe(flat)
        if self.buckets < 2:
            on_comm(eng.grads)
        else:
            off = eng.bucket0_offset
            on_comm(eng.grads[off:])
            self._graphs[1].launch()
            on_comm(eng.grads[:off])
        done = torch.cuda.Event(); done.record(self.comm_stream)
        self.stream.wait_event(done)
        self._graphs[-1].launch()

    def forward_only(self, inputs=None):
        eng = self.engine
        self.stream.wait_stream(torch.cuda.current_stream(eng.dev))
        with torch.cuda.stream(self.stream):
            if inputs is not None:
                eng.set_inputs(inputs['image'], inputs['future_image'], inputs.get('mask'))
                for v in (inputs['image'], inputs['future_image'], inputs.get('mask')):
                    if torch.is_tensor(v) and v.is_cuda:
                        v.record_stream(self.stream)
            if self.use_graph:
                if getattr(self, '_fwd_graph', None) is None:
                    snap = eng.snapshot()
                    eng.forward(True)
                    self.stream.synchronize()
                    eng.restore(snap)
                    self.stream.synchronize()
                    g = ops.Graph()
                    g.capture_begin()
                    eng._training = True
                    eng.run(eng.prog_fwd)
                    g.capture_end()
                    self._fwd_graph = g
                eng._training = True
                self._fwd_graph.launch()
            else:
                eng.forward(True)
        torch.cuda.current_stream(eng.dev).wait_stream(self.stream)
        return eng.loss

    def measure_phases(self, steps=5):
        eng = self.engine
        old_mode, old_buf = eng._stamp_mode, eng._stamp_buf
        eng._stamp_mode = 'marks'
        if eng._stamp_buf is None:
            eng._stamp_buf = torch.zeros(8192, dtype=torch.int64, device=eng.dev)
        self._graphs = None
        rows = []
        try:
            for _ in range(max(1, steps)):
                self.step(None)
                self.synchronize()
                rep = eng.stamp_report()
                t = {}
                for us, _lane, label in rep:
                    t[label] = us
                bwd_end = t.get('bwd2:end', t.get('bwd:end'))
                if None in (t.get('fwd:start'), t.get('fwd:end'), t.get('bwd:start'), bwd_end, t.get('opt:start'), t.get('opt:end')):
                    continue
                rows.append(((t['fwd:end'] - t['fwd:start']) / 1e3, (bwd_end - t['bwd:start']) / 1e3,
                             (t['opt:start'] - bwd_end) / 1e3, (t['opt:end'] - t['opt:start']) / 1e3))
        finally:
            eng._stamp_mode, eng._stamp_buf = old_mode, old_buf
            self._graphs = None
            self.synchronize()
        if not rows:
            return None
        med = [sorted(r[i] for r in rows)[len(rows) // 2] for i in range(4)]
        return {'forward': round(med[0], 4), 'backward': round(med[1], 4), 'exchange_exposed': round(med[2], 4),
                'optimizer': round(med[3], 4), 'steps': len(rows)}

    def synchronize(self):
        self.stream.synchronize()


def setup_training(opts, model_factory, clip_value=None, use_graph=True):
    world = int(os.environ.get('WORLD_SIZE', '1'))
    assert opts['batch_size'] % world == 0, 'Batch size must be divisible by number of GPUs'
    model = model_factory.create()
    return TrainStep(model, opts['batch_size'] // world, opts['image_size'], world_size=world, use_graph=use_graph)


class SummaryWriter(object):

    def __init__(self, log_dir):
        from ..utils.tf_events import EventFileWriter
        os.makedirs(log_dir, exist_ok=True)
        self.path = os.path.join(log_dir, 'summaries.jsonl')
        self._f = open(self.path, 'a')
        self.events = EventFileWriter(log_dir)

    def add_summary(self, record, step, images=None):
        rec = {'step': int(step), 'time': time.time()}
        rec.update(record)
        self._f.write(json.dumps(rec) + '\n')
        family = str(record.get('tag', 'train'))
        scalars = {}
        for k, v in record.items():
            if k == 'tag':
                continue
            if isinstance(v, (list, tuple)):
                for i, x in enumerate(v):
                    scalars['%s/%s/%d' % (family, k, i)] = float(x)
            else:
                scalars['%s/%s' % (family, k)] = float(v)
        self.events.add_scalars(scalars, step, images={'%s/%s' % (family, k): v for k, v in (images or {}).items()})

    def flush(self):
        self._f.flush()
        self.events.flush()

    def close(self):
        self._f.close()
        self.events.close()


def image_summaries(eng, max_outputs=3):
    from ..models.imm_model import colorize_landmark_maps
    n = min(int(max_outputs), eng.B)
    S = eng.S

    def tile(x):
        x = x[:n].float().clamp(0, 255).to(torch.uint8).cpu().numpy()
        return x.transpose(1, 0, 2, 3).reshape(S, n * S, 3)

    full = torch.empty(eng.B, S, S, eng.K, device=eng.dev)
    ops.gauss_render_f32(eng.mu, eng.B, eng.K, eng.inv_std, S, full, eng.cfg.gauss_mode)
    maps = colorize_landmark_maps(full[:n])
    maps = maps / maps.amax().clamp_min(1e-12) * 255.0
    return {'im': tile(eng.in_image), 'future_im': tile(eng.in_future), 'future_im_pred': tile(eng.future_im_pred),
            'pose_embedding': tile(maps)}


def run_test_pass(model, test_dataset, step, writer=None, verbose=True):
    total, count, it_n = 0.0, 0, 0
    for inputs in test_dataset:
        t0 = time.time()
        _, loss, _ = model.build(inputs, training_pl=False, build_loss=True)
        value = float(loss)
        n = int(inputs['image'].shape[0])
        total, count = total + value * n, count + n
        if verbose:
            dt = time.time() - t0
            print('test: step %d, loss = %.4f (%.1f examples/sec) %.3f sec/batch' % (step, value, n / dt, dt))
        it_n += 1
    if verbose:
        print('iteration through test set finished')
    mean = total / max(count, 1)
    if writer is not None and count:
        writer.add_summary({'tag': 'test', 'loss': mean, 'n_samples': count}, step)
        writer.flush()
    return mean


def train_loop(opts, train_step, data_iter, num_steps, log_every=10, checkpoint_fn=None, test_dataset=None, model=None,
               summary_writer=None, fwd_only=False):
    t_start, n_seen = time.time(), 0
    rank = int(os.environ.get('RANK', '0'))
    eng = train_step.engine
    start_step = int(eng.step_count)
    n_summary = int(opts.get('n_summary') or 0)
    n_image = int(opts.get('n_image_summary', 100) or 0)
    n_test = int(opts.get('n_test') or 0)
    n_ckpt = int(opts.get('n_checkpoint') or 0)
    scaled = getattr(eng, 'loss_scale_state', None) is not None
    step = start_step
    last_event_step = None
    while fwd_only and step < num_steps:
        t0 = time.time()
        loss = train_step.forward_only(next(data_iter))
        n_seen += opts['batch_size']
        if (step - start_step) % log_every == 0:
            train_step.synchronize()
            loss_value = mean_tower_loss(loss, train_step.world_size, train_step.group)
            assert loss_value == loss_value, 'Model diverged with loss = NaN'
            dt = time.time() - t0
            if rank == 0:
                print('step %d, loss = %.4f (%.1f examples/sec; %.3f sec/batch) [fwd_only]' % (step, loss_value, opts['batch_size'] / dt, dt))
        step += 1
    while step < num_steps:
        t0 = time.time()
        loss = train_step.step(next(data_iter))
        n_seen += opts['batch_size']
        do_log = (step - start_step) % log_every == 0
        do_sum = bool(n_summary) and step % n_summary == 0
        synced = False
        if scaled and (do_log or do_sum or (n_test and step % n_test == 0) or (n_ckpt and step % n_ckpt == 0)):
# ... 45 lines not shown
```

include/imm_hip.h:

```cpp
#ifndef IMM_HIP_H
#define IMM_HIP_H

#include <stdint.h>

#ifdef __cplusplus
extern "C" {
#endif

#define IMM_ABI_VERSION 28

enum imm_dtype { IMM_BF16 = 0, IMM_F16 = 1, IMM_F32 = 2 };

enum imm_error {
  IMM_OK = 0,
  IMM_E_INVALID = -1,
  IMM_E_UNSUPPORTED = -2,
  IMM_E_HIP = -3
};

#define IMM_CONV_BIAS 1
#define IMM_CONV_RELU 2
#define IMM_CONV_STATS 4
#define IMM_CONV_MASK 8
#define IMM_CONV_OUT_F32 16

typedef struct imm_conv_desc {
  int32_t batch, hi, wi, ci;
  int32_t ldx;
  int32_t ho, wo, co;
  int32_t ldy;
  int32_t kh, kw, stride, pad_t, pad_l;
  int32_t updiv;
  int32_t kpad;
  int32_t flags;
  int32_t ldmask;
  int32_t out_scale, out_off_y, out_off_x;
} imm_conv_desc;

int imm_abi_version(void);
const char* imm_last_error(void);
const char* imm_source_digest(void);
int imm_device_info(int32_t* out2_host);
int imm_set_cu_limit(int cus);
int imm_get_cu_limit(void);
int imm_debug_stamp(uint64_t* slots, int index, void* stream);
int imm_copy_f32(float* dst, const float* src, int64_t n, void* stream);
int imm_graph_begin(void* stream);
int imm_graph_end(void* stream, void** graph_exec_out_host);
int imm_graph_launch(void* graph_exec, void* stream);
int imm_graph_destroy(void* graph_exec);

int imm_pack_weights(const float* w, void* wt, int dtype, int mode, int kh, int kw, int ci_real, int co_real,
                     int c_pad, int rows, int kpad, void* stream);

int imm_pack_weights_multi_blocks(int mode, int rows, int kpad);
int imm_pack_weights_multi(const int64_t* jobs, const int32_t* blk_first, int n_jobs, int n_blocks, int dtype,
                           void* stream);
int imm_wgrad_reduce_multi(const int64_t* jobs, const int32_t* blk_first, int n_jobs, int n_blocks, void* stream);

int imm_conv2d_group(const imm_conv_desc* descs, int n, int dtype, const void* x, const void* const* wts, void* y,
                     float* stats_partial, const void* mask_ref, void* stream);
int imm_conv2d_group_stats_blocks(const imm_conv_desc* descs, int n);
int imm_conv2d_nol_supported(const imm_conv_desc* desc_host);
int imm_conv2d_nol_stats_blocks(const imm_conv_desc* desc_host);
int imm_conv2d_nol(const imm_conv_desc* desc_host, int dtype, const void* x_raw, const float* x_scale, const float* x_shift,
                   int x_relu, const void* wt, const float* bias, void* y, float* stats_partial, void* stream);
int imm_conv2d_dgrad_s2_supported(int batch, int h, int w, int lddy, int c_dx, int lddx);
int imm_conv2d_dgrad_s2(const void* dy, int lddy, const void* wt, int kpad, void* dx, int lddx, int c_dx, int dtype, int batch,
                        int h, int w, void* stream);
int imm_conv2d(const imm_conv_desc* desc_host, int dtype, const void* x, const void* wt, const float* bias,
               void* y, float* stats_partial, const void* mask_ref, void* stream);
int imm_conv_stats_blocks(const imm_conv_desc* desc_host);
int imm_conv2d_variant(const imm_conv_desc* desc_host, int dtype);
int imm_conv2d_tap_supported(const imm_conv_desc* desc_host);
int imm_conv2d_tap(const imm_conv_desc* desc_host, int dtype, const void* x, const void* wt, void* y, const void* a_pred,
                   const void* a_gt, int lda, const float* loss_mask, int S, const float* coef, int idx, int l1, void* stream);
int imm_conv2d_wgrad(const imm_conv_desc* desc_host, int dtype, const void* x, const void* dy, int lddy,
                     float* slab, int nsplit, void* stream);
int imm_conv2d_wgrad_splits(const imm_conv_desc* desc_host, int lddy);
int imm_conv2d_wgrad_reduce(const float* slab, int nsplit, int kh, int kw, int ci_pad, int ci_real, int co,
                            int kpad, float* dw, void* stream);
typedef struct imm_wgrad_job {
  imm_conv_desc desc;
  const void* x; const void* dy; float* slab;
  int32_t lddy, nsplit;
  const float* x_scale; const float* x_shift;
  int32_t x_relu, reserved;
} imm_wgrad_job;
int64_t imm_conv2d_wgrad_multi_table_bytes(int n);
int imm_conv2d_wgrad_variant(const imm_conv_desc* desc_host, int lddy, int dtype, int* wg_per_split_host, int* units_host,
                             int* wg_per_cu_host);
int imm_conv2d_wgrad_multi_plan(const imm_wgrad_job* jobs_host, int n, int dtype, void* table_host);
int imm_conv2d_wgrad_multi(const void* table_host, const void* table_dev, void* stream);
int imm_colsum(const void* dy, int dtype, int64_t npix, int c, int c_out, int ld, float* partial, float* out,
               void* stream);
int imm_colsum_blocks(int64_t npix, int c);

int imm_bn_finalize(const float* partial, int nblk, int c, int64_t count, const float* gamma, const float* beta,
                    float eps, float momentum, int training, float* moving_mean, float* moving_var,
                    float* scale, float* shift, float* mean, float* rstd, void* stream);
int imm_bn_apply_relu(const void* y, int dtype, int64_t npix, int c, int ldy, const float* scale,
                      const float* shift, int relu, void* x_out, int ldx, void* stream);
int imm_bn_apply_fused(const float* partial, int nblk, int c, int64_t count, const float* gamma, const float* beta, float eps,
                       float momentum, int training, float* moving_mean, float* moving_var, float* scale, float* shift,
                       float* mean, float* rstd, const void* y, int dtype, int ldy, int relu, void* x_out, int ldx,
                       void* up2x_out, int ldu, int h, int w, void* stream);
int imm_rows_reduce(const float* in, int rows, int width, int group, float* out, void* stream);
int imm_bn_bwd_reduce(const void* dout, int lddo, const void* y, int ldy, int dtype, int64_t npix, int c,
                      const float* scale, const float* shift, const float* mean, const float* rstd, int relu,
                      float* partial, void* stream);
int imm_bn_bwd_blocks(int64_t npix, int c);
int imm_bn_bwd_reduce_up(const void* dy_up, int lddy, void* dprev, int lddp, const void* y, int ldy, int dtype, int batch, int h,
                         int w, int c, const float* scale, const float* shift, const float* mean, const float* rstd, int relu,
                         float* partial, void* stream);
int imm_bn_bwd_finalize(const float* partial, int nblk, int c, int ldp, int64_t count, const float* gamma, const float* beta,
                        const float* rstd, int from_out, float* dgamma, float* dbeta, float* coef, void* stream);
int imm_bn_bwd_apply(const void* dout, int lddo, const void* y, int ldy, int dtype, int64_t npix, int c,
                     const float* scale, const float* shift, const float* mean, const float* rstd, int relu,
                     const float* coef, void* dy_out, int lddy, void* stream);
int imm_bn_bwd_apply_fused(const float* partial, int nblk, int c, int64_t count, const float* gamma, const void* dout, int lddo,
                           const void* y, int ldy, int dtype, const float* scale, const float* shift, const float* mean,
                           const float* rstd, int relu, float* dgamma, float* dbeta, void* dy_out, int lddy, void* stream);

int imm_upsample2x_fwd(const void* x, void* y, int dtype, int batch, int h, int w, int c, int ldx, int ldy,
                       void* stream);
int imm_upsample2x_bwd(const void* dy, void* dx, int dtype, int batch, int h, int w, int c, int lddy, int lddx,
                       void* stream);
int imm_upsample2x_bwd_bn(const void* dy, void* dx, int dtype, int batch, int h, int w, int c, int lddy, int lddx,
                          const void* out, int ldo, float* partial, void* stream);
int imm_upsample2x_bwd_bn_blocks(int batch, int h, int w, int c);
int imm_resize_ac_fwd(const void* x, void* y, int dtype, int batch, int hi, int wi, int ho, int wo, int c,
                      int ldx, int ldy, void* stream);
int imm_resize_ac_bwd(const void* dy, void* dx, int dtype, int batch, int hi, int wi, int ho, int wo, int c,
                      int lddy, int lddx, void* stream);
int imm_maxpool2_fwd(const void* x, void* y, int dtype, int batch, int h, int w, int c, void* stream);
int imm_maxpool2_bwd(const void* x, const void* dy, void* dx, int dtype, int batch, int h, int w, int c,
                     int relu_mask, void* stream);

int imm_pack_image(const float* src, void* dst, int dtype, int64_t npix, void* stream);
int imm_pack_image_taps(const float* src, void* dst, int dtype, int batch, int h, int w, int kw, int pad_l, int ld,
                        void* stream);

int imm_conv_first_supported(int batch, int s, int co, int ldy);
int imm_conv_first_stats_blocks(int batch, int s);
int imm_conv_first(const float* image, const void* wt, int kpad, const float* bias, void* y, int ldy, float* stats_partial, int dtype,
                   int batch, int s, int co, int flags, void* stream);

#define IMM_GAUSS_ROT 0
#define IMM_GAUSS_FLAT 1
#define IMM_GAUSS_ANKUSH 2
int imm_softargmax_gauss_fwd(const float* heat, int ldh, int batch, int h, int w, int k, float inv_std, int s,
                             float* mu, float* py, float* px, void* gauss_out, int ldg, int dtype, int gauss_mode,
                             void* stream);
int imm_softargmax_gauss_bwd(const void* dgauss, int ldg, int dtype, int batch, int h, int w, int k, float inv_std,
                             int s, const float* mu, const float* py, const float* px, void* dheat, int lddh,
                             int gauss_mode, void* stream);
typedef struct imm_keypoint_desc {
  const float* w;
  const float* b;
  const float* geom;
  float* keypoints;
  int32_t m;
  int32_t image_size;
} imm_keypoint_desc;
int imm_pose_head_fwd(const void* feat, int ldf, int c, const void* wt, int kpad, const float* bias, int dtype, int batch, int h,
                      int w, int k, float inv_std, int s, float* heat, int ldh, float* mu, float* py, float* px, void* gauss_out,
                      int ldg, int gauss_mode, const imm_keypoint_desc* kp, void* stream);
int imm_pose_head_bwd(const void* dgauss, int ldg, int dtype, int batch, int h, int w, int k, float inv_std, int s, const float* mu,
                      const float* py, const float* px, void* dheat, int lddh, int gauss_mode, const void* wt_dgrad, int kpad_d,
                      int c, void* dfeat, int lddf, float* bias_partial, void* stream);
int imm_gauss_render_f32(const float* mu, int batch, int k, float inv_std, int s, float* out, int gauss_mode, void* stream);

int imm_vgg_conv1_1_fwd(const float* gt, const float* pred, int ldp, int batch, int s, const float* w9x64,
                        const float* b64, void* out, int dtype, int halves, void* stream);
int imm_vgg_head_supported(int batch, int s, int dtype);
int64_t imm_vgg_head_scratch_bytes(int batch, int s);
int imm_vgg_head_fwd(const float* gt, const float* pred, int ldp, int batch, int s, const float* w9x64, const float* b64,
                     const void* wt12, int kpad12, const float* b12, void* a11, int store_from, void* y12, void* gray_scratch,
                     int dtype, void* stream);
int imm_vgg_conv1_1_bwd(const void* dz, int dtype, int batch, int s, const float* w9x64, const float* gt,
                        const float* pred, int ldp, const float* mask, const float* coef, int input_idx, int l1,
                        void* dpred, int lddp, void* stream);
int imm_image_loss_grad(const float* gt, const float* pred, int ldp, int batch, int s, const float* mask,
                        const float* coef, int idx, int l1, void* dpred, int lddp, int dtype, void* stream);

#define IMM_SSE_BLOCKS 512
int imm_masked_sse_multi(int n, const void* const* a, const void* const* b, const int32_t* s_host, const int32_t* c_host,
                         float* const* partial, int dtype, int batch, const float* mask, int S, int l1, void* stream);
int imm_masked_sse_all(int n, const void* const* a, const void* const* b, const int32_t* s_host, const int32_t* c_host,
                       float* const* partial, int dtype, int batch, const float* mask, int S, int l1,
                       const float* img_a, int lda, const float* img_b, int ldb, int img_c, float* img_partial, void* stream);
int imm_masked_sse(const void* a, const void* b, int dtype, int batch, int s, int c, const float* mask, int S, int l1,
                   float* partial, void* stream);
int imm_masked_sse_pool(const void* a, const void* b, int dtype, int batch, int s, int c, const float* mask, int S,
                        float* partial, void* pool_a, void* pool_b, void* stream);
int imm_masked_sse_f32(const float* a, int lda, const float* b, int ldb, int batch, int s, int c, const float* mask,
                       int l1, float* partial, void* stream);
#define IMM_LOSS_PERCEPTUAL 0
#define IMM_LOSS_L2 1
int imm_perceptual_finalize(const float* partial, int nfeat, const float* nel, float* agg, int training,
                            const float* wd_loss, int l1, int mode, const float* loss_scale, float* out, void* stream);
int imm_cost_ema(const float* cost3, float* state4, float decay, void* stream);
int imm_rms16(const void* x, int64_t n, int dtype, float* partial, int nblk, float* out, void* stream);
int imm_unpool_tap_grad(void* da, const void* dpool, const void* a_pred, const void* a_gt, int dtype, int batch, int s, int c,
                        const float* mask, int S, const float* coef, int idx, void* stream);
int imm_tap_grad(void* da, int has_in, const void* a_pred, const void* a_gt, int dtype, int batch, int s, int c,
                 const float* mask, int S, const float* coef, int idx, int relu, int l1, void* stream);

#define IMM_OPT_ADAM 0
#define IMM_OPT_ADADELTA 1
#define IMM_OPT_ADAGRAD 2
typedef struct imm_opt_hparams {
  float lr_start, lr_decay; int32_t lr_step; float lr_multiple;
  float beta1, beta2, eps, clip;
  float grad_scale;
  int32_t optim;
  int32_t scale_growth_interval;
  float scale_max;
} imm_opt_hparams;
int imm_weight_decay_loss(const float* params, const int32_t* blk_seg, const int32_t* blk_begin,
                          const int32_t* blk_end, int nblk, const float* seg_wd, float* blk_partial, float* out,
                          void* stream);
int imm_clip_adam_step(float* params, float* grads, float* m, float* v, const int32_t* blk_seg,
                       const int32_t* blk_begin, const int32_t* blk_end, int nblk, int nseg,
                       const int32_t* seg_first_blk, const float* seg_wd, float* blk_partial, float* seg_norm2,
                       int32_t* step_count, int32_t* adam_t, float* lr_state, const imm_opt_hparams* hp_host,
                       float* loss_scale_state, void* stream);

int imm_rccl_unique_id(void* out128_host);
int imm_rccl_init(int rank, int world, const void* unique_id128_host, void** comm_out_host);
int imm_rccl_allreduce(void* comm, float* buf, int64_t count, void* stream);
int imm_rccl_destroy(void* comm);

int64_t imm_conv2d_workspace_bytes(const imm_conv_desc* desc_host);
int64_t imm_conv2d_group_workspace_bytes(const imm_conv_desc* descs, int n);
int64_t imm_conv2d_wgrad_workspace_bytes(const imm_conv_desc* desc_host, int lddy, int nsplit);
int64_t imm_colsum_workspace_bytes(int64_t npix, int c);
int64_t imm_bn_bwd_workspace_bytes(int64_t npix, int c);
int64_t imm_upsample2x_bwd_bn_workspace_bytes(int batch, int h, int w, int c);
int64_t imm_masked_sse_workspace_bytes(int nfeat);

int imm_tps_warp(const float* src, int ld_src, int batch, int h, int w, int c, const float* basis_t, int m3,
                 const float* w_tps, float* dst, int ld_dst, float* dst_c0, float* dst_rest, int ld_rest, void* stream);
int imm_tps_warp_pad(const float* src, int ld_src, int batch, int h, int w, int c, int pad_y, int pad_x, int grid_h, int grid_w,
                     int crop_y, int crop_x, int out_h, int out_w, const float* basis_t, int m3, const float* w_tps,
                     float* dst, int ld_dst, void* stream);

int imm_resize_crop_u8(const uint8_t* src, const int64_t* offsets, const int32_t* hw, const int32_t* boxes, int batch, int c,
                       int resize_h, int resize_w, int crop_y0, int crop_x0, int out_h, int out_w, float* dst, int ld_dst,
                       void* stream);





int imm_crc32c(const void* data, uint64_t n, uint32_t* crc_inout);

#ifdef __cplusplus
}
#endif
#include "imm_align.h"
#include "imm_compose.h"
#include "imm_unalign.h"
#include "imm_track.h"
#endif
```

Baseline: 10250 images/s.

## Fold weight-gradient slab reduction and weight-decay loss into optimizer tail kernels

Adds a fused optimizer tail. The split-K weight-gradient slab reduction now happens inside the grad-prepare/clip pass, and each block of the Adam kernel emits per-block weight-decay partials for the next step's loss. The perceptual finalize kernel then reduces those partials itself, so the separate weight-decay loss pass and the standalone slab-reduce launches go away. The aim is fewer kernel launches and fewer passes over the flat gradient buffer. In exchange it adds table plumbing, relies on an ensure_wd_rows initialization so the first step's weight-decay term is valid, and changes the reduction order.

```diff
diff --git a/__graft_entry__.py b/__graft_entry__.py
--- a/__graft_entry__.py
+++ b/__graft_entry__.py
@@ -12,7 +12,7 @@
     import imm_amd
     from imm_amd import _lib
     handle = _lib.load()
-    for name in _lib.declared_symbols() + _lib.alignment_symbols() + _lib.compose_symbols() + _lib.unalign_symbols() + _lib.track_symbols():
+    for name in _lib.declared_symbols() + _lib.alignment_symbols() + _lib.compose_symbols() + _lib.unalign_symbols() + _lib.track_symbols() + _lib.opt_tail_symbols():
         getattr(handle, name)
     from oracle import imm_oracle, np_ref
     print('built', lib)
diff --git a/imm_amd/_lib.py b/imm_amd/_lib.py
--- a/imm_amd/_lib.py
+++ b/imm_amd/_lib.py
@@ -11,7 +11,7 @@
 SSE_BLOCKS = 512
 OPTIMIZERS = {'adam': 0, 'adadelta': 1, 'adagrad': 2}
 GAUSS_MODES = {'rot': 0, 'flat': 1, 'ankush': 2}
-ABI_VERSION = 28
+ABI_VERSION = 29
 
 
 class ImmHipError(RuntimeError):
@@ -167,6 +167,12 @@
 _lib = None
 
 
+_SIGS_OPT_TAIL = {
+    'imm_opt_tail_step': [_P, _P, _P, _P, _P, _P, _P, _I, _I, _P, _P, _P, _P, _P, _P, _P, _P, _P, C.POINTER(OptHParams), _P, _I, _P],
+    'imm_perceptual_finalize_wd': [_P, _I, _P, _P, _I, _P, _I, _I, _I, _P, _P, _P],
+}
+
+
 def declared_symbols():
     return sorted(list(_SIGS) + list(_SIGS64) + ['imm_last_error', 'imm_source_digest'])
 
@@ -185,6 +191,10 @@
 
 def track_symbols():
     return sorted(_SIGS_TRACK)
+
+
+def opt_tail_symbols():
+    return sorted(_SIGS_OPT_TAIL)
 
 
 def load():
@@ -206,7 +216,7 @@
     for name in ('imm_last_error', 'imm_source_digest'):
         getattr(lib, name).restype = C.c_char_p
         getattr(lib, name).argtypes = []
-    for name, args in list(_SIGS.items()) + list(_SIGS_ALIGN.items()) + list(_SIGS_COMPOSE.items()) + list(_SIGS_UNALIGN.items()) + list(_SIGS_TRACK.items()):
+    for name, args in list(_SIGS.items()) + list(_SIGS_ALIGN.items()) + list(_SIGS_COMPOSE.items()) + list(_SIGS_UNALIGN.items()) + list(_SIGS_TRACK.items()) + list(_SIGS_OPT_TAIL.items()):
         fn = getattr(lib, name)
         fn.argtypes = args
         fn.restype = C.c_int
diff --git a/imm_amd/csrc/loss_optim.hip b/imm_amd/csrc/loss_optim.hip
--- a/imm_amd/csrc/loss_optim.hip
+++ b/imm_amd/csrc/loss_optim.hip
@@ -277,13 +277,28 @@
                                                                          const float* __restrict__ nel, float* agg,
                                                                          int training, const float* __restrict__ wd_loss,
                                                                          int l1, int mode, const float* __restrict__ loss_scale,
-                                                                         float* __restrict__ out) {
+                                                                         float* __restrict__ out,
+                                                                         const float* __restrict__ wd_partial, int n_wd) {
   __shared__ double sse[16];
+  __shared__ double wdred[LO_THREADS];
   const int tid = threadIdx.x, lane = tid & 63, wave = tid >> 6;
+  if (wd_partial && tid >= PF_THREADS - LO_THREADS) {
+    const int t = tid - (PF_THREADS - LO_THREADS);
+    double v = 0.0;
+    for (int i0 = t; i0 < n_wd; i0 += 8 * LO_THREADS) {
+      float x[8];
+#pragma unroll
+      for (int k = 0; k < 8; ++k) x[k] = wd_partial[min(i0 + k * LO_THREADS, n_wd - 1)];
+#pragma unroll
+      for (int k = 0; k < 8; ++k)
+        if (i0 + k * LO_THREADS < n_wd) v += (double)x[k];
+    }
+    wdred[t] = v;
+  }
   const float nel_f = tid < nfeat ? nel[tid] : 1.f;
   const float agg_f = tid < nfeat ? agg[tid] : 1.f;
   const float ls = (tid < nfeat && loss_scale) ? loss_scale[0] : 1.f;
-  const float wd = (tid == 0 && wd_loss) ? wd_loss[0] : 0.f;
+  float wd = (tid == 0 && wd_loss) ? wd_loss[0] : 0.f;
   if (wave < nfeat) {
     const float* pf = partial + wave * IMM_SSE_BLOCKS + lane;
     float x[IMM_SSE_BLOCKS / 64];
@@ -297,6 +312,12 @@
     if (lane == 0) sse[wave] = v;
   }
   __syncthreads();
+  if (wd_partial && wave == 0) {
+    double a = (wdred[lane] + wdred[lane + 128]) + (wdred[lane + 64] + wdred[lane + 192]);
+#pragma unroll
+    for (int o = 32; o >= 1; o >>= 1) a += __shfl_down(a, o, 64);
+    if (tid == 0) wd = (float)a;
+  }
   if (mode == IMM_LOSS_L2) {
     if (tid == 0) {
       const float m = (float)(sse[0] / (double)nel_f);
@@ -338,8 +359,20 @@
   IMM_REQUIRE(partial && nel && agg && out && nfeat > 0 && nfeat <= 16, "perceptual_finalize: args");
   IMM_REQUIRE(mode == IMM_LOSS_PERCEPTUAL || (mode == IMM_LOSS_L2 && nfeat == 1 && !l1), "perceptual_finalize: mode");
   hipLaunchKernelGGL(perceptual_finalize_kernel, dim3(1), dim3(PF_THREADS), 0, (hipStream_t)stream, partial, nfeat, nel,
-                     agg, training, wd_loss, l1, mode, loss_scale, out);
+                     agg, training, wd_loss, l1, mode, loss_scale, out, (const float*)nullptr, 0);
   IMM_CHECK_LAUNCH("imm_perceptual_finalize");
+  return 0;
+}
+
+extern "C" int imm_perceptual_finalize_wd(const float* partial, int nfeat, const float* nel, float* agg, int training,
+                                          const float* wd_partial, int n_wd, int l1, int mode, const float* loss_scale,
+                                          float* out, void* stream) {
+  IMM_REQUIRE(partial && nel && agg && out && nfeat > 0 && nfeat <= 16, "perceptual_finalize_wd: args");
+  IMM_REQUIRE(wd_partial && n_wd > 0, "perceptual_finalize_wd: chunk rows");
+  IMM_REQUIRE(mode == IMM_LOSS_PERCEPTUAL || (mode == IMM_LOSS_L2 && nfeat == 1 && !l1), "perceptual_finalize_wd: mode");
+  hipLaunchKernelGGL(perceptual_finalize_kernel, dim3(1), dim3(PF_THREADS), 0, (hipStream_t)stream, partial, nfeat, nel,
+                     agg, training, (const float*)nullptr, l1, mode, loss_scale, out, wd_partial, n_wd);
+  IMM_CHECK_LAUNCH("imm_perceptual_finalize_wd");
   return 0;
 }
 
@@ -576,6 +609,18 @@
   return 0;
 }
 
+template <typename V> __device__ __forceinline__ V zerov();
+template <> __device__ __forceinline__ float zerov<float>() { return 0.f; }
+template <> __device__ __forceinline__ float4 zerov<float4>() { return make_float4(0.f, 0.f, 0.f, 0.f); }
+template <typename V> __device__ __forceinline__ V ldv(const float* p);
+template <> __device__ __forceinline__ float ldv<float>(const float* p) { return *p; }
+template <> __device__ __forceinline__ float4 ldv<float4>(const float* p) { return *(const float4*)p; }
+template <> __device__ __forceinline__ float2 zerov<float2>() { return make_float2(0.f, 0.f); }
+template <> __device__ __forceinline__ float2 ldv<float2>(const float* p) { return *(const float2*)p; }
+__device__ __forceinline__ float2 addv(float2 a, float2 b) { return make_float2(a.x + b.x, a.y + b.y); }
+__device__ __forceinline__ float addv(float a, float b) { return a + b; }
+__device__ __forceinline__ float4 addv(float4 a, float4 b) { return make_float4(a.x + b.x, a.y + b.y, a.z + b.z, a.w + b.w); }
+
 __device__ __forceinline__ void opt_learning_rate(const imm_opt_hparams& hp, int gs, int tt, float* lr_t, float* lr) {
   const double l = (double)hp.lr_multiple * (double)hp.lr_start * pow((double)hp.lr_decay, (double)(gs / hp.lr_step));
   *lr_t = (float)(l * sqrt(1.0 - pow((double)hp.beta2, (double)tt)) / (1.0 - pow((double)hp.beta1, (double)tt)));
@@ -623,6 +668,7 @@
   if (threadIdx.x == 0) blk_partial[blk] = acc;
 }
 
+#define OPT_WD_STAGE 2048
 __global__ __launch_bounds__(LO_THREADS) void clip_adam_kernel(float* __restrict__ params, const float* __restrict__ grads,
                                                                float* __restrict__ m, float* __restrict__ v,
                                                                const int32_t* __restrict__ blk_seg,
@@ -632,8 +678,11 @@
                                                                const float* __restrict__ blk_partial, int nblk,
                                                                float* __restrict__ seg_norm2, int32_t* __restrict__ step_count,
                                                                int32_t* __restrict__ adam_t, const float* __restrict__ lr_state,
-                                                               float* __restrict__ ls, imm_opt_hparams hp) {
+                                                               float* __restrict__ ls, imm_opt_hparams hp,
+                                                               const float* __restrict__ seg_wd, float* __restrict__ wd_partial) {
   __shared__ double dred[LO_THREADS / 64];
+  __shared__ float red[4];
+  __shared__ float wl[OPT_WD_STAGE];
   const int blk = blockIdx.x, tid = threadIdx.x;
   const bool extra = blk == nblk;
   const int seg = extra ? 0 : blk_seg[blk];
@@ -702,18 +751,42 @@
       w -= lr * g / sqrtf(vi);
     }
   };
-  for (int i = b0 + tid; i < a0; i += LO_THREADS) one(grads[i], m[i], v[i], params[i]);
+  const float wdc = wd_partial ? seg_wd[seg] : 0.f;
+  const bool stage = wdc != 0.f && b1 - b0 <= OPT_WD_STAGE;
+  for (int i = b0 + tid; i < a0; i += LO_THREADS) {
+    float w = params[i];
+    one(grads[i], m[i], v[i], w);
+    params[i] = w;
+    if (stage) wl[i - b0] = w;
+  }
   if (first) {
     one(g0.x, m0.x, v0.x, w0.x); one(g0.y, m0.y, v0.y, w0.y); one(g0.z, m0.z, v0.z, w0.z); one(g0.w, m0.w, v0.w, w0.w);
     *(float4*)(m + i0) = m0; *(float4*)(v + i0) = v0; *(float4*)(params + i0) = w0;
+    if (stage) { float* q = wl + (i0 - b0); q[0] = w0.x; q[1] = w0.y; q[2] = w0.z; q[3] = w0.w; }
   }
   for (int i = i0 + 4 * LO_THREADS; i < a1; i += 4 * LO_THREADS) {
     const float4 g = *(const float4*)(grads + i);
     float4 mi = *(const float4*)(m + i), vi = *(const float4*)(v + i), w = *(const float4*)(params + i);
     one(g.x, mi.x, vi.x, w.x); one(g.y, mi.y, vi.y, w.y); one(g.z, mi.z, vi.z, w.z); one(g.w, mi.w, vi.w, w.w);
     *(float4*)(m + i) = mi; *(float4*)(v + i) = vi; *(float4*)(params + i) = w;
-  }
-  for (int i = a1 + tid; i < b1; i += LO_THREADS) one(grads[i], m[i], v[i], params[i]);
+    if (stage) { float* q = wl + (i - b0); q[0] = w.x; q[1] = w.y; q[2] = w.z; q[3] = w.w; }
+  }
+  for (int i = a1 + tid; i < b1; i += LO_THREADS) {
+    float w = params[i];
+    one(grads[i], m[i], v[i], w);
+    params[i] = w;
+    if (stage) wl[i - b0] = w;
+  }
+  if (wd_partial) {
+    __syncthreads();
+    float acc = 0.f;
+    if (stage)
+      for (int i = tid; i < b1 - b0; i += LO_THREADS) { const float w = wl[i]; acc += w * w; }
+    else if (wdc != 0.f)
+      for (int i = b0 + tid; i < b1; i += LO_THREADS) { const float w = params[i]; acc += w * w; }
+    acc = block_sum_256(acc, red);
+    if (tid == 0) wd_partial[blk] = 0.5f * wdc * acc;
+  }
 }
 
 extern "C" int imm_clip_adam_step(float* params, float* grads, float* m, float* v, const int32_t* blk_seg,
@@ -729,7 +802,153 @@
   hipLaunchKernelGGL(grad_prepare_kernel, dim3(nblk + 1), dim3(LO_THREADS), 0, s, params, grads, blk_seg, blk_begin, blk_end,
                      seg_wd, hp->grad_scale, loss_scale_state, blk_partial, nblk, step_count, adam_t, lr_state, *hp);
   hipLaunchKernelGGL(clip_adam_kernel, dim3(nblk + 1), dim3(LO_THREADS), 0, s, params, grads, m, v, blk_seg, blk_begin, blk_end,
-                     seg_first_blk, blk_partial, nblk, seg_norm2, step_count, adam_t, lr_state, loss_scale_state, *hp);
+                     seg_first_blk, blk_partial, nblk, seg_norm2, step_count, adam_t, lr_state, loss_scale_state, *hp,
+                     (const float*)nullptr, (float*)nullptr);
   IMM_CHECK_LAUNCH("imm_clip_adam_step");
   return 0;
 }
+
+#define OPT_SLAB_FIELDS 8
+
+template <int SL, typename V>
+__device__ __forceinline__ V slab_sum(const float* __restrict__ sp, int nsplit, int64_t sstride, bool two) {
+  V acc[SL], a1[SL];
+#pragma unroll
+  for (int l = 0; l < SL; ++l) { acc[l] = zerov<V>(); a1[l] = zerov<V>(); }
+  const int last = nsplit - 1;
+#pragma unroll 1
+  for (int s0 = 0; s0 < nsplit; s0 += 2 * SL) {
+    V x[SL];
+#pragma unroll
+    for (int l = 0; l < SL; ++l) x[l] = ldv<V>(sp + (int64_t)min(s0 + l, last) * sstride);
+#pragma unroll
+    for (int l = 0; l < SL; ++l)
+      if (s0 + l < nsplit) acc[l] = addv(acc[l], x[l]);
+    if (s0 + SL < nsplit) {
+#pragma unroll
+      for (int l = 0; l < SL; ++l) x[l] = ldv<V>(sp + (int64_t)min(s0 + SL + l, last) * sstride);
+#pragma unroll
+      for (int l = 0; l < SL; ++l)
+        if (s0 + SL + l < nsplit) {
+          if (two) a1[l] = addv(a1[l], x[l]);
+          else acc[l] = addv(acc[l], x[l]);
+        }
+    }
+  }
+  V total = two ? addv(acc[0], a1[0]) : acc[0];
+#pragma unroll
+  for (int l = 1; l < SL; ++l) total = addv(total, two ? addv(acc[l], a1[l]) : acc[l]);
+  return total;
+}
+
+template <int SL>
+__device__ __forceinline__ float opt_prepare_chunk(const float* __restrict__ params, float* __restrict__ grads,
+                                                   const int64_t* __restrict__ d, int b0, int b1, float grad_scale, float wd) {
+  const float* __restrict__ slab = SL ? (const float*)d[0] : nullptr;
+  const int nsplit = SL ? (int)d[1] : 0, ci_pad = SL ? (int)d[2] : 1, ci_real = SL ? (int)d[3] : 1, co = SL ? (int)d[4] : 1;
+  const int64_t sstride = SL ? d[5] * (int64_t)co : 0;
+  const int off = SL ? (int)d[7] : 0;
+  const bool two = (co & 3) == 0;
+  const bool wide = two && ((uintptr_t)slab & 15) == 0;
+  auto at = [&](int e) -> const float* {
+    const int n = e % co, tc = e / co;
+    const int c = tc % ci_real, tap = tc / ci_real;
+    return slab + ((int64_t)tap * ci_pad + c) * co + n;
+  };
+  auto one = [&](int i) -> float { return SL ? slab_sum<SL ? SL : 1, float>(at(i - off), nsplit, sstride, two) : grads[i]; };
+  auto col = [&](int e) -> float4 {
+    const float* sp = at(e);
+    if (SL < 16) return slab_sum<SL ? SL : 1, float4>(sp, nsplit, sstride, true);
+    const float2 lo = slab_sum<16, float2>(sp, nsplit, sstride, true), hi = slab_sum<16, float2>(sp + 2, nsplit, sstride, true);
+    return make_float4(lo.x, lo.y, hi.x, hi.y);
+  };
+  auto quad = [&](int i) -> float4 {
+    const int e = i - off, k = e & 3;
+    const float4 q0 = col(e - k);
+    if (k == 0) return q0;
+    const float4 q1 = col(e - k + 4);
+    return k == 1 ? make_float4(q0.y, q0.z, q0.w, q1.x) : k == 2 ? make_float4(q0.z, q0.w, q1.x, q1.y)
+                                                                 : make_float4(q0.w, q1.x, q1.y, q1.z);
+  };
+  float acc = 0.f;
+  const int a0 = min((b0 + 3) & ~3, b1), a1 = max(a0, b1 & ~3);
+  for (int i = b0 + threadIdx.x; i < a0; i += LO_THREADS) {
+    const float g = one(i) * grad_scale + wd * params[i];
+    grads[i] = g; acc += g * g;
+  }
+  for (int i = a0 + 4 * threadIdx.x; i < a1; i += 4 * LO_THREADS) {
+    float4 g;
+    if (!SL) g = *(const float4*)(grads + i);
+    else if (wide) g = quad(i);
+    else { g.x = one(i); g.y = one(i + 1); g.z = one(i + 2); g.w = one(i + 3); }
+    const float4 w = *(const float4*)(params + i);
+    g.x = g.x * grad_scale + wd * w.x; g.y = g.y * grad_scale + wd * w.y;
+    g.z = g.z * grad_scale + wd * w.z; g.w = g.w * grad_scale + wd * w.w;
+    *(float4*)(grads + i) = g;
+    acc += (g.x * g.x + g.y * g.y) + (g.z * g.z + g.w * g.w);
+  }
+  for (int i = a1 + threadIdx.x; i < b1; i += LO_THREADS) {
+    const float g = one(i) * grad_scale + wd * params[i];
+    grads[i] = g; acc += g * g;
+  }
+  return acc;
+}
+
+__global__ __launch_bounds__(LO_THREADS) void grad_reduce_prepare_kernel(const float* __restrict__ params, float* __restrict__ grads,
+                                                                         const int32_t* __restrict__ blk_seg,
+                                                                         const int32_t* __restrict__ blk_begin,
+                                                                         const int32_t* __restrict__ blk_end,
+                                                                         const float* __restrict__ seg_wd,
+                                                                         const int64_t* __restrict__ blk_slab, float grad_scale,
+                                                                         const float* __restrict__ loss_scale,
+                                                                         float* __restrict__ blk_partial, int nblk,
+                                                                         const int32_t* __restrict__ step_count,
+                                                                         const int32_t* __restrict__ adam_t, float* __restrict__ lr_state,
+                                                                         imm_opt_hparams hp) {
+  __shared__ float red[4];
+  const int blk = blockIdx.x;
+  if (blk == nblk) {
+    if (threadIdx.x == 0) opt_learning_rate(hp, step_count[0], adam_t[0] + 1, lr_state, lr_state + 1);
+    return;
+  }
+  if (loss_scale) grad_scale *= 1.f / loss_scale[0];
+  const float wd = seg_wd[blk_seg[blk]];
+  const int b0 = blk_begin[blk], b1 = blk_end[blk];
+  const int64_t* d = blk_slab ? blk_slab + (int64_t)blk * OPT_SLAB_FIELDS : nullptr;
+  const int lanes = (d && d[0]) ? (int)d[6] : 0;
+  float acc;
+  switch (lanes) {
+    case 0: acc = opt_prepare_chunk<0>(params, grads, d, b0, b1, grad_scale, wd); break;
+    case 1: acc = opt_prepare_chunk<1>(params, grads, d, b0, b1, grad_scale, wd); break;
+    case 2: acc = opt_prepare_chunk<2>(params, grads, d, b0, b1, grad_scale, wd); break;
+    case 4: acc = opt_prepare_chunk<4>(params, grads, d, b0, b1, grad_scale, wd); break;
+    case 8: acc = opt_prepare_chunk<8>(params, grads, d, b0, b1, grad_scale, wd); break;
+    default: acc = opt_prepare_chunk<16>(params, grads, d, b0, b1, grad_scale, wd); break;
+  }
+  acc = block_sum_256(acc, red);
+  if (threadIdx.x == 0) blk_partial[blk] = acc;
+}
+
+extern "C" int imm_opt_tail_step(float* params, float* grads, float* m, float* v, const int32_t* blk_seg,
+                                 const int32_t* blk_begin, const int32_t* blk_end, int nblk, int nseg,
+                                 const int32_t* seg_first_blk, const float* seg_wd, const int64_t* blk_slab, float* blk_partial,
+                                 float* wd_partial, float* seg_norm2, int32_t* step_count, int32_t* adam_t, float* lr_state,
+                                 const imm_opt_hparams* hp, float* loss_scale_state, int stages, void* stream) {
+  IMM_REQUIRE(params && grads && m && v && blk_seg && blk_begin && blk_end && seg_first_blk && seg_wd && blk_partial &&
+                  seg_norm2 && step_count && adam_t && lr_state && hp, "opt_tail_step: null");
+  IMM_REQUIRE(nblk > 0 && nseg > 0 && hp->lr_step > 0, "opt_tail_step: dims");
+  IMM_REQUIRE(hp->optim >= IMM_OPT_ADAM && hp->optim <= IMM_OPT_ADAGRAD, "opt_tail_step: optim %d", hp->optim);
+  IMM_REQUIRE(stages >= 1 && stages <= 3, "opt_tail_step: stages %d (1 = gradient pass, 2 = update, 3 = both)", stages);
+  IMM_REQUIRE(wd_partial != blk_partial, "opt_tail_step: wd_partial must be a buffer of its own");
+  hipStream_t s = (hipStream_t)stream;
+  if (stages & 1)
+    hipLaunchKernelGGL(grad_reduce_prepare_kernel, dim3(nblk + 1), dim3(LO_THREADS), 0, s, params, grads, blk_seg, blk_begin,
+                       blk_end, seg_wd, blk_slab, hp->grad_scale, loss_scale_state, blk_partial, nblk, step_count, adam_t,
+                       lr_state, *hp);
+  if (stages & 2)
+    hipLaunchKernelGGL(clip_adam_kernel, dim3(nblk + 1), dim3(LO_THREADS), 0, s, params, grads, m, v, blk_seg, blk_begin, blk_end,
+                       seg_first_blk, blk_partial, nblk, seg_norm2, step_count, adam_t, lr_state, loss_scale_state, *hp,
+                       seg_wd, wd_partial);
+  IMM_CHECK_LAUNCH("imm_opt_tail_step");
+  return 0;
+}
diff --git a/imm_amd/engine.py b/imm_amd/engine.py
--- a/imm_amd/engine.py
+++ b/imm_amd/engine.py
@@ -178,6 +178,9 @@
         self.adam_t = torch.zeros(1, dtype=torch.int32, device=self.dev)
         self.lr_state = self._zeros(2)
         self.wd_loss = self._zeros(1)
+        self.wd_partial = self._zeros(self.tab.nblk)
+        self._wd_valid = False
+        self._grads_flat = False
         hp = dict(lr_start=1e-3, lr_decay=0.95, lr_step=100000, lr_multiple=1.0, beta1=0.9, beta2=0.999, eps=1e-8,
                   clip=1.0, grad_scale=1.0 / world_size, optim='adam', scale_growth_interval=1000, scale_max=2.0 ** 24)
         hp.update(hparams or {})
@@ -216,6 +219,7 @@
         self._pack_jobs, self._reduce_jobs, self._wgrad_pending, self._colsum_pending = [], [], [], []
         self._training = True
         self._build_network()
+        self._build_folded_tail()
         self.init_parameters(seed)
 
     def _zeros(self, *shape, dtype=torch.float32):
@@ -860,6 +864,8 @@
         self._add(self.prog_fwd, lambda: ops.perceptual_finalize(self.sse_partial, nfeat, self.nel, self.loss_agg,
                                                                  self._training, self.wd_loss, self.loss_out, l1, mode,
                                                                  self.loss_scale_state), 'loss_finalize')
+        self._finalize_wd = lambda: ops.perceptual_finalize_wd(self.sse_partial, nfeat, self.nel, self.loss_agg, self._training,
+                                                               self.wd_partial, self.loss_out, l1, mode, self.loss_scale_state)
         self.coef = self.loss_out[2 * nfeat:3 * nfeat]
 
         self._build_backward()
@@ -871,6 +877,61 @@
                                                             self.adam_t, self.lr_state, self.hp, self.loss_scale_state),
                   'clip_adam', 0.0, self.tab.total * 36.0)
         self.prog_opt.extend(self.prog_pack)
+
+    def _build_folded_tail(self):
+        self._prog_std = (list(self.prog_fwd), list(self.prog_bwd), list(self.prog_opt))
+        self._prog_fold = None
+        self.tail_folded = False
+        last = self.prog_bwd[-1] if self.prog_bwd else None
+        ok = (self.world_size == 1 and self.dp_buckets < 2 and not self.wg_cus and last is not None and last.tag == 'wgrad_reduce'
+              and bool(self._reduce_jobs) and os.environ.get('IMM_OPT_TAIL', '1') != '0')
+        if not ok:
+            return
+        self._fold_slabs = os.environ.get('IMM_OPT_TAIL', '1') != 'wd'
+        self.slab_tab = ops.slab_table(self.tab, [j for j, _n in self._reduce_jobs], self.grads, self.dev)
+        self._reduce_launch = last
+
+        def tail(stages, slabs):
+            return lambda: ops.opt_tail_step(self.params, self.grads, self.adam_m, self.adam_v, self.tab,
+                                             self.slab_tab if slabs else None, self.opt_blk_partial, self.wd_partial, self.seg_norm2,
+                                             self.step_count, self.adam_t, self.lr_state, self.hp, self.loss_scale_state, stages)
+        slab_bytes = sum(float(j[2]) * n * 4.0 for j, n in self._reduce_jobs)
+        fwd = []
+        for l in self.prog_fwd:
+            if l.tag == 'wd_loss':
+                l = _Launch(None, 'folded:wd_loss', lane=l.lane, group=l.group)
+            elif l.tag == 'loss_finalize':
+                l = _Launch(self._finalize_wd, l.tag, l.flops, l.bytes, l.name, l.lane, l.variant, l.cus, l.group)
+            fwd.append(l)
+        opt = [_Launch(tail(1, True), 'wgrad_reduce', 0.0, slab_bytes + self.tab.total * 8.0, last.name + ' + grad_prepare'),
+               _Launch(tail(2, True), 'clip_adam', 0.0, self.tab.total * 28.0)] + list(self.prog_pack)
+        self._prog_opt_flat = [_Launch(tail(3, False), 'clip_adam', 0.0, self.tab.total * 36.0)] + list(self.prog_pack)
+        if self._fold_slabs:
+            self._prog_fold = (fwd, list(self.prog_bwd[:-1]), opt)
+        else:
+            self._prog_fold = (fwd, list(self.prog_bwd), list(self._prog_opt_flat))
+        self.set_tail(True)
+
+    def set_tail(self, folded):
+        folded = bool(folded) and self._prog_fold is not None
+        if folded == self.tail_folded:
+            return
+        for dst, src in zip((self.prog_fwd, self.prog_bwd, self.prog_opt), self._prog_fold if folded else self._prog_std):
+            dst[:] = src
+        self.tail_folded = folded
+        self._grads_flat = False
+
+    def params_written(self):
+        self._wd_valid = False
+
+    def ensure_wd_rows(self):
+        if self.tail_folded and not self._wd_valid:
+            ops.weight_decay_loss(self.params, self.tab, self.wd_partial, self.wd_loss)
+            self._wd_valid = True
+
+    def _update_issued(self):
+        if not torch.cuda.is_current_stream_capturing():
+            self._wd_valid = 'clip_adam' not in self._skip_tags
 
     def _pack_vgg(self):
         if not self.vgg_layers:
@@ -1083,10 +1144,14 @@
             d_out, ldd = dx, lddx
 
     def run(self, prog):
+        if prog is self.prog_pack:
+            self._wd_valid = False
         if not self.two_streams:
             for l in prog:
                 if l.fn is not None:
                     self._issue(l)
+            if prog is self.prog_opt and self.tail_folded:
+                self._update_issued()
             return
         main = torch.cuda.current_stream(self.dev)
         streams = {0: main}
@@ -1138,6 +1203,8 @@
                 lane_stream(l.lane).wait_event(events[l.tag[5:]])
                 stamp(l.lane, l.tag + ' resumes')
         stamp(0, 'end')
+        if prog is self.prog_opt and self.tail_folded:
+            self._update_issued()
 
     @staticmethod
     def _issue(l):
@@ -1188,6 +1255,7 @@
 
     def forward(self, training=True):
         self._training = bool(training)
+        self.ensure_wd_rows()
         self.run(self.prog_fwd)
 
     def forward_model_only(self, training=False):
@@ -1196,6 +1264,10 @@
 
     def backward(self):
         self.run(self.prog_bwd)
+        if self.tail_folded and self._fold_slabs:
+            if self._reduce_launch.tag not in self._skip_tags:
+                self._issue(self._reduce_launch)
+            self._grads_flat = True
 
     def snapshot(self):
         return {'params': self.params.clone(), 'm': self.adam_m.clone(), 'v': self.adam_v.clone(),
@@ -1213,6 +1285,11 @@
         self.run(self.prog_pack)
 
     def optimizer_step(self):
+        if self.tail_folded and self._grads_flat:
+            self._grads_flat = False
+            self.run(self._prog_opt_flat)
+            self._update_issued()
+            return
         self.run(self.prog_opt)
 
     @property
diff --git a/imm_amd/ops.py b/imm_amd/ops.py
--- a/imm_amd/ops.py
+++ b/imm_amd/ops.py
@@ -132,12 +132,17 @@
     call('imm_pack_weights_multi', _p(tab.jobs), _p(tab.blk_first), tab.n_jobs, tab.n_blocks, dtype_enum(dtype), _s())
 
 
+def reduce_lanes(nsplit):
+    lanes = 1
+    while lanes < min(16, int(nsplit)):
+        lanes *= 2
+    return lanes
+
+
 def reduce_table(jobs, outputs_per_job, device):
     rows, blocks = [], []
     for j, n in zip(jobs, outputs_per_job):
-        lanes = 1
-        while lanes < min(16, int(j[2])):
-            lanes *= 2
+        lanes = reduce_lanes(j[2])
         rows.append(tuple(j[:8]) + (lanes,))
         blocks.append(max(1, -(-int(n) // (1024 // lanes))))
     return JobTable(rows, None, None, device, blocks_per_job=blocks)
@@ -457,6 +462,11 @@
 def perceptual_finalize(partial, nfeat, nel, agg, training, wd_loss, out, l1=False, mode=LOSS_PERCEPTUAL, loss_scale=None):
     call('imm_perceptual_finalize', _p(partial), nfeat, _p(nel), _p(agg), int(training), _p(wd_loss), int(l1), int(mode),
          _p(loss_scale), _p(out), _s())
+
+
+def perceptual_finalize_wd(partial, nfeat, nel, agg, training, wd_partial, out, l1=False, mode=LOSS_PERCEPTUAL, loss_scale=None):
+    call('imm_perceptual_finalize_wd', _p(partial), nfeat, _p(nel), _p(agg), int(training), _p(wd_partial), int(wd_partial.numel()),
+         int(l1), int(mode), _p(loss_scale), _p(out), _s())
 
 
 def tap_grad(da, has_in, a_pred, a_gt, batch, s, c, mask, S, coef, idx, relu, l1=False):
@@ -554,6 +564,35 @@
 def weight_decay_loss(params, tab, blk_partial, out):
     call('imm_weight_decay_loss', _p(params), _p(tab.blk_seg), _p(tab.blk_begin), _p(tab.blk_end), tab.nblk, _p(tab.seg_wd),
          _p(blk_partial), _p(out), _s())
+
+
+OPT_SLAB_FIELDS = 8
+
+
+def slab_table(tab, jobs, grads, device):
+    base = grads.data_ptr()
+    by_off = {}
+    for j in jobs:
+        off, rem = divmod(int(j[1]) - base, 4)
+        if rem or off not in tab.offsets[:-1]:
+            raise ValueError('slab_table: a job does not write a whole tensor of the flat gradient buffer')
+        seg = tab.offsets.index(off)
+        if int(j[3]) * int(j[5]) * int(j[6]) != tab.offsets[seg + 1] - off or off in by_off:
+            raise ValueError('slab_table: job and tensor %d disagree' % seg)
+        if int(j[3]) * int(j[4]) > int(j[7]) or int(j[5]) > int(j[4]) or int(j[2]) < 1:
+            raise ValueError('slab_table: slab geometry of tensor %d' % seg)
+        by_off[off] = (int(j[0]), int(j[2]), int(j[4]), int(j[5]), int(j[6]), int(j[7]), reduce_lanes(j[2]), off)
+    zero = (0,) * OPT_SLAB_FIELDS
+    seg_of = tab.blk_seg.tolist()
+    rows = [by_off.get(tab.offsets[s], zero) for s in seg_of]
+    return torch.tensor(rows, dtype=torch.int64, device=device)
+
+
+def opt_tail_step(params, grads, m, v, tab, blk_slab, blk_partial, wd_partial, seg_norm2, step_count, adam_t, lr_state, hp,
+                  loss_scale_state=None, stages=3):
+    call('imm_opt_tail_step', _p(params), _p(grads), _p(m), _p(v), _p(tab.blk_seg), _p(tab.blk_begin), _p(tab.blk_end),
+         tab.nblk, tab.nseg, _p(tab.seg_first_blk), _p(tab.seg_wd), _p(blk_slab), _p(blk_partial), _p(wd_partial), _p(seg_norm2),
+         _p(step_count), _p(adam_t), _p(lr_state), C.byref(hp), _p(loss_scale_state), int(stages), _s())
 
 
 def clip_adam_step(params, grads, m, v, tab, blk_partial, seg_norm2, step_count, adam_t, lr_state, hp, loss_scale_state=None):
diff --git a/imm_amd/train/cnn_train_multi.py b/imm_amd/train/cnn_train_multi.py
--- a/imm_amd/train/cnn_train_multi.py
+++ b/imm_amd/train/cnn_train_multi.py
@@ -58,7 +58,7 @@
     COLLECTIVES = ('pg', 'native', 'graph')
 
     def __init__(self, model, batch_per_rank, image_size, world_size=1, use_graph=True, group=None, split_graphs=False,
-                 collective=None, debug_poison=None):
+                 collective=None, debug_poison=None, fold_tail=None):
         self.model = model
         self.world_size = world_size
         self.split = split_graphs or world_size > 1
@@ -70,6 +70,7 @@
         if abs(self.engine.hp.grad_scale - 1.0 / world_size) > 1e-9:
             raise ValueError('engine was built for world_size %g' % (1.0 / self.engine.hp.grad_scale))
         self.use_graph = use_graph
+        self.fold = (not self.split) and (fold_tail is None or bool(fold_tail)) and self.engine._prog_fold is not None
         if collective is None:
             collective = ('graph' if os.environ.get('IMM_RCCL_GRAPH', '0') != '0' else
                           'native' if os.environ.get('IMM_RCCL_NATIVE', '0') != '0' else 'pg')
@@ -116,7 +117,12 @@
             if self.debug_poison and self._poison_mask is None:
                 snap0 = eng.snapshot(); self._poison(); eng.restore(snap0)
             snap = eng.snapshot()
-            eng.forward(True); eng.backward(); eng.optimizer_step()
+            if self.fold:
+                eng._training = True
+                eng.ensure_wd_rows()
+                eng.run(eng.prog_fwd); eng.run(eng.prog_bwd); eng.run(eng.prog_opt)
+            else:
+                eng.forward(True); eng.backward(); eng.optimizer_step()
             self.stream.synchronize()
             eng.restore(snap)
             self.stream.synchronize()
@@ -182,6 +188,7 @@
 
     def step(self, inputs=None):
         eng = self.engine
+        eng.set_tail(self.fold)
         self.stream.wait_stream(torch.cuda.current_stream(eng.dev))
         with torch.cuda.stream(self.stream):
             if inputs is not None:
@@ -192,7 +199,11 @@
             if self.use_graph:
                 if self._graphs is None:
                     self._capture()
+                if self.fold:
+                    eng.ensure_wd_rows()
                 self._graphs[0].launch()
+                if self.fold:
+                    eng._update_issued()
                 hook = self.after_backward
                 if self.graph_resident:
                     pass
@@ -219,6 +230,10 @@
                     self._graphs[2].launch()
                 if self.debug_poison and not self.graph_resident and self.split:
                     self._poison()
+            elif self.fold and self.after_backward is None:
+                eng._training = True
+                eng.ensure_wd_rows()
+                eng.run(eng.prog_fwd); eng.run(eng.prog_bwd); eng.run(eng.prog_opt)
             else:
                 eng.forward(True)
                 eng.backward()
@@ -248,6 +263,7 @@
 
     def forward_only(self, inputs=None):
         eng = self.engine
+        eng.set_tail(self.fold)
         self.stream.wait_stream(torch.cuda.current_stream(eng.dev))
         with torch.cuda.stream(self.stream):
             if inputs is not None:
@@ -269,6 +285,7 @@
                     g.capture_end()
                     self._fwd_graph = g
                 eng._training = True
+                eng.ensure_wd_rows()
                 self._fwd_graph.launch()
             else:
                 eng.forward(True)
diff --git a/include/imm_hip.h b/include/imm_hip.h
--- a/include/imm_hip.h
+++ b/include/imm_hip.h
@@ -7,7 +7,7 @@
 extern "C" {
 #endif
 
-#define IMM_ABI_VERSION 28
+#define IMM_ABI_VERSION 29
 
 enum imm_dtype { IMM_BF16 = 0, IMM_F16 = 1, IMM_F32 = 2 };
 
@@ -254,6 +254,7 @@
 
 
 
+
 int imm_crc32c(const void* data, uint64_t n, uint32_t* crc_inout);
 
 #ifdef __cplusplus
@@ -263,4 +264,5 @@
 #include "imm_compose.h"
 #include "imm_unalign.h"
 #include "imm_track.h"
+#include "imm_opt_tail.h"
 #endif
diff --git a/include/imm_opt_tail.h b/include/imm_opt_tail.h
--- /dev/null
+++ b/include/imm_opt_tail.h
@@ -0,0 +1,25 @@
+#ifndef IMM_OPT_TAIL_H
+#define IMM_OPT_TAIL_H
+
+#include <stdint.h>
+
+#ifdef __cplusplus
+extern "C" {
+#endif
+
+#define IMM_OPT_SLAB_FIELDS 8
+
+int imm_opt_tail_step(float* params, float* grads, float* m, float* v, const int32_t* blk_seg, const int32_t* blk_begin,
+                      const int32_t* blk_end, int nblk, int nseg, const int32_t* seg_first_blk, const float* seg_wd,
+                      const int64_t* blk_slab, float* blk_partial, float* wd_partial, float* seg_norm2, int32_t* step_count,
+                      int32_t* adam_t, float* lr_state, const imm_opt_hparams* hp_host, float* loss_scale_state, int stages,
+                      void* stream);
+
+int imm_perceptual_finalize_wd(const float* partial, int nfeat, const float* nel, float* agg, int training,
+                               const float* wd_partial, int n_wd, int l1, int mode, const float* loss_scale, float* out,
+                               void* stream);
+
+#ifdef __cplusplus
+}
+#endif
+#endif
```

New measurement: 9793 images/s. 4.4% lower.
